# gopi-erabati/Object-Pose-Estimation

Measured on NVIDIA B200. Metric: frames_per_sec_fpfh_sacia_icp_640x480, higher is better.
Workload: dtype f32

## Files before the change

object-pose-estimation_b200/csrc/pipeline.cu:

```cuda
#include <algorithm>
#include <atomic>
#include <cmath>
#include <functional>
#include <memory>
#include <thread>
#include <sched.h>

#include "ope_host.cuh"

using namespace ope;


namespace {

bool model_cache_enabled() {
  const char* e = std::getenv("OPE_MODEL_CACHE");
  return !e || std::atoi(e) != 0;
}

int clone_cloud(ope_ctx* ctx, const ope_cloud* in, ope_cloud** out) {
  ope_cloud* o = nullptr;
  OPE_TRY(cloud_alloc(ctx, in->n, in->normals != nullptr, &o));
  cudaError_t e = cudaSuccess;
  if (in->n) {
    e = cudaMemcpyAsync(o->pts, in->pts, in->n * sizeof(float4), cudaMemcpyDeviceToDevice, ctx->stream);
    if (e == cudaSuccess && in->normals)
      e = cudaMemcpyAsync(o->normals, in->normals, in->n * sizeof(float4), cudaMemcpyDeviceToDevice, ctx->stream);
  }
  if (e != cudaSuccess) { ope_cloud_free(ctx, o); return fail(ctx, OPE_ERR_CUDA, "device copy failed: %s", cudaGetErrorString(e)); }
  *out = o;
  return OPE_OK;
}

struct StageTimer {
  ope_pose_tracker* t;
  explicit StageTimer(ope_pose_tracker* tr) : t(tr) { if (t->timing) cudaEventRecord(t->ev0, t->ctx->stream); }
  void lap(int s) {
    if (!t->timing) return;
    cudaEventRecord(t->ev1, t->ctx->stream);
    cudaEventSynchronize(t->ev1);
    float ms = 0;
    cudaEventElapsedTime(&ms, t->ev0, t->ev1);
    t->stage_ms[s] += ms;
    std::swap(t->ev0, t->ev1);
  }
};

int sub_sample_and_normals(ope_pose_tracker* t, StageTimer& tm, ope_cloud* in, float leaf, ope_cloud** out) {
  ope_ctx* ctx = t->ctx;
  int* d_idx = nullptr;
  size_t m = 0;
  OPE_TRY(uniform_sample_device(ctx, in, leaf, &d_idx, &m));
  ope_cloud* ds = nullptr;
  int rc = gather_cloud(ctx, in, d_idx, m, &ds);
  dfree(ctx, d_idx);
  if (rc != OPE_OK) return rc;
  dfree(ctx, ds->normals);
  ds->normals = nullptr;
  tm.lap(0);
  const float vp[3] = {0, 0, 0};
  rc = normals_device(ctx, ds, t->prm.normal_k, vp);
  if (rc != OPE_OK) { ope_cloud_free(ctx, ds); return rc; }
  tm.lap(1);
  *out = ds;
  return OPE_OK;
}

struct CloudGuard {
  ope_ctx* ctx;
  ope_cloud* c = nullptr;
  explicit CloudGuard(ope_ctx* x) : ctx(x) {}
  ~CloudGuard() { if (c) ope_cloud_free(ctx, c); }
};
struct DevGuard {
  ope_ctx* ctx;
  float* p = nullptr;
  explicit DevGuard(ope_ctx* x) : ctx(x) {}
  ~DevGuard() { dfree(ctx, p); }
};

}

extern "C" {

int ope_pose_tracker_create(ope_ctx* ctx, const ope_pose_params* prm, ope_pose_tracker** out) {
  OPE_ENTER(ctx);
  if (!ctx || !out) return OPE_ERR_INVALID;
  ope_pose_tracker* t = new ope_pose_tracker();
  t->ctx = ctx;
  if (prm) t->prm = *prm; else ope_pose_params_default(&t->prm);
  if (cudaEventCreate(&t->ev0) != cudaSuccess || cudaEventCreate(&t->ev1) != cudaSuccess ||
      cudaEventCreate(&t->evt0) != cudaSuccess || cudaEventCreate(&t->evt1) != cudaSuccess) {
    delete t;
    return fail(ctx, OPE_ERR_CUDA, "event creation failed");
  }
  *out = t;
  return OPE_OK;
}

void ope_pose_tracker_destroy(ope_pose_tracker* t) {
  if (!t) return;
  if (t->alignedSource) ope_cloud_free(t->ctx, t->alignedSource);
  if (t->cloudModel) ope_cloud_free(t->ctx, t->cloudModel);
  cudaEventDestroy(t->ev0); cudaEventDestroy(t->ev1); cudaEventDestroy(t->evt0); cudaEventDestroy(t->evt1);
  delete t;
}

int ope_pose_stage_ms(const ope_pose_tracker* t, double out[8]) {
  if (!t || !out) return OPE_ERR_INVALID;
  std::memcpy(out, t->stage_ms, sizeof(t->stage_ms));
  return OPE_OK;
}

int ope_pose_estimate_final_device(ope_pose_tracker* t, ope_cloud** source, const ope_cloud* target,
                                   const ope_rng_table* table, ope_pose_result* res) {
  OPE_ENTER((t ? t->ctx : nullptr));
  if (!t || !source || !*source || !res) return OPE_ERR_INVALID;
  ope_ctx* ctx = t->ctx;
  const ope_pose_params& P = t->prm;
  std::memset(res, 0, sizeof(*res));
  std::memset(t->stage_ms, 0, sizeof(t->stage_ms));
  if (t->timing) cudaEventRecord(t->evt0, ctx->stream);
  StageTimer tm(t);
  ope_cloud* p_source = *source;
  const size_t nt = target ? target->n : 0;
  if (t->firstTimePose == 0) {
    if (t->cloudModel) { ope_cloud_free(ctx, t->cloudModel); t->cloudModel = nullptr; }
    OPE_TRY(clone_cloud(ctx, p_source, &t->cloudModel));
  }
  t->firstTimePose++;
  Mat4 coarse = mat4_identity(), fine = mat4_identity();

  if (nt != 0 && t->fitnessScoreFine > P.coarse_refit_threshold) {
    res->ran_coarse = 1;
    CloudGuard sp(ctx), tp(ctx);
    DevGuard fs(ctx), ft(ctx);
    bool cached = t->cache_sp && t->cache_fs && t->firstTimePose == 1 && t->cache_model_n == p_source->n;
    ope_cloud sp_view;
    const ope_cloud* spc = nullptr;
    const float* fsp = nullptr;
    ModelCacheEntry* hit = nullptr;
    unsigned long long src_hash = 0;
    const bool use_ctx_cache = !cached && model_cache_enabled();
    if (use_ctx_cache) {
      OPE_TRY(cloud_content_hash(ctx, p_source, &src_hash));
      for (auto& e : ctx->model_cache)
        if (e.hash == src_hash && e.n == p_source->n && e.leaf == P.coarse_leaf && e.k == P.normal_k && e.radius == P.fpfh_radius) hit = &e;
      if (hit) { hit->stamp = ++ctx->model_cache_clock; ctx->model_cache_hits++; } else ctx->model_cache_misses++;
      tm.lap(0);
    }
    if (cached || hit) {
      sp_view = cached ? *t->cache_sp : *hit->sp;
      sp_view.ctx = ctx; sp_view.grids.clear();
      spc = &sp_view; fsp = cached ? t->cache_fs : hit->fs;
      cached = true;
    } else {
      OPE_TRY(sub_sample_and_normals(t, tm, p_source, P.coarse_leaf, &sp.c));
      spc = sp.c;
    }
    OPE_TRY(sub_sample_and_normals(t, tm, const_cast<ope_cloud*>(target), P.coarse_leaf, &tp.c));
    if (!cached) {
      OPE_TRY(fpfh_device(ctx, sp.c, P.fpfh_radius, &fs.p, nullptr));
      fsp = fs.p;
      if (use_ctx_cache) {
        ModelCacheEntry e;
        e.hash = src_hash; e.n = p_source->n; e.leaf = P.coarse_leaf; e.k = P.normal_k; e.radius = P.fpfh_radius;
        e.sp = sp.c; e.fs = fs.p; e.stamp = ++ctx->model_cache_clock;
        ope_cloud_invalidate(ctx, e.sp);
        sp.c = nullptr; fs.p = nullptr;
        if (ctx->model_cache.size() >= 4) {
          size_t old = 0;
          for (size_t i = 1; i < ctx->model_cache.size(); ++i) if (ctx->model_cache[i].stamp < ctx->model_cache[old].stamp) old = i;
          ope_cloud_free(ctx, ctx->model_cache[old].sp); dfree(ctx, ctx->model_cache[old].fs);
          ctx->model_cache[old] = e;
          hit = &ctx->model_cache[old];
        } else {
          ctx->model_cache.push_back(e);
          hit = &ctx->model_cache.back();
        }
        sp_view = *hit->sp; sp_view.ctx = ctx; sp_view.grids.clear();
        spc = &sp_view; fsp = hit->fs;
        cached = true;
      }
    }
    OPE_TRY(fpfh_device(ctx, tp.c, P.fpfh_radius, &ft.p, nullptr));
    tm.lap(2);
    res->n_src_coarse = (int32_t)spc->n; res->n_tgt_coarse = (int32_t)tp.c->n;
    ope_cloud* fresh = nullptr;
    if ((int)tp.c->n < P.min_target_features) {
      OPE_TRY(clone_cloud(ctx, p_source, &fresh));
    } else {
      ope_reg_result rr;
      int src_rc = sacia_device(ctx, spc, fsp, tp.c, ft.p, P.sacia, table, nullptr, &rr, nullptr);
      if (cached) ope_cloud_invalidate(ctx, &sp_view);
      OPE_TRY(src_rc);
      tm.lap(3);
      std::memcpy(coarse.m, rr.T, sizeof(coarse.m));
      res->sacia_best_iteration = rr.best_iteration; res->sacia_best_error = rr.best_error;
      OPE_TRY(cloud_alloc(ctx, p_source->n, false, &fresh));
      ope_cloud view = *p_source;
      view.normals = nullptr; view.grids.clear();
      const int trc = transform_device(ctx, &view, coarse, fresh);
      if (trc != OPE_OK) { ope_cloud_free(ctx, fresh); return trc; }
      tm.lap(6);
    }
    if (t->alignedSource) ope_cloud_free(ctx, t->alignedSource);
    t->alignedSource = fresh;
  }
  if (nt != 0 && t->alignedSource) {
    CloudGuard sp(ctx), tp(ctx);
    OPE_TRY(sub_sample_and_normals(t, tm, t->alignedSource, P.fine_leaf, &sp.c));
    OPE_TRY(sub_sample_and_normals(t, tm, const_cast<ope_cloud*>(target), P.fine_leaf, &tp.c));
    OPE_TRY(remove_nan_normals_device(ctx, &sp.c));
    OPE_TRY(remove_nan_normals_device(ctx, &tp.c));
    tm.lap(1);
    res->n_src_fine = (int32_t)sp.c->n; res->n_tgt_fine = (int32_t)tp.c->n;
    if ((int)tp.c->n >= P.min_target_points) {
      ope_reg_result rr;
      OPE_TRY(icp_device(ctx, sp.c, tp.c, P.icp, mat4_identity(), &rr, nullptr, nullptr));
      tm.lap(4);
      std::memcpy(fine.m, rr.T, sizeof(fine.m));
      OPE_TRY(fitness_device(ctx, sp.c, tp.c, fine, DBL_MAX, &t->fitnessScoreFine));
      tm.lap(5);
      ope_cloud* moved = nullptr;
      OPE_TRY(cloud_alloc(ctx, t->alignedSource->n, false, &moved));
      int rc = transform_device(ctx, t->alignedSource, fine, moved);
      if (rc != OPE_OK) { ope_cloud_free(ctx, moved); return rc; }
      ope_cloud_free(ctx, t->alignedSource);
      t->alignedSource = moved;
      t->alignedStrength = (double)rr.n_correspondences / (double)((long)sp.c->n + (long)tp.c->n);
      res->icp_iterations = rr.iterations; res->icp_converged = rr.converged; res->icp_state = rr.state;
      tm.lap(6);
    }
  }
  const Mat4 pose = mat4_mul(coarse, fine);
  Mat4 rigid = mat4_identity();
  if (t->cloudModel && t->cloudModel->n > 0 && t->cloudModel->n <= p_source->n) {
    OPE_TRY(umeyama_device(ctx, t->cloudModel->pts, p_source->pts, nullptr, nullptr, t->cloudModel->n, rigid.m));
  }
  const Mat4 final_pose = mat4_mul(rigid, pose);
  {
    ope_cloud* copy = nullptr;
    if (t->alignedSource) OPE_TRY(clone_cloud(ctx, t->alignedSource, &copy));
    else OPE_TRY(cloud_alloc(ctx, 0, false, &copy));
    ope_cloud_free(ctx, p_source);
    *source = copy;
  }
  tm.lap(6);
  std::memcpy(res->final_pose, final_pose.m, 64); std::memcpy(res->coarse_pose, coarse.m, 64);
  std::memcpy(res->fine_pose, fine.m, 64); std::memcpy(res->rigid_model_pose, rigid.m, 64);
  res->fitness = t->fitnessScoreFine; res->align_strength = t->alignedStrength;
  if (t->timing) {
    cudaEventRecord(t->evt1, ctx->stream);
    cudaEventSynchronize(t->evt1);
    float ms = 0;
    cudaEventElapsedTime(&ms, t->evt0, t->evt1);
    t->stage_ms[7] = ms;
  }
  return OPE_OK;
}

}

namespace ope {
int run_chunks_on_lanes(ope_ctx* ctx, size_t n, const std::atomic<int>* stop,
                        const std::function<int(ope_ctx*, size_t, size_t, size_t)>& run_chunk, size_t chunk_items) {
  const char* ce = std::getenv("OPE_BATCH_CHUNK");
  const char* le = std::getenv("OPE_BATCH_LANES");
  int cores = (int)std::thread::hardware_concurrency();
  {
    cpu_set_t set;
    CPU_ZERO(&set);
    if (sched_getaffinity(0, sizeof(set), &set) == 0 && CPU_COUNT(&set) > 0) cores = CPU_COUNT(&set);
    const char* lw = std::getenv("LOCAL_WORLD_SIZE");
    if (lw && std::atoi(lw) > 1) cores = std::max(1, cores / std::atoi(lw));
  }
  int lanes = std::max(1, std::min(le ? std::atoi(le) : std::max(2, cores - 1), 8));
  if (ctx->batch_timing) lanes = 1;
  size_t chunk = chunk_items ? chunk_items : (size_t)std::max(1, ce ? std::atoi(ce) : 296);
  if (!ce && !chunk_items) {
    if (lanes > 1) {
      const size_t per_round = (size_t)lanes * 32;
      const size_t rounds = std::max<size_t>(1, (n + per_round / 2) / per_round);
      chunk = std::max<size_t>(std::min<size_t>(8, n), (n + rounds * lanes - 1) / (rounds * lanes));
    } else {
      const size_t rounds = std::max<size_t>(3, (n + 295) / 296);
      chunk = std::max<size_t>(std::min<size_t>(74, n), (n + rounds - 1) / rounds);
    }
  }
  const size_t n_chunks = (n + chunk - 1) / chunk;
  lanes = (int)std::min<size_t>((size_t)lanes, n_chunks);
  while ((int)ctx->workers.size() < lanes - 1) {
    ope_ctx* w = nullptr;
    const int rc = ope_ctx_create(ctx->device, nullptr, &w);
    if (rc != OPE_OK) return fail(ctx, rc, "worker context creation failed");
    ctx->workers.push_back(w);
  }
  if (lanes > 1) OPE_TRY(ope_ctx_synchronize(ctx));
  int wait_mode = lanes + 1 > cores ? 2 : 0;
  if (const char* e = std::getenv("OPE_BATCH_LANE_SYNC")) wait_mode = std::strcmp(e, "block") == 0 ? 2 : std::strcmp(e, "yield") == 0 ? 1 : 0;
  struct WaitMode {
    ope_ctx* main; cudaEvent_t saved_event; bool saved_yield; cudaEvent_t mine = nullptr;
    explicit WaitMode(ope_ctx* c) : main(c), saved_event(c->sync_event), saved_yield(c->sync_yield) {}
    ~WaitMode() { main->sync_event = saved_event; main->sync_yield = saved_yield; if (mine) cudaEventDestroy(mine); }
  } wait_guard(ctx);
  if (lanes > 1) {
    for (int l = 0; l < lanes; ++l) {
      ope_ctx* c = l == 0 ? ctx : ctx->workers[(size_t)l - 1];
      if (l > 0 && c->sync_event) { cudaEventDestroy(c->sync_event); c->sync_event = nullptr; }
      cudaEvent_t ev = nullptr;
      if (wait_mode != 0 && cudaEventCreateWithFlags(&ev, (wait_mode == 2 ? cudaEventBlockingSync : 0) | cudaEventDisableTiming) != cudaSuccess) ev = nullptr;
      if (l == 0) wait_guard.mine = ev;
      c->sync_event = ev;
      c->sync_yield = wait_mode == 1 && ev;
    }
  }
  std::atomic<size_t> next_chunk{0};
  std::atomic<int> lane_rc{OPE_OK};
  std::mutex lane_mu;
  std::string lane_msg;
  auto run_lane = [&](ope_ctx* c) {
    ope::enter(c);
    for (;;) {
      const size_t f0 = next_chunk.fetch_add(1) * chunk;
      if (f0 >= n || lane_rc.load() != OPE_OK || (stop && stop->load() != OPE_OK)) break;
      const size_t nf = std::min(chunk, n - f0);
      const int rc = run_chunk(c, f0, nf, f0 / chunk);
      if (rc != OPE_OK) {
        std::lock_guard<std::mutex> lock(lane_mu);
        if (lane_rc.load() == OPE_OK) { lane_rc.store(rc); lane_msg = c->error; }
        break;
      }
    }
    if (c != ctx) stream_sync(c);
  };
  {
    std::vector<std::thread> lane_threads;
    struct JoinLanes { std::vector<std::thread>& t; ~JoinLanes() { for (auto& th : t) if (th.joinable()) th.join(); } } join_lanes{lane_threads};
    try {
      for (int l = 1; l < lanes; ++l) lane_threads.emplace_back(run_lane, ctx->workers[(size_t)l - 1]);
    } catch (...) {
    }
    run_lane(ctx);
  }
  if (lane_rc.load() != OPE_OK) return fail(ctx, lane_rc.load(), "%s", lane_msg.c_str());
  return OPE_OK;
}

}

extern "C" {

namespace {

int pose_one_frame(ope_ctx* c, const ope_pose_params& P, const ope_cloud* model, const ope_cloud* sp, const float* fs,
                   const ope_frame_input& in, const ope_rng_table* table, ope_pose_result* res) {
  struct IcpSettings {
    ope_ctx* c; bool prefer_small; int max_blocks;
    ~IcpSettings() { c->icp_prefer_small = prefer_small; c->icp_max_blocks = max_blocks; }
  } restore{c, c->icp_prefer_small, c->icp_max_blocks};
  c->icp_prefer_small = true;
  c->icp_max_blocks = std::max(8, c->sm_count / 8);
  ope_pose_tracker* t = nullptr;
  int rc = ope_pose_tracker_create(c, &P, &t);
  ope_cloud* src = nullptr;
  ope_cloud* tgt_owned = nullptr;
  const ope_cloud* tgt = nullptr;
  if (rc == OPE_OK) {
    t->timing = false;
    t->cache_sp = sp; t->cache_fs = fs; t->cache_model_n = model->n;
    rc = clone_cloud(c, model, &src);
  }
  if (rc == OPE_OK) {
    if (in.points) {
      if (in.n > 0) rc = ope_cloud_upload(c, in.points, in.n, in.stride, in.offset, nullptr, 0, 0, &tgt_owned);
      tgt = tgt_owned;
    } else if (in.cloud && ((const ope_cloud*)in.cloud)->n > 0) {
      ope_cloud view = *(const ope_cloud*)in.cloud;
      view.normals = nullptr; view.grids.clear(); view.bbox_valid = false;
      rc = clone_cloud(c, &view, &tgt_owned);
      tgt = tgt_owned;
    }
  }
  if (rc == OPE_OK) rc = ope_pose_estimate_final_device(t, &src, tgt, table, res);
  if (src) ope_cloud_free(c, src);
  if (tgt_owned) ope_cloud_free(c, tgt_owned);
  if (t) ope_pose_tracker_destroy(t);
  return rc;
}

}

int ope_pose_batch(ope_ctx* ctx, const ope_pose_params* prm, const float* model_xyz, size_t n_model, const ope_frame_input* frames,
                   size_t n_frames, const ope_rng_table* tables, int workers, ope_pose_result* results, int32_t* status) {
  OPE_ENTER(ctx);
  if (!ctx || !model_xyz || n_model == 0 || (!frames && n_frames) || !results) return OPE_ERR_INVALID;
  if (n_frames == 0) return OPE_OK;
  ope_pose_params P;
  if (prm) P = *prm; else ope_pose_params_default(&P);
  struct Borrowed { ope_cloud* c = nullptr; } model, sp;
  struct BorrowedF { float* p = nullptr; } fs;
  Mat4 rigid = mat4_identity();
  {
    unsigned long long h = 0x9e3779b97f4a7c15ull;
    const uint32_t* w = (const uint32_t*)model_xyz;
    unsigned long long h2 = 0xc2b2ae3d27d4eb4full;
    const size_t words = n_model * 3;
    size_t i = 0;
    for (; i + 2 <= words; i += 2) {
      h = (h ^ w[i]) * 0x9fb21c651e98df25ull; h = (h << 29) | (h >> 35);
      h2 = (h2 ^ w[i + 1]) * 0x9fb21c651e98df25ull; h2 = (h2 << 31) | (h2 >> 33);
    }
    for (; i < words; ++i) { h = (h ^ w[i]) * 0x9fb21c651e98df25ull; h = (h << 29) | (h >> 35); }
    h ^= h2 * 3 + n_model;
    BatchModelCache& C = ctx->batch_model;
    const bool hit = model_cache_enabled() && C.model && C.hash == h && C.n == n_model && C.leaf == P.coarse_leaf && C.k == P.normal_k &&
                     C.radius == P.fpfh_radius;
    if (!hit) {
      if (C.model) ope_cloud_free(ctx, C.model);
      if (C.sp) ope_cloud_free(ctx, C.sp);
      dfree(ctx, C.fs);
      C = BatchModelCache();
      OPE_TRY(ope_cloud_upload(ctx, model_xyz, n_model, 12, 0, nullptr, 0, 0, &C.model));
      ope_pose_tracker tmp;
      tmp.ctx = ctx; tmp.prm = P; tmp.timing = false;
      StageTimer tm(&tmp);
      OPE_TRY(sub_sample_and_normals(&tmp, tm, C.model, P.coarse_leaf, &C.sp));
      OPE_TRY(fpfh_device(ctx, C.sp, P.fpfh_radius, &C.fs, nullptr));
      Mat4 R = mat4_identity();
      OPE_TRY(umeyama_device(ctx, C.model->pts, C.model->pts, nullptr, nullptr, C.model->n, R.m));
      std::memcpy(C.rigid, R.m, sizeof(C.rigid));
      C.hash = h; C.n = n_model; C.leaf = P.coarse_leaf; C.k = P.normal_k; C.radius = P.fpfh_radius;
    }
    model.c = C.model; sp.c = C.sp; fs.p = C.fs;
    std::memcpy(rigid.m, C.rigid, sizeof(C.rigid));
  }
  std::vector<int32_t> draw_s, draw_p;
  std::vector<ope_rng_table> drawn;
  std::atomic<size_t> tables_ready{n_frames};
  std::atomic<int> draw_rc{OPE_OK};
  std::thread drawer;
  struct JoinDrawer { std::thread& t; ~JoinDrawer() { if (t.joinable()) t.join(); } } join_drawer{drawer};
  if (!tables) {
    const int H = P.sacia.max_iterations, S = P.sacia.nr_samples, K = P.sacia.k_correspondences;
    if (H < 1 || S < 1 || K < 1) return fail(ctx, OPE_ERR_INVALID, "bad SAC-IA parameters");
    auto xyz = std::make_shared<std::vector<float>>(3 * std::max<size_t>(sp.c->n, 1));
    OPE_TRY(ope_cloud_download(ctx, sp.c, xyz->data(), nullptr));
    draw_s.resize(n_frames * (size_t)H * S); draw_p.resize(n_frames * (size_t)H * S);
    drawn.resize(n_frames);
    tables_ready.store(0);
    const size_t n_sp = sp.c->n;
    const float msd0 = P.sacia.min_sample_distance;
    auto draw_all = [&, xyz, H, S, K, n_sp, msd0]() {
      for (size_t f = 0; f < n_frames; ++f) {
        float msd = msd0;
        int32_t* s = draw_s.data() + f * (size_t)H * S;
        int32_t* p = draw_p.data() + f * (size_t)H * S;
        const int rc = ope_sacia_draw(xyz->data(), n_sp, 12, H, S, K, &msd, s, p);
        if (rc != OPE_OK) { draw_rc.store(rc); tables_ready.store(n_frames); return; }
        drawn[f] = ope_rng_table{H, S, s, p};
        tables_ready.store(f + 1, std::memory_order_release);
      }
    };
    try { drawer = std::thread(draw_all); } catch (...) { draw_all(); }
    tables = drawn.data();
  }
  const bool fast = icp_small_batch_applicable(P.icp, 1, 1) && P.icp.n_rejectors >= 0;
  std::mutex frame_mu;
  std::vector<size_t> rest;
  int lrc = run_chunks_on_lanes(ctx, n_frames, &draw_rc, [&](ope_ctx* c, size_t f0, size_t nf, size_t) -> int {
    PoseChunk ch;
    ch.targets = frames + f0; ch.first = f0; ch.active.assign(nf, fast ? 1 : 0);
    ch.src_pts = sp.c->pts; ch.src_fpfh = fs.p; ch.src_n = (int)sp.c->n;
    ch.fine_src.assign(nf, model.c->pts); ch.fine_n.assign(nf, (int)model.c->n);
    OPE_TRY(pose_chunk(c, P, (int)nf, ch, [&](PoseChunk& k) -> int {
      while (tables_ready.load(std::memory_order_acquire) < f0 + nf) sched_yield();
      for (size_t i = 0; i < nf; ++i) k.tables[i] = tables + f0 + i;
      return OPE_OK;
    }));
    for (size_t i = 0; i < nf; ++i) {
      const size_t f = f0 + i;
      if (ch.active[i]) {
        results[f] = chunk_pose_result(ch, (int)i, rigid);
        if (status) status[f] = OPE_OK;
        continue;
      }
      std::lock_guard<std::mutex> lock(frame_mu);
      rest.push_back(f);
    }
    return OPE_OK;
  });
  if (lrc != OPE_OK) {
    if (draw_rc.load() != OPE_OK) tables_ready.store(n_frames);
    return lrc;
  }
  if (drawer.joinable()) drawer.join();
  if (draw_rc.load() != OPE_OK) return fail(ctx, draw_rc.load(), "selectSamples failed");
  std::sort(rest.begin(), rest.end());
  size_t failed_frame = n_frames;
  int failed_rc = OPE_OK;
  std::string failed_msg;
  lrc = run_chunks_on_lanes(ctx, rest.size(), nullptr, [&](ope_ctx* c, size_t i0, size_t, size_t) -> int {
    const size_t f = rest[i0];
    const int rc = pose_one_frame(c, P, model.c, sp.c, fs.p, frames[f], tables + f, &results[f]);
    if (status) status[f] = rc;
    if (rc != OPE_OK) {
      std::lock_guard<std::mutex> lock(frame_mu);
      if (f < failed_frame) { failed_frame = f; failed_rc = rc; failed_msg = c->error; }
    }
    return OPE_OK;
  }, 1);
  if (lrc != OPE_OK) return lrc;
  if (failed_rc != OPE_OK) return fail(ctx, failed_rc, "frame %zu: %s", failed_frame, failed_msg.c_str());
  return OPE_OK;
}

int ope_register_point_clouds(ope_ctx* ctx, const ope_frame_input* views, size_t n_views, const ope_icp_params* prm, int normal_k,
                              ope_reg_result* pair_results, ope_cloud** merged) {
  OPE_ENTER(ctx);
  if (!ctx || !views || n_views == 0 || !prm || !merged) return OPE_ERR_INVALID;
  auto load = [&](const ope_frame_input& v, ope_cloud** out) -> int {
    if (v.points) return ope_cloud_upload(ctx, v.points, v.n, v.stride, v.offset, nullptr, 0, 0, out);
    if (!v.cloud) return fail(ctx, OPE_ERR_INVALID, "view without points");
    ope_cloud view = *(const ope_cloud*)v.cloud;
    view.normals = nullptr; view.grids.clear();
    return clone_cloud(ctx, &view, out);
  };
  CloudGuard cur(ctx);
  OPE_TRY(load(views[0], &cur.c));
  const float vp[3] = {0, 0, 0};
  for (size_t i = 0; i + 1 < n_views; ++i) {
    CloudGuard tgt(ctx), moved(ctx);
    OPE_TRY(load(views[i + 1], &tgt.c));
    ope_reg_result rr;
    std::memset(&rr, 0, sizeof(rr));
    for (int j = 0; j < 16; ++j) rr.T[j] = (j % 5 == 0) ? 1.f : 0.f;
    if (cur.c->n > 0 && tgt.c->n > 0) {
      ope_cloud_invalidate(ctx, cur.c);
      OPE_TRY(normals_device(ctx, cur.c, normal_k, vp));
      OPE_TRY(normals_device(ctx, tgt.c, normal_k, vp));
      OPE_TRY(icp_device(ctx, cur.c, tgt.c, *prm, mat4_identity(), &rr, nullptr, nullptr));
    }
    if (pair_results) pair_results[i] = rr;
    Mat4 M;
    std::memcpy(M.m, rr.T, sizeof(M.m));
    OPE_TRY(cloud_alloc(ctx, cur.c->n, false, &moved.c));
    ope_cloud view = *cur.c;
    view.normals = nullptr; view.grids.clear();
    OPE_TRY(transform_device(ctx, &view, M, moved.c));
    dfree(ctx, tgt.c->normals); tgt.c->normals = nullptr;
    OPE_TRY(ope_cloud_append(ctx, moved.c, tgt.c));
    std::swap(cur.c, moved.c);
  }
  OPE_CUDA_TRY(ctx, stream_sync(ctx));
  *merged = cur.c;
  cur.c = nullptr;
  return OPE_OK;
}

int ope_pose_batch_stage_ms(ope_ctx* ctx, int enable, double out[12]) {
  if (!ctx) return OPE_ERR_INVALID;
  if (out) std::memcpy(out, ctx->batch_stage_ms, 12 * sizeof(double));
  if (enable >= 0) { ctx->batch_timing = enable != 0; std::memset(ctx->batch_stage_ms, 0, sizeof(ctx->batch_stage_ms)); }
  return OPE_OK;
}

int ope_pose_estimate_final(ope_pose_tracker* t, float* source_xyz, size_t ns, const void* target, size_t nt, size_t tstride,
                            size_t toffset, const ope_rng_table* table, ope_pose_result* res) {
  OPE_ENTER((t ? t->ctx : nullptr));
  if (!t || !source_xyz || !res) return OPE_ERR_INVALID;
  ope_ctx* ctx = t->ctx;
  ope_cloud* src = nullptr;
  OPE_TRY(ope_cloud_upload(ctx, source_xyz, ns, 12, 0, nullptr, 0, 0, &src));
  CloudGuard tg(ctx);
  if (nt > 0) {
    int rc = ope_cloud_upload(ctx, target, nt, tstride, toffset, nullptr, 0, 0, &tg.c);
    if (rc != OPE_OK) { ope_cloud_free(ctx, src); return rc; }
  }
  int rc = ope_pose_estimate_final_device(t, &src, tg.c, table, res);
  if (rc == OPE_OK && src->n == ns) rc = ope_cloud_download(ctx, src, source_xyz, nullptr);
  ope_cloud_free(ctx, src);
  return rc;
}

}
// ... 1 lines not shown
```

object-pose-estimation_b200/csrc/registration.cu:

```cuda
#include <cooperative_groups.h>

#include <algorithm>
#include <cmath>
#include <cstdlib>

#include <map>
#include <mutex>

#include <chrono>
#include "ope_host.cuh"
#include "ope_octet.cuh"

namespace cg = cooperative_groups;

namespace ope {

__global__ void transform_kernel(const float4* __restrict__ in, const float4* __restrict__ in_n, int n, Mat4 T,
                                 float4* __restrict__ out, float4* __restrict__ out_n) {
  int i = blockIdx.x * blockDim.x + threadIdx.x;
  if (i >= n) return;
  float4 p = __ldg(in + i);
  float4 o = p;
  xform_point(T, p.x, p.y, p.z, o.x, o.y, o.z);
  out[i] = o;
  if (in_n && out_n) {
    float4 v = __ldg(in_n + i);
    float4 w = v;
    xform_normal(T, v.x, v.y, v.z, w.x, w.y, w.z);
    out_n[i] = w;
  }
}

static constexpr int kRedThreads = 256;
static constexpr int kMomentAcc = 16;

__device__ __forceinline__ double warp_sum_d(double v) {
  for (int o = 16; o > 0; o >>= 1) v += __shfl_xor_sync(0xffffffffu, v, o);
  return v;
}

template <int NACC>
__device__ __forceinline__ void block_reduce_store(double* acc, double* smem , double* dst) {
  const int lane = threadIdx.x & 31, warp = threadIdx.x >> 5, nw = blockDim.x >> 5;
#pragma unroll
  for (int a = 0; a < NACC; ++a) acc[a] = warp_sum_d(acc[a]);
  if (lane == 0)
    for (int a = 0; a < NACC; ++a) smem[warp * NACC + a] = acc[a];
  __syncthreads();
  if (threadIdx.x < NACC) {
    double s = 0.0;
    for (int w = 0; w < nw; ++w) s += smem[w * NACC + threadIdx.x];
    dst[threadIdx.x] = s;
  }
  __syncthreads();
}

__global__ void moments_kernel(const float4* __restrict__ src, const float4* __restrict__ tgt, const int* __restrict__ is,
                               const int* __restrict__ it, int n, double* __restrict__ partials) {
  __shared__ double smem[(kRedThreads / 32) * kMomentAcc];
  double acc[kMomentAcc];
  for (int a = 0; a < kMomentAcc; ++a) acc[a] = 0.0;
  double o[3];
  { const float4 t0 = __ldg(tgt); moment_origin(t0.x, t0.y, t0.z, o[0], o[1], o[2]); }
  for (int i = blockIdx.x * blockDim.x + threadIdx.x; i < n; i += gridDim.x * blockDim.x) {
    const float4 s = __ldg(src + (is ? is[i] : i));
    const float4 t = __ldg(tgt + (it ? it[i] : i));
    const double sv[3] = {(double)s.x - o[0], (double)s.y - o[1], (double)s.z - o[2]};
    const double tv[3] = {(double)t.x - o[0], (double)t.y - o[1], (double)t.z - o[2]};
    acc[0] += 1.0;
    acc[1] += sv[0]; acc[2] += sv[1]; acc[3] += sv[2];
    acc[4] += tv[0]; acc[5] += tv[1]; acc[6] += tv[2];
    for (int c = 0; c < 3; ++c)
      for (int r = 0; r < 3; ++r) acc[7 + c * 3 + r] += tv[r] * sv[c];
  }
  block_reduce_store<kMomentAcc>(acc, smem, partials + (size_t)blockIdx.x * kMomentAcc);
}
__device__ __forceinline__ void umeyama_final(const double* __restrict__ partials, int nblocks, float* __restrict__ out16, const float4* __restrict__ tgt) {
  __shared__ double acc[kMomentAcc];
  const int a = threadIdx.x >> 5, lane = threadIdx.x & 31;
  if (a < kMomentAcc) {
    double s = 0.0;
    for (int b = lane; b < nblocks; b += 32) s += partials[(size_t)b * kMomentAcc + a];
    s = warp_sum_d(s);
    if (lane == 0) acc[a] = s;
  }
  __syncthreads();
  if (threadIdx.x == 0) {
    Mat4 T;
    double o[3];
    const float4 t0 = __ldg(tgt);
    moment_origin(t0.x, t0.y, t0.z, o[0], o[1], o[2]);
    umeyama_from_moments(acc, T, o[0], o[1], o[2]);
    for (int i = 0; i < 16; ++i) out16[i] = T.m[i];
  }
}
__global__ void umeyama_final_kernel(const double* __restrict__ partials, int nblocks, float* __restrict__ out16,
                                     const float4* __restrict__ tgt) {
  umeyama_final(partials, nblocks, out16, tgt);
}

__global__ void __launch_bounds__(kRedThreads) track_commit_kernel(const TrackCommit* __restrict__ commits, double* __restrict__ partials) {
  __shared__ double smem[(kRedThreads / 32) * kMomentAcc];
  const TrackCommit& c = commits[blockIdx.y];
  if ((int)blockIdx.x >= c.nb) return;
  const int stride = c.nb * kRedThreads;
  Mat4 C, F;
  for (int i = 0; i < 16; ++i) { C.m[i] = c.coarse[i]; F.m[i] = c.fine[i]; }
  for (int i = blockIdx.x * kRedThreads + threadIdx.x; i < c.n_in; i += stride) {
    float4 p = __ldg(c.in + i);
    if (c.pre) { float4 q = p; xform_point(C, p.x, p.y, p.z, q.x, q.y, q.z); p = q; }
    float4 o = p;
    xform_point(F, p.x, p.y, p.z, o.x, o.y, o.z);
    c.out_aligned[i] = o;
    c.out_source[i] = o;
  }
  if (c.n_model == 0) return;
  double acc[kMomentAcc];
  for (int a = 0; a < kMomentAcc; ++a) acc[a] = 0.0;
  double o[3];
  { const float4 t0 = __ldg(c.src); moment_origin(t0.x, t0.y, t0.z, o[0], o[1], o[2]); }
  for (int i = blockIdx.x * kRedThreads + threadIdx.x; i < c.n_model; i += stride) {
    const float4 s = __ldg(c.model + i);
    const float4 t = __ldg(c.src + i);
    const double sv[3] = {(double)s.x - o[0], (double)s.y - o[1], (double)s.z - o[2]};
    const double tv[3] = {(double)t.x - o[0], (double)t.y - o[1], (double)t.z - o[2]};
    acc[0] += 1.0;
    acc[1] += sv[0]; acc[2] += sv[1]; acc[3] += sv[2];
    acc[4] += tv[0]; acc[5] += tv[1]; acc[6] += tv[2];
    for (int cc = 0; cc < 3; ++cc)
      for (int r = 0; r < 3; ++r) acc[7 + cc * 3 + r] += tv[r] * sv[cc];
  }
  block_reduce_store<kMomentAcc>(acc, smem, partials + ((size_t)blockIdx.y * gridDim.x + blockIdx.x) * kMomentAcc);
}
__global__ void track_umeyama_final_kernel(const TrackCommit* __restrict__ commits, const double* __restrict__ partials, int max_nb,
                                           float* __restrict__ out16) {
  const TrackCommit& c = commits[blockIdx.x];
  if (c.n_model == 0) return;
  umeyama_final(partials + (size_t)blockIdx.x * max_nb * kMomentAcc, c.nb, out16 + (size_t)blockIdx.x * 16, c.src);
}

static constexpr int kNnThreads = 256;
__global__ void __launch_bounds__(kNnThreads) fitness_kernel(GridView g, const float4* __restrict__ src, int n, Mat4 T,
                                                             float max_range_f, double* __restrict__ partials) {
  extern __shared__ __align__(16) unsigned char smem_raw[];
  Nn1Smem<kNnThreads>* nn = reinterpret_cast<Nn1Smem<kNnThreads>*>(smem_raw);
  __shared__ double smem[(kNnThreads / 32) * 2];
  double acc[2] = {0.0, 0.0};
  for (int base = blockIdx.x * kNnThreads; base < n; base += gridDim.x * kNnThreads) {
    const int i = base + (int)threadIdx.x;
    float x = 0, y = 0, z = 0;
    bool ok = false;
    if (i < n) {
      const float4 p = __ldg(src + i);
      xform_point(T, p.x, p.y, p.z, x, y, z);
      ok = finite3(x, y, z);
    }
    float d2;
    const int idx = block_nn1<kNnThreads>(g, nn, ok, x, y, z, FLT_MAX, -1, nullptr, d2);
    if (ok && idx >= 0 && d2 <= max_range_f) { acc[0] += (double)d2; acc[1] += 1.0; }
  }
  block_reduce_store<2>(acc, smem, partials + (size_t)blockIdx.x * 2);
}
static constexpr int kFitSmemMax = 4096;
__global__ void __launch_bounds__(kNnThreads) fitness_smem_kernel(const float4* __restrict__ tgt, int nt, const float4* __restrict__ src, int n,
                                                                  Mat4 T, float max_range_f, double* __restrict__ partials) {
  extern __shared__ __align__(16) float4 tg_fit[];
  __shared__ double smem[(kNnThreads / 32) * 2];
  const int nt8 = (nt + 7) & ~7;
  for (int j = threadIdx.x; j < nt8; j += kNnThreads) tg_fit[j] = j < nt ? __ldg(tgt + j) : make_float4(INFINITY, INFINITY, INFINITY, 0.0f);
  __syncthreads();
  double acc[2] = {0.0, 0.0};
  for (int base = blockIdx.x * kNnThreads; base < n; base += gridDim.x * kNnThreads) {
    const int i = base + (int)threadIdx.x;
    float x = 0, y = 0, z = 0;
    bool ok = false;
    if (i < n) {
      const float4 p = __ldg(src + i);
      xform_point(T, p.x, p.y, p.z, x, y, z);
      ok = finite3(x, y, z);
    }
    float best = INFINITY;
    if (ok) {
      for (int j0 = 0; j0 < nt8; j0 += 8) {
        float d2[8];
#pragma unroll
        for (int u = 0; u < 8; ++u) { const float4 t = tg_fit[j0 + u]; d2[u] = dist2(x, y, z, t.x, t.y, t.z); }
#pragma unroll
        for (int u = 0; u < 8; ++u) if (d2[u] < best) best = d2[u];
      }
    }
    if (ok && best <= max_range_f) { acc[0] += (double)best; acc[1] += 1.0; }
  }
  block_reduce_store<2>(acc, smem, partials + (size_t)blockIdx.x * 2);
}
__global__ void sum_partials_kernel(const double* __restrict__ partials, int nblocks, int nacc, double* __restrict__ out) {
  const int a = threadIdx.x >> 5, lane = threadIdx.x & 31;
  if (blockIdx.x != 0 || a >= nacc) return;
  double s = 0.0;
  for (int b = lane; b < nblocks; b += 32) s += partials[(size_t)b * nacc + a];
  s = warp_sum_d(s);
  if (lane == 0) out[a] = s;
}

struct IcpDev {
  GridView grid;
  const float4* tgt_pts;
  const float4* tgt_nrm;
  const float4* src0_pts;
  const float4* src0_nrm;
  const float4* src_sorted;
  int n_src;
  int n_work;
  float4* cur_pts;
  float4* cur_nrm;
  int max_iterations, min_corr, estimator, k_search, n_rej, transformation, variant, force_all;
  int rej_kind[OPE_MAX_REJECTORS];
  double rej_thr[OPE_MAX_REJECTORS];
  double max_corr_dist;
  float max_d2_f;
  double rot_thr, trans_thr, rel_mse_thr, abs_mse_thr;
  int max_similar, fail_after_max;
  int* corr_match;
  float* corr_d2;
  int* seed;
  float4* ref;
  float cert_gap;
  int dfs_max;
  int tgt_in_smem;
  int n_tgt;
  int split_min;
  int small_max;
  float4* def_q;
  int4* def_m;
  float4* def_res;
  int* def_count;
  int* def_head;
  double* partials;
  unsigned* barrier;
  ope_reg_result* result;
  long long* phase_cycles;
  Mat4 guess;
};

static constexpr int kIcpThreads = 512;
static constexpr int kIcpWarps = kIcpThreads / 32;
static constexpr int kIcpAcc = 17;
static constexpr int kIcpMaxBlocks = 1024;
static constexpr int kIcpSmemMaxTargets = 4096;
static constexpr int kIcpSplitMin = 6144;


struct IcpSmem {
  OctStack wstack[kIcpWarps];
  float2 knn_buf[kIcpWarps][kKnnBufCap + 32];
  LeafList leaves[kIcpWarps];
  int dir[kDirEntries];
  Nn1Smem<kIcpThreads> nn;
  double red[kIcpWarps][kIcpAcc];
  double totals[kIcpAcc];
  int prefix[2][kIcpMaxBlocks];
  int warp_cnt[2][kIcpWarps];
  int n_def[2];
  Mat4 T_inc;
  int stop;
};

__device__ __forceinline__ void grid_barrier(unsigned* counter, unsigned target) {
  __syncthreads();
  if (threadIdx.x == 0) {
    asm volatile("red.release.gpu.global.add.u32 [%0], 1;" ::"l"(counter) : "memory");
    unsigned v;
    do {
      asm volatile("ld.acquire.gpu.global.u32 %0, [%1];" : "=r"(v) : "l"(counter) : "memory");
    } while (v < target);
  }
  __syncthreads();
}

__device__ __forceinline__ double warp_reduce16(const double* v, int lane, int& slot) {
  double w8[8], w4[4], w2[2], w1;
  const bool b16 = lane & 16, b8 = lane & 8, b4 = lane & 4, b2 = lane & 2;
#pragma unroll
  for (int j = 0; j < 8; ++j) {
    const double keep = b16 ? v[j + 8] : v[j], give = b16 ? v[j] : v[j + 8];
    w8[j] = keep + __shfl_xor_sync(0xffffffffu, give, 16);
  }
#pragma unroll
  for (int j = 0; j < 4; ++j) {
    const double keep = b8 ? w8[j + 4] : w8[j], give = b8 ? w8[j] : w8[j + 4];
    w4[j] = keep + __shfl_xor_sync(0xffffffffu, give, 8);
  }
#pragma unroll
  for (int j = 0; j < 2; ++j) {
    const double keep = b4 ? w4[j + 2] : w4[j], give = b4 ? w4[j] : w4[j + 2];
    w2[j] = keep + __shfl_xor_sync(0xffffffffu, give, 4);
  }
  {
    const double keep = b2 ? w2[1] : w2[0], give = b2 ? w2[0] : w2[1];
    w1 = keep + __shfl_xor_sync(0xffffffffu, give, 2);
  }
  w1 += __shfl_xor_sync(0xffffffffu, w1, 1);
  slot = (b16 ? 8 : 0) + (b8 ? 4 : 0) + (b4 ? 2 : 0) + (b2 ? 1 : 0);
  return w1;
}

__device__ __forceinline__ double moment_term(int e, const float4 p, const float4 t, float d2, const double o[3]) {
  if (e == 0) return 1.0;
  if (e < 4) return e == 1 ? (double)p.x - o[0] : (e == 2 ? (double)p.y - o[1] : (double)p.z - o[2]);
  if (e < 7) return e == 4 ? (double)t.x - o[0] : (e == 5 ? (double)t.y - o[1] : (double)t.z - o[2]);
  if (e < 16) {
    const int c = (e - 7) / 3, r = (e - 7) % 3;
    const double sv = c == 0 ? (double)p.x - o[0] : (c == 1 ? (double)p.y - o[1] : (double)p.z - o[2]);
    const double tv = r == 0 ? (double)t.x - o[0] : (r == 1 ? (double)t.y - o[1] : (double)t.z - o[2]);
    return tv * sv;
  }
  return (double)d2;
}

__device__ __forceinline__ int icp_reject(const IcpDev& a, int s, int orig, const float4 p, int match) {
  const bool stale = a.variant == OPE_ICP_VARIANT_MODCORR;
  for (int r = 0; r < a.n_rej && match >= 0; ++r) {
    const float4 sn = stale ? __ldg(a.src0_nrm + orig) : a.cur_nrm[s];
    double score;
    if (a.rej_kind[r] == OPE_REJ_SURFACE_NORMAL) {
      const float4 tn = __ldg(a.tgt_nrm + match);
      score = (double)((sn.x * tn.x) + (sn.y * tn.y) + (sn.z * tn.z));
    } else {
      const float4 sp = stale ? __ldg(a.src0_pts + orig) : p;
      const double sl = (double)sqrtf(sp.x * sp.x + sp.y * sp.y + sp.z * sp.z);
      score = (double)((sn.x * (-sp.x / sl)) + (sn.y * (-sp.y / sl)) + (sn.z * (-sp.z / sl)));
    }
    if (!(score > a.rej_thr[r])) match = -1;
  }
  return match;
}

__device__ __forceinline__ int icp_gate(const IcpDev& a, int s, int orig, const float4 p, int nn, float d2) {
  int match = nn;
  if (match >= 0 && (double)d2 > a.max_corr_dist * a.max_corr_dist) match = -1;
  if (match >= 0) match = icp_reject(a, s, orig, p, match);
  return match;
}

__device__ __forceinline__ int icp_correspond_shooting(const IcpDev& a, OctStack* st, int s, int orig, const float4 p, bool use_seed,
                                                       float& d2_out, const float4* tg_smem = nullptr, float2* knn_buf = nullptr) {
  const unsigned full = 0xffffffffu;
  const int lane = threadIdx.x & 31;
  const bool ok = finite3(p.x, p.y, p.z);
  const bool stale = a.variant == OPE_ICP_VARIANT_MODCORR;
  const int k = a.k_search < a.grid.n ? a.k_search : a.grid.n;
  float bound = FLT_MAX;
  if (use_seed && ok) {
    int pj = -1;
    if (lane < k) pj = a.seed[(size_t)s * a.k_search + lane];
    float d = 0.0f;
    if (pj >= 0) { const float4 t = tg_smem ? tg_smem[pj] : __ldg(a.tgt_pts + pj); d = dist2(p.x, p.y, p.z, t.x, t.y, t.z); }
    const bool all_valid = __ballot_sync(full, lane >= k || pj >= 0) == full;
    for (int o = 16; o > 0; o >>= 1) d = fmaxf(d, __shfl_xor_sync(full, d, o));
    if (all_valid) bound = d;
  }
  float ld;
  int li;
  const int cnt = tg_smem ? (knn_buf ? warp_knn_smem_bounded(tg_smem, a.n_tgt, a.grid.n, ok, p.x, p.y, p.z, a.k_search, bound, knn_buf, ld, li)
                                     : warp_knn_smem(tg_smem, a.n_tgt, a.grid.n, ok, p.x, p.y, p.z, a.k_search, bound, ld, li))
                          : warp_knn(a.grid, st, ok, p.x, p.y, p.z, a.k_search, bound, ld, li);
  if (a.seed && lane < a.k_search) a.seed[(size_t)s * a.k_search + lane] = (lane < cnt) ? li : -1;
  int match = -1;
  float d2 = 0.0f;
  if (cnt > 0) {
    const float4 nr = stale ? __ldg(a.src0_nrm + orig) : a.cur_nrm[s];
    const double N[3] = {nr.x, nr.y, nr.z};
    double dist = DBL_MAX;
    int jdx = 0x7fffffff;
    if (lane < cnt) {
      const float4 t = tg_smem ? tg_smem[li] : __ldg(a.tgt_pts + li);
      const float px = t.x - p.x, py = t.y - p.y, pz = t.z - p.z;
      const double V[3] = {px, py, pz};
      const double C0 = N[1] * V[2] - N[2] * V[1], C1 = N[2] * V[0] - N[0] * V[2], C2 = N[0] * V[1] - N[1] * V[0];
      dist = C0 * C0 + C1 * C1 + C2 * C2;
      jdx = lane;
      if (!(dist < DBL_MAX)) { dist = DBL_MAX; jdx = 0x7fffffff; }
    }
    for (int o = 16; o > 0; o >>= 1) {
      const double od = __shfl_xor_sync(full, dist, o);
      const int oj = __shfl_xor_sync(full, jdx, o);
      if (od < dist || (od == dist && oj < jdx)) { dist = od; jdx = oj; }
    }
    const int pick = jdx == 0x7fffffff ? 0 : jdx;
    const double min_dist = jdx == 0x7fffffff ? DBL_MAX : dist;
    if (!(min_dist > a.max_corr_dist)) {
      match = __shfl_sync(full, li, pick);
      d2 = __shfl_sync(full, ld, pick);
    }
  }
  if (match >= 0) match = icp_reject(a, s, orig, p, match);
  d2_out = d2;
  return match;
}

__device__ __forceinline__ void icp_move(const IcpDev& a, const Mat4& T, int s) {
  float4 p = a.cur_pts[s];
  if (!finite3(p.x, p.y, p.z)) return;
  float x, y, z;
  xform_point(T, p.x, p.y, p.z, x, y, z);
  p.x = x; p.y = y; p.z = z;
  a.cur_pts[s] = p;
  if (a.cur_nrm) {
    float4 v = a.cur_nrm[s];
    if (finite3(v.x, v.y, v.z)) {
      xform_normal(T, v.x, v.y, v.z, x, y, z);
      v.x = x; v.y = y; v.z = z;
      a.cur_nrm[s] = v;
    }
  }
}

__global__ void __launch_bounds__(kIcpThreads, 1) icp_kernel(IcpDev a) {
  extern __shared__ __align__(16) unsigned char smem_raw[];
  IcpSmem* sm = reinterpret_cast<IcpSmem*>(smem_raw);
  double morg[3];
  { const float4 t0 = a.n_tgt > 0 ? __ldg(a.tgt_pts) : make_float4(0, 0, 0, 0); moment_origin(t0.x, t0.y, t0.z, morg[0], morg[1], morg[2]); }
  const int lane = threadIdx.x & 31, warp = threadIdx.x >> 5;
  const int gwarp = blockIdx.x * kIcpWarps + warp, n_gwarps = gridDim.x * kIcpWarps;
  const bool shooting = a.estimator == OPE_EST_NORMAL_SHOOTING;
  OctStack* st = &sm->wstack[warp];

  const int chunk = (a.n_work + (int)gridDim.x - 1) / (int)gridDim.x;
  const int lo = min(a.n_work, (int)blockIdx.x * chunk), hi = min(a.n_work, lo + chunk);
  const int wchunk = (a.n_work + n_gwarps - 1) / n_gwarps;
  const int wlo = min(a.n_work, gwarp * wchunk), whi = min(a.n_work, wlo + wchunk);

  const bool have_guess = !mat4_is_identity(a.guess);
  for (int s = blockIdx.x * kIcpThreads + threadIdx.x; s < a.n_work; s += gridDim.x * kIcpThreads) {
    float4 p = __ldg(a.src_sorted + s);
    const int orig = __float_as_int(p.w);
    float4 v = a.src0_nrm ? __ldg(a.src0_nrm + orig) : make_float4(0, 0, 0, 0);
    if (have_guess) {
      float x, y, z;
      xform_point(a.guess, p.x, p.y, p.z, x, y, z);
      p.x = x; p.y = y; p.z = z;
      if (a.src0_nrm && finite3(v.x, v.y, v.z)) {
        xform_normal(a.guess, v.x, v.y, v.z, x, y, z);
        v.x = x; v.y = y; v.z = z;
      }
    }
    a.cur_pts[s] = p;
    if (a.cur_nrm) a.cur_nrm[s] = v;
  }
  float4* tg_smem = nullptr;
  if (a.tgt_in_smem) {
    tg_smem = reinterpret_cast<float4*>(smem_raw + ((sizeof(IcpSmem) + 15) & ~(size_t)15));
    for (int j = threadIdx.x; j < a.n_tgt; j += kIcpThreads) tg_smem[j] = __ldg(a.tgt_pts + j);
  } else {
    far_dir_load(a.grid, sm->dir);
  }
  FarDir fdir;
  fdir.sdir = sm->dir; fdir.dl = far_dir_level(a.grid);
  unsigned bar_target = gridDim.x;
  grid_barrier(a.barrier, bar_target);

  Mat4 final_t = a.guess;
  double prev_mse = DBL_MAX, cur_mse = DBL_MAX;
  int similar = 0, iterations = 0, state = OPE_CONV_NOT_CONVERGED, converged = 0, n_corr = 0;
  int pass = 0;

  long long t_phase[7] = {0, 0, 0, 0, 0, 0, 0};
  long long t_prev[7] = {0, 0, 0, 0, 0, 0, 0};
  const bool prof_any = a.phase_cycles != nullptr;
  long long n_far = 0;
  const bool prof = a.phase_cycles != nullptr && blockIdx.x == 0 && threadIdx.x == 0;
  for (;; ++pass) {
    long long t0 = prof ? clock64() : 0;
    for (int e = lane; e < kIcpAcc; e += 32) sm->red[warp][e] = 0.0;
    if (threadIdx.x < 2) sm->n_def[threadIdx.x] = 0;
    __syncthreads();
    if (!shooting) {
      for (int base = lo; base < hi; base += kIcpThreads) {
        const int s = base + (int)threadIdx.x;
        const bool in_range = s < hi;
        float4 p = make_float4(0, 0, 0, 0);
        int sd = -1;
        if (in_range) { p = a.cur_pts[s]; if (pass > 0) sd = __ldcg(a.seed + s); }
        const int orig = __float_as_int(p.w);
        const bool ok = in_range && a.grid.n > 0 && finite3(p.x, p.y, p.z);
        Nn1State nst;
        nst.d1 = FLT_MAX; nst.i1 = 0x7fffffff; nst.s2 = FLT_MAX;
        bool far = false, certified = false;
        int total = 0;
        unsigned node_mask = 0u;
        if (ok) {
          const float ux = (p.x - a.grid.ox) * a.grid.inv_h, uy = (p.y - a.grid.oy) * a.grid.inv_h, uz = (p.z - a.grid.oz) * a.grid.inv_h;
          if (sd >= 0) {
            const float4 t = __ldg(a.tgt_pts + sd);
            nst.d1 = dist2(p.x, p.y, p.z, t.x, t.y, t.z);
            nst.i1 = sd;
            const float4 rf = __ldcg(a.ref + s);
            if (rf.w > 0.0f) {
              const float delta = sqrtf(dist2(p.x, p.y, p.z, rf.x, rf.y, rf.z));
              const float d1n = sqrtf(nst.d1);
              certified = (d1n + 2.0f * delta) * 1.00001f + 2e-6f < rf.w;
              if (!certified && a.max_d2_f < FLT_MAX) {
                const float lim = sqrtf(a.max_d2_f) * 1.00001f + 2e-6f;
                certified = d1n > lim && rf.w - delta > lim;
              }
            }
          } else {
            nn1_probe(a.grid, p.x, p.y, p.z, ux, uy, uz, [&](int b, int e) {
              for (int i = b; i < e; ++i) {
                const float4 c = __ldg(a.grid.pts + i);
                nn1_offer(nst, dist2(p.x, p.y, p.z, c.x, c.y, c.z), __float_as_int(c.w));
              }
            });
            nst.s2 = FLT_MAX;
          }
          if (!certified) {
            float r2 = 0.0f;
            far = !nn1_fast(a.grid, p.x, p.y, p.z, ux, uy, uz, a.max_d2_f, a.cert_gap, nst, &r2, &total, &node_mask);
            if (far && total <= a.dfs_max) {
              nn1_thread_dfs(a.grid, p.x, p.y, p.z, ux, uy, uz, a.max_d2_f, a.cert_gap, nst, &r2);
              far = false;
            }
            if (!far) a.ref[s] = make_float4(p.x, p.y, p.z, sqrtf(fminf(nst.s2, r2)));
          }
        }
        const float best_d2 = nst.d1;
        const int best_i = nst.i1;
        int nsub = far ? ((total > a.split_min) ? __popc(node_mask) : 1) : 0;
// ... 7 lines not shown
          __syncthreads();
          if (block_total > hi - lo) { nsub = nsub > 1 ? 1 : nsub; continue; }
          before += incl - nsub;
          if (far) {
            int k = 0;
            for (int j = 0; j < 8; ++j) {
              if (nsub > 1 && !((node_mask >> j) & 1u)) continue;
              if (nsub == 1 && j > 0) break;
              const int slot = hi - 1 - (before + k);
              a.def_q[slot] = make_float4(p.x, p.y, p.z, nst.d1);
              a.def_m[slot] = make_int4(s, nst.i1, orig, nsub > 1 ? j : -1);
              ++k;
            }
          }
          if (threadIdx.x == 0) sm->n_def[1] = block_total;
          break;
        }
        __syncthreads();
        int m = -1;
        float d2 = 0.0f;
        if (ok && !far) {
          const int nn = best_i == 0x7fffffff ? -1 : best_i;
          a.seed[s] = nn;
          d2 = best_d2;
          m = icp_gate(a, s, orig, p, nn, d2);
          a.corr_match[orig] = m;
          a.corr_d2[orig] = d2;
        } else if (in_range && !far) {
          a.seed[s] = -1;
          a.corr_match[orig] = -1;
        }
        if (__ballot_sync(0xffffffffu, m >= 0) != 0u) {
          double v[16];
#pragma unroll
          for (int e = 0; e < 16; ++e) v[e] = 0.0;
          double dsum = 0.0;
          if (m >= 0) {
            const float4 t = __ldg(a.tgt_pts + m);
#pragma unroll
            for (int e = 0; e < 16; ++e) v[e] = moment_term(e, p, t, d2, morg);
            dsum = (double)d2;
          }
          int slot;
          const double w = warp_reduce16(v, lane, slot);
          dsum = warp_sum_d(dsum);
          if ((lane & 1) == 0) sm->red[warp][slot] += w;
          if (lane == 1) sm->red[warp][16] += dsum;
        }
        __syncthreads();
      }
      if (threadIdx.x < 2) a.def_count[threadIdx.x * gridDim.x + blockIdx.x] = sm->n_def[threadIdx.x];
      if (prof) { const long long t1 = clock64(); t_phase[0] += t1 - t0; t0 = t1; n_far += sm->n_def[0] + sm->n_def[1]; }
      bar_target += gridDim.x;
      grid_barrier(a.barrier, bar_target);
      if (prof) { const long long t1 = clock64(); t_phase[1] += t1 - t0; t0 = t1; }
      if (warp < 2) {
        int run = 0;
        for (int b0 = 0; b0 < (int)gridDim.x; b0 += 32) {
          const int b = b0 + lane;
          int c = b < (int)gridDim.x ? __ldcg(a.def_count + warp * gridDim.x + b) : 0;
          for (int o = 1; o < 32; o <<= 1) { const int t = __shfl_up_sync(0xffffffffu, c, o); if (lane >= o) c += t; }
          if (b < (int)gridDim.x) sm->prefix[warp][b] = run + c;
          run += __shfl_sync(0xffffffffu, c, 31);
        }
      }
      __syncthreads();
      if (blockIdx.x == 0 && threadIdx.x < 2) a.def_head[((pass + 1) & 1) * 2 + threadIdx.x] = 0;
      {
        const int total_l = sm->prefix[1][gridDim.x - 1];
        int* head = a.def_head + (pass & 1) * 2 + 1;
        OctStack* stw = &sm->wstack[warp];
        LeafList* llw = &sm->leaves[warp];
        for (;;) {
          int e = 0;
          if (lane == 0) e = atomicAdd(head, 1);
          e = __shfl_sync(0xffffffffu, e, 0);
          if (e >= total_l) break;
          int bl = 0, br = (int)gridDim.x - 1;
          while (bl < br) { const int mid = (bl + br) >> 1; if (sm->prefix[1][mid] > e) br = mid; else bl = mid + 1; }
          const int j = e - (bl > 0 ? sm->prefix[1][bl - 1] : 0);
          const int slot = min(a.n_work, min(a.n_work, bl * chunk) + chunk) - 1 - j;
          const float4 q = __ldcg(a.def_q + slot);
          const int4 qm = __ldcg(a.def_m + slot);
          Nn1State nst;
          nst.d1 = q.w; nst.i1 = qm.y; nst.s2 = FLT_MAX;
          float r2 = 0.0f;
          const long long q0 = prof_any ? clock64() : 0;
          unsigned long long* cnt = (prof_any && pass < 64) ? (unsigned long long*)(a.phase_cycles + 16 + 64 * 8 + 64 + pass * 4) : nullptr;
          if (pass == 0) coop_nn1_far<32, true>(a.grid, fdir, stw, llw, q.x, q.y, q.z, a.max_d2_f, a.cert_gap, nst, &r2, cnt, qm.w);
          else coop_nn1_far<32, false>(a.grid, fdir, stw, llw, q.x, q.y, q.z, a.max_d2_f, a.cert_gap, nst, &r2, cnt, qm.w);
          if (prof_any && lane == 0 && pass < 64) {
            atomicMax((unsigned long long*)(a.phase_cycles + 16 + pass * 8 + 7), (unsigned long long)(clock64() - q0));
            atomicAdd((unsigned long long*)(a.phase_cycles + 16 + 64 * 8 + pass), 1ull);
          }
          if (lane == 0) a.def_res[slot] = make_float4(nst.d1, __int_as_float(nst.i1), nst.s2, r2);
          __syncwarp();
        }
      }
      if (prof) { const long long t1 = clock64(); t_phase[2] += t1 - t0; t0 = t1; }
      bar_target += gridDim.x;
      grid_barrier(a.barrier, bar_target);
      if (prof) { const long long t1 = clock64(); t_phase[3] += t1 - t0; t0 = t1; }
      {
        const int n_def = sm->n_def[1];
        for (int base = 0; base < n_def; base += kIcpThreads) {
          const int j = base + (int)threadIdx.x;
          int m = -1;
          float d2 = 0.0f;
          float4 p = make_float4(0, 0, 0, 0);
          if (j < n_def) {
            const int qslot = hi - 1 - j;
            const int4 qm = a.def_m[qslot];
            const bool first = j == 0 || a.def_m[qslot + 1].x != qm.x;
            if (first) {
              p = a.def_q[qslot];
              Nn1State nst;
              nst.d1 = FLT_MAX; nst.i1 = 0x7fffffff; nst.s2 = FLT_MAX;
              float r2 = FLT_MAX;
              for (int k = 0; k < 8 && j + k < n_def; ++k) {
                if (k > 0 && a.def_m[qslot - k].x != qm.x) break;
                const float4 r = __ldcg(a.def_res + (qslot - k));
                const float rd1 = r.x, rs2 = r.z;
                const int ri1 = __float_as_int(r.y);
                r2 = fminf(r2, r.w);
                if (ri1 == nst.i1) { nst.s2 = fminf(nst.s2, rs2); continue; }
                if (nb_less(rd1, ri1, nst.d1, nst.i1)) { nst.s2 = fminf(fminf(nst.s2, rs2), nst.d1); nst.d1 = rd1; nst.i1 = ri1; }
                else nst.s2 = fminf(fminf(nst.s2, rs2), rd1);
              }
              const int nn = nst.i1 == 0x7fffffff ? -1 : nst.i1;
              d2 = nst.d1;
              m = icp_gate(a, qm.x, qm.z, p, nn, d2);
              a.seed[qm.x] = nn; a.corr_match[qm.z] = m; a.corr_d2[qm.z] = d2;
              a.ref[qm.x] = make_float4(p.x, p.y, p.z, sqrtf(fminf(nst.s2, r2)));
            }
          }
          if (__ballot_sync(0xffffffffu, m >= 0) != 0u) {
            double v[16];
#pragma unroll
            for (int e = 0; e < 16; ++e) v[e] = 0.0;
            double dsum = 0.0;
            if (m >= 0) {
              const float4 t = __ldg(a.tgt_pts + m);
#pragma unroll
              for (int e = 0; e < 16; ++e) v[e] = moment_term(e, p, t, d2, morg);
              dsum = (double)d2;
            }
            int slot;
            const double w = warp_reduce16(v, lane, slot);
            dsum = warp_sum_d(dsum);
            if ((lane & 1) == 0) sm->red[warp][slot] += w;
            if (lane == 1) sm->red[warp][16] += dsum;
          }
        }
      }
      if (prof) { const long long t1 = clock64(); t_phase[4] += t1 - t0; t0 = t1; }
    } else {
      for (int s = wlo; s < whi; ++s) {
        const float4 p = a.cur_pts[s];
        const int orig = __float_as_int(p.w);
        float d2 = 0.0f;
        const int m = icp_correspond_shooting(a, st, s, orig, p, pass > 0, d2, tg_smem, sm->knn_buf[warp]);
        if (lane == 0) { a.corr_match[orig] = m; a.corr_d2[orig] = d2; }
        if (m >= 0 && lane < kIcpAcc) {
          const float4 t = tg_smem ? tg_smem[m] : __ldg(a.tgt_pts + m);
          sm->red[warp][lane] += moment_term(lane, p, t, d2, morg);
        }
        __syncwarp();
      }
      if (prof) { const long long t1 = clock64(); t_phase[0] += t1 - t0; t0 = t1; }
    }
    __syncthreads();
    double* my_partials = a.partials + ((size_t)(pass & 1) * gridDim.x + blockIdx.x) * kIcpAcc;
    if (threadIdx.x < kIcpAcc) {
      double sum = 0.0;
#pragma unroll
      for (int w = 0; w < kIcpWarps; ++w) sum += sm->red[w][threadIdx.x];
      my_partials[threadIdx.x] = sum;
    }
    bar_target += gridDim.x;
    grid_barrier(a.barrier, bar_target);
    if (prof) { const long long t1 = clock64(); t_phase[4] += t1 - t0; t0 = t1; }
    for (int e = warp; e < kIcpAcc; e += kIcpWarps) {
      const double* base = a.partials + (size_t)(pass & 1) * gridDim.x * kIcpAcc;
      double sum = 0.0;
      for (int b0 = lane; b0 < (int)gridDim.x; b0 += 32 * 8) {
        double v[8];
#pragma unroll
        for (int k = 0; k < 8; ++k) { const int b = b0 + 32 * k; v[k] = b < (int)gridDim.x ? __ldcg(base + (size_t)b * kIcpAcc + e) : 0.0; }
#pragma unroll
        for (int k = 0; k < 8; ++k) sum += v[k];
      }
      sum = warp_sum_d(sum);
      if (lane == 0) sm->totals[e] = sum;
    }
    __syncthreads();
    if (warp == 0) {
      int stop = 0;
      n_corr = (int)sm->totals[0];
      if (n_corr < a.min_corr) {
        state = OPE_CONV_NO_CORRESPONDENCES; converged = 0; stop = 2;
        if (lane == 0) sm->T_inc = mat4_identity();
      } else {
        const double n = sm->totals[0];
        double mean = 0.0;
        if (lane < 6) mean = sm->totals[1 + lane] / n;
        double ms[3], mt[3];
#pragma unroll
        for (int k = 0; k < 3; ++k) { ms[k] = __shfl_sync(0xffffffffu, mean, k); mt[k] = __shfl_sync(0xffffffffu, mean, 3 + k); }
        float sg = 0.0f;
        if (lane < 9) {
          const int c = lane / 3, r = lane % 3;
          const double msc = c == 0 ? ms[0] : (c == 1 ? ms[1] : ms[2]);
          const double mtr = r == 0 ? mt[0] : (r == 1 ? mt[1] : mt[2]);
          sg = (float)(sm->totals[7 + lane] / n - mtr * msc);
        }
        float sigma[9];
#pragma unroll
        for (int k = 0; k < 9; ++k) sigma[k] = __shfl_sync(0xffffffffu, sg, k);
        if (lane == 0) {
          Mat4 T;
          const double msu[3] = {ms[0] + morg[0], ms[1] + morg[1], ms[2] + morg[2]};
          const double mtu[3] = {mt[0] + morg[0], mt[1] + morg[1], mt[2] + morg[2]};
          umeyama_from_sigma_means(sigma, msu, mtu, T);
          sm->T_inc = T;
          final_t = mat4_mul(T, final_t);
          ++iterations;
          state = OPE_CONV_NOT_CONVERGED;
          int conv = 0;
          if (iterations >= a.max_iterations) {
            if (!a.fail_after_max) { state = OPE_CONV_ITERATIONS; conv = 1; }
            else { conv = 0; stop = 1; }
          } else {
            const double cos_angle = 0.5 * (double)(T(0, 0) + T(1, 1) + T(2, 2) - 1);
            const double translation_sqr = (double)(T(0, 3) * T(0, 3) + T(1, 3) * T(1, 3) + T(2, 3) * T(2, 3));
            int hit = 0, hit_state = 0;
            if (cos_angle >= a.rot_thr && translation_sqr <= a.trans_thr) { hit = 1; hit_state = OPE_CONV_TRANSFORM; }
            else {
              cur_mse = sm->totals[16] / (double)n_corr;
              if (fabs(cur_mse - prev_mse) < a.abs_mse_thr) { hit = 1; hit_state = OPE_CONV_ABS_MSE; }
              else if (fabs(cur_mse - prev_mse) / prev_mse < a.rel_mse_thr) { hit = 1; hit_state = OPE_CONV_REL_MSE; }
              else prev_mse = cur_mse;
            }
            if (hit) {
              if (similar < a.max_similar) ++similar;
              else { similar = 0; state = hit_state; conv = 1; }
            }
          }
          converged = conv;
          if (a.force_all && iterations < a.max_iterations) conv = 0;
          if (conv) stop = 1;
        }
      }
      if (lane == 0) sm->stop = stop;
    }
    __syncthreads();
    if (prof) { const long long t1 = clock64(); t_phase[5] += t1 - t0; t0 = t1; }
    const int stop = sm->stop;
    if (stop != 2) {
      const Mat4 T = sm->T_inc;
      if (!shooting) { for (int s = lo + (int)threadIdx.x; s < hi; s += kIcpThreads) icp_move(a, T, s); }
      else { for (int s = wlo + lane; s < whi; s += 32) icp_move(a, T, s); __syncwarp(); }
    }
    if (prof) {
      const long long t1 = clock64(); t_phase[6] += t1 - t0;
      if (pass < 64) for (int k = 0; k < 7; ++k) { a.phase_cycles[16 + pass * 8 + k] = t_phase[k] - t_prev[k]; t_prev[k] = t_phase[k]; }
    }
    if (stop) break;
  }
  if (prof) {
    for (int i = 0; i < 7; ++i) a.phase_cycles[i] = t_phase[i];
    a.phase_cycles[7] = n_far;
  }
  if (blockIdx.x == 0 && threadIdx.x == 0) {
    ope_reg_result r;
    for (int i = 0; i < 16; ++i) r.T[i] = final_t.m[i];
    r.converged = converged; r.state = state; r.iterations = iterations; r.n_correspondences = n_corr;
    r.last_mse = cur_mse; r.best_error = 0.0; r.best_iteration = 0; r.reserved = 0;
    *a.result = r;
  }
}

static constexpr int kSlabSlots = 32;
static constexpr int kIcpSmallMaxBlocks = 32;

static constexpr int kIcpSmallThreads = 128;
template <int THREADS>
__device__ __forceinline__ void heap_sift(float2* column, int i, float2 v, const int n) {
  for (;;) {
    const int l = 2 * i + 1;
    if (l >= n) break;
    float2 cv = column[l * THREADS];
    int pick = l;
    if (l + 1 < n) {
      const float2 cr = column[(l + 1) * THREADS];
      if (nb_less(cv.x, __float_as_int(cv.y), cr.x, __float_as_int(cr.y))) { cv = cr; pick = l + 1; }
    }
    if (!nb_less(v.x, __float_as_int(v.y), cv.x, __float_as_int(cv.y))) break;
    column[i * THREADS] = cv;
    i = pick;
  }
  column[i * THREADS] = v;
}

template <int THREADS>
struct IcpSmallSmem {
  double red[THREADS / 32][kIcpAcc];
  double totals[kIcpAcc];
  float2 knn_buf[THREADS / 32][kKnnBufCap + 32];
  float4 wbox[THREADS / 32][2];
  Mat4 T_inc;
  int stop;
};

template <int THREADS>
__device__ __forceinline__ void icp_small_body(const IcpDev& a, const int bid, const int nblk) {
  constexpr int kIcpThreads = THREADS, kIcpWarps = THREADS / 32;
  extern __shared__ __align__(16) unsigned char smem_raw[];
  double morg[3];
  { const float4 t0 = a.n_tgt > 0 ? __ldg(a.tgt_pts) : make_float4(0, 0, 0, 0); moment_origin(t0.x, t0.y, t0.z, morg[0], morg[1], morg[2]); }
  IcpSmallSmem<THREADS>* sm = reinterpret_cast<IcpSmallSmem<THREADS>*>(smem_raw);
  float4* tg = reinterpret_cast<float4*>(smem_raw + ((sizeof(IcpSmallSmem<THREADS>) + 15) & ~(size_t)15));
  const int n_tgt8 = (a.n_tgt + 7) & ~7, n_groups = n_tgt8 >> 3;
  float4* blo = tg + n_tgt8;
  float4* bhi = blo + n_groups;
  float2* slab = reinterpret_cast<float2*>(bhi + n_groups);
  const unsigned full = 0xffffffffu;
  const int tid = threadIdx.x, lane = tid & 31, warp = tid >> 5;
  const int s = bid * kIcpThreads + tid;
  const bool in_range = s < a.n_work;
  const bool stale = a.variant == OPE_ICP_VARIANT_MODCORR;
  const int k = a.k_search < a.grid.n ? a.k_search : a.grid.n;
  auto col = [&](int slot) -> float2& { return slab[slot * kIcpThreads + tid]; };

  float4 p = make_float4(0, 0, 0, 0), nv = make_float4(0, 0, 0, 0);
  int orig = 0;
  if (in_range) {
    p = __ldg(a.src_sorted + s);
    orig = __float_as_int(p.w);
    if (a.src0_nrm) nv = __ldg(a.src0_nrm + orig);
    if (!mat4_is_identity(a.guess)) {
      float x, y, z;
      xform_point(a.guess, p.x, p.y, p.z, x, y, z);
      p.x = x; p.y = y; p.z = z;
      if (a.src0_nrm && finite3(nv.x, nv.y, nv.z)) { xform_normal(a.guess, nv.x, nv.y, nv.z, x, y, z); nv.x = x; nv.y = y; nv.z = z; }
    }
  }
  for (int j = tid; j < n_tgt8; j += kIcpThreads) tg[j] = j < a.n_tgt ? __ldg(a.tgt_pts + j) : make_float4(INFINITY, INFINITY, INFINITY, 0.0f);
  __syncthreads();
  for (int g = tid; g < n_groups; g += kIcpThreads) {
    float4 lo = make_float4(INFINITY, INFINITY, INFINITY, 0.0f), hi = make_float4(-INFINITY, -INFINITY, -INFINITY, 0.0f);
    for (int u = 0; u < 8; ++u) {
      const float4 t = tg[8 * g + u];
      if (!finite3(t.x, t.y, t.z)) continue;
      lo.x = fminf(lo.x, t.x); lo.y = fminf(lo.y, t.y); lo.z = fminf(lo.z, t.z);
      hi.x = fmaxf(hi.x, t.x); hi.y = fmaxf(hi.y, t.y); hi.z = fmaxf(hi.z, t.z);
    }
    blo[g] = lo; bhi[g] = hi;
  }
  __syncthreads();
  const bool ok = in_range && k > 0 && finite3(p.x, p.y, p.z);

  Mat4 final_t = a.guess;
  double prev_mse = DBL_MAX, cur_mse = DBL_MAX;
  int similar = 0, iterations = 0, state = OPE_CONV_NOT_CONVERGED, converged = 0, n_corr = 0;
  unsigned bar_target = 0;
  const bool prof = a.phase_cycles != nullptr && bid == 0 && tid == 0;
  long long t_phase[4] = {0, 0, 0, 0};

  auto coop_query = [&](int q, float bound) {
    const float qx = __shfl_sync(full, p.x, q), qy = __shfl_sync(full, p.y, q), qz = __shfl_sync(full, p.z, q);
    float ld; int li;
    const int cnt = warp_knn_smem_bounded(tg, a.n_tgt, a.grid.n, true, qx, qy, qz, a.k_search, bound, sm->knn_buf[warp], ld, li);
    float2* c = slab + (warp * 32 + q);
    if (lane < kSlabSlots) c[lane * kIcpThreads] = lane < cnt ? make_float2(ld, __int_as_float(li)) : make_float2(FLT_MAX, __int_as_float(-1));
    return cnt;
  };

  for (int pass = 0;; ++pass) {
    long long t0 = prof ? clock64() : 0;
    int c = 0;
    bool have = false;
    bool seeded = pass > 0;
    if (pass == 0) {
      const bool leader = (lane & 7) == 0;
      const unsigned lead = __ballot_sync(full, ok && leader);
      for (unsigned m = lead; m != 0u; m &= m - 1u) { const int q = __ffs(m) - 1; const int cnt = coop_query(q, FLT_MAX); if (lane == q) { c = cnt; have = true; } }
      __syncwarp();
      seeded = !leader && ((lead >> (lane & ~7)) & 1u);
    }
    float bound = FLT_MAX;
    if (ok && !have && seeded) {
      const float2* seed_col = slab + (pass == 0 ? (tid & ~7) : tid);
      float b = 0.0f;
      bool all = true;
#pragma unroll 4
      for (int j = 0; j < k; ++j) {
        const int idx = __float_as_int(seed_col[j * kIcpThreads].y);
        if (idx < 0) { all = false; continue; }
        const float4 t = tg[idx];
        b = fmaxf(b, dist2(p.x, p.y, p.z, t.x, t.y, t.z));
      }
      if (all) bound = b;
    }
    if (pass == 0) __syncwarp();
    const bool scan = ok && !have && bound < FLT_MAX;
    int n_ins = 0;
    bool heaped = false;
    float2 root = make_float2(0.0f, 0.0f);
    const long long ts0 = a.phase_cycles ? clock64() : 0;
    if (__any_sync(full, scan)) {
      auto insert_full = [&](float d2, int j) {
        ++n_ins;
        if (!heaped) {
          for (int i = kSlabSlots / 2 - 1; i >= 0; --i) heap_sift<THREADS>(slab + tid, i, col(i), kSlabSlots);
          heaped = true;
          root = col(0);
          bound = root.x;
        }
        if (nb_less(d2, j, root.x, __float_as_int(root.y))) {
          heap_sift<THREADS>(slab + tid, 0, make_float2(d2, __int_as_float(j)), kSlabSlots);
          root = col(0);
          bound = root.x;
        }
      };
      float wlx = scan ? p.x : INFINITY, wly = scan ? p.y : INFINITY, wlz = scan ? p.z : INFINITY;
      float whx = scan ? p.x : -INFINITY, why = scan ? p.y : -INFINITY, whz = scan ? p.z : -INFINITY;
      float wb = scan ? bound : 0.0f;
#pragma unroll
      for (int o = 16; o > 0; o >>= 1) {
        wlx = fminf(wlx, __shfl_xor_sync(full, wlx, o)); wly = fminf(wly, __shfl_xor_sync(full, wly, o)); wlz = fminf(wlz, __shfl_xor_sync(full, wlz, o));
        whx = fmaxf(whx, __shfl_xor_sync(full, whx, o)); why = fmaxf(why, __shfl_xor_sync(full, why, o)); whz = fmaxf(whz, __shfl_xor_sync(full, whz, o));
        wb = fmaxf(wb, __shfl_xor_sync(full, wb, o));
      }
      if (lane == 0) { sm->wbox[warp][0] = make_float4(wlx, wly, wlz, wb * 1.0002f + 1e-30f); sm->wbox[warp][1] = make_float4(whx, why, whz, 0.0f); }
      __syncwarp();
      for (int g0 = 0; g0 < n_groups; g0 += 32) {
        bool near = false;
        if (g0 + lane < n_groups) {
          const float4 lo = blo[g0 + lane], hi = bhi[g0 + lane], wl = sm->wbox[warp][0], wh = sm->wbox[warp][1];
          const float ex = fmaxf(fmaxf(lo.x - wh.x, wl.x - hi.x), 0.0f), ey = fmaxf(fmaxf(lo.y - wh.y, wl.y - hi.y), 0.0f),
                      ez = fmaxf(fmaxf(lo.z - wh.z, wl.z - hi.z), 0.0f);
          near = ex * ex + ey * ey + ez * ez <= wl.w;
        }
        for (unsigned cand = __ballot_sync(full, near); cand != 0u; cand &= cand - 1u) {
          const int g = g0 + __ffs(cand) - 1;
          const int j0 = 8 * g;
          bool mine = scan;
          if (mine) {
            const float4 lo = blo[g], hi = bhi[g];
            const float ex = fmaxf(fmaxf(lo.x - p.x, p.x - hi.x), 0.0f), ey = fmaxf(fmaxf(lo.y - p.y, p.y - hi.y), 0.0f),
                        ez = fmaxf(fmaxf(lo.z - p.z, p.z - hi.z), 0.0f);
            mine = ex * ex + ey * ey + ez * ez <= bound * 1.0001f + 1e-30f;
          }
          if (!mine) continue;
          float d2[8];
#pragma unroll
          for (int u = 0; u < 8; ++u) { const float4 t = tg[j0 + u]; d2[u] = dist2(p.x, p.y, p.z, t.x, t.y, t.z); }
          unsigned hit = 0u;
#pragma unroll
          for (int u = 0; u < 8; ++u) hit |= (d2[u] <= bound ? 1u : 0u) << u;
          if (hit == 0u) continue;
          if (c + __popc(hit) <= kSlabSlots) {
#pragma unroll
            for (int u = 0; u < 8; ++u)
              if ((hit >> u) & 1u) { col(c) = make_float2(d2[u], __int_as_float(j0 + u)); ++c; }
          } else {
#pragma unroll
            for (int u = 0; u < 8; ++u) {
              const bool h = (hit >> u) & 1u;
              const bool room = c < kSlabSlots;
              if (h & room) col(c) = make_float2(d2[u], __int_as_float(j0 + u));
              if (h & !room) insert_full(d2[u], j0 + u);
              c += (h & room) ? 1 : 0;
            }
          }
        }
      }
    }
    const bool unserved = ok && !have && (!scan || c < k);
    const unsigned redo = __ballot_sync(full, unserved);
    if (a.phase_cycles && pass < 64) {
      unsigned long long* pc = (unsigned long long*)(a.phase_cycles + 16 + pass * 8);
      const unsigned long long dt = (unsigned long long)(clock64() - ts0);
      if (lane == 0) { atomicAdd(pc + 0, dt); atomicMax(pc + 1, dt); atomicAdd(pc + 5, 1ull); }
      if (n_ins > 0) { atomicAdd(pc + 2, (unsigned long long)n_ins); atomicAdd(pc + 3, 1ull); }
      if (ok) atomicAdd(pc + 4, (unsigned long long)c);
    }
    if (a.phase_cycles && bid == 0 && lane == 0 && pass > 0) atomicAdd((unsigned long long*)&a.phase_cycles[4], (unsigned long long)__popc(redo));
    if (a.phase_cycles && bid == 0 && ok && pass > 0) atomicAdd((unsigned long long*)&a.phase_cycles[5], (unsigned long long)c);
    for (unsigned m = redo; m != 0u; m &= m - 1u) {
      const int q = __ffs(m) - 1;
      const float bq = __shfl_sync(full, scan ? bound : FLT_MAX, q);
      const int cnt = coop_query(q, bq);
      if (lane == q) c = cnt;
    }
    __syncwarp();
    if (prof) { const long long t1 = clock64(); t_phase[0] += t1 - t0; t0 = t1; }
    int match = -1;
    float d2m = 0.0f;
    if (ok && c > 0) {
      const float4 nr = stale ? __ldg(a.src0_nrm + orig) : nv;
      const double N0 = nr.x, N1 = nr.y, N2 = nr.z;
      double best = DBL_MAX;
      int best_idx = -1, first_idx = -1;
      float best_d2 = 0.0f, first_d2 = 0.0f;
      while (heaped && c > k) {
        --c;
        if (c > 0) heap_sift<THREADS>(slab + tid, 0, col(c), c);
      }
      while (c > k) {
        int worst = 0;
        float2 wv = col(0);
        for (int e = 1; e < c; ++e) { const float2 o = col(e); if (nb_less(wv.x, __float_as_int(wv.y), o.x, __float_as_int(o.y))) { wv = o; worst = e; } }
        --c;
        if (worst != c) col(worst) = col(c);
      }
      float best_key = 0.0f;
#pragma unroll 4
      for (int e = 0; e < c; ++e) {
        const float2 mine = col(e);
        const int mi = __float_as_int(mine.y);
        if (first_idx < 0 || nb_less(mine.x, mi, first_d2, first_idx)) { first_idx = mi; first_d2 = mine.x; }
        const float4 t = tg[mi];
        const float px = t.x - p.x, py = t.y - p.y, pz = t.z - p.z;
        const double V0 = px, V1 = py, V2 = pz;
        const double C0 = N1 * V2 - N2 * V1, C1 = N2 * V0 - N0 * V2, C2 = N0 * V1 - N1 * V0;
        const double dist = C0 * C0 + C1 * C1 + C2 * C2;
        if (dist < DBL_MAX && (dist < best || (dist == best && nb_less(mine.x, mi, best_key, best_idx)))) {
          best = dist; best_idx = mi; best_d2 = mine.x; best_key = mine.x;
        }
      }
      const int pick_idx = best_idx < 0 ? first_idx : best_idx;
      const float pick_d2 = best_idx < 0 ? first_d2 : best_d2;
      const double min_dist = best_idx < 0 ? DBL_MAX : best;
      if (!(min_dist > a.max_corr_dist)) { match = pick_idx; d2m = pick_d2; }
      for (int r = 0; r < a.n_rej && match >= 0; ++r) {
        const float4 sn = stale ? __ldg(a.src0_nrm + orig) : nv;
        double score;
        if (a.rej_kind[r] == OPE_REJ_SURFACE_NORMAL) {
          const float4 tn = __ldg(a.tgt_nrm + match);
          score = (double)((sn.x * tn.x) + (sn.y * tn.y) + (sn.z * tn.z));
        } else {
          const float4 sp = stale ? __ldg(a.src0_pts + orig) : p;
          const double sl = (double)sqrtf(sp.x * sp.x + sp.y * sp.y + sp.z * sp.z);
          score = (double)((sn.x * (-sp.x / sl)) + (sn.y * (-sp.y / sl)) + (sn.z * (-sp.z / sl)));
        }
        if (!(score > a.rej_thr[r])) match = -1;
      }
    }
    if (ok) for (int j = (c < k ? c : k); j < k; ++j) col(j) = make_float2(FLT_MAX, __int_as_float(-1));
    if (in_range) { a.corr_match[orig] = match; a.corr_d2[orig] = d2m; }
    if (prof) { const long long t1 = clock64(); t_phase[1] += t1 - t0; t0 = t1; }
    {
      double v[16];
#pragma unroll
      for (int e = 0; e < 16; ++e) v[e] = 0.0;
      double dsum = 0.0;
      if (match >= 0) {
        const float4 t = tg[match];
#pragma unroll
        for (int e = 0; e < 16; ++e) v[e] = moment_term(e, p, t, d2m, morg);
        dsum = (double)d2m;
      }
      int slot;
      const double wsum = warp_reduce16(v, lane, slot);
      dsum = warp_sum_d(dsum);
      if ((lane & 1) == 0) sm->red[warp][slot] = wsum;
      if (lane == 1) sm->red[warp][16] = dsum;
    }
    __syncthreads();
    double* my_partials = a.partials + ((size_t)(pass & 1) * nblk + bid) * kIcpAcc;
    if (tid < kIcpAcc) {
      double sum = 0.0;
#pragma unroll
      for (int wv = 0; wv < kIcpWarps; ++wv) sum += sm->red[wv][tid];
      my_partials[tid] = sum;
    }
    if (nblk > 1) { bar_target += nblk; grid_barrier(a.barrier, bar_target); } else __syncthreads();
    if (tid < kIcpAcc) {
      const double* base = a.partials + (size_t)(pass & 1) * nblk * kIcpAcc;
      double sum = 0.0;
      for (int b0 = 0; b0 < nblk; b0 += 8) {
        double v[8];
#pragma unroll
        for (int u = 0; u < 8; ++u) v[u] = b0 + u < nblk ? __ldcg(base + (size_t)(b0 + u) * kIcpAcc + tid) : 0.0;
#pragma unroll
        for (int u = 0; u < 8; ++u) sum += v[u];
      }
      sm->totals[tid] = sum;
    }
    __syncthreads();
    if (prof) { const long long t1 = clock64(); t_phase[2] += t1 - t0; t0 = t1; }
    if (tid == 0) {
      int stop = 0;
      n_corr = (int)sm->totals[0];
      if (n_corr < a.min_corr) {
        state = OPE_CONV_NO_CORRESPONDENCES; converged = 0; stop = 2;
        sm->T_inc = mat4_identity();
      } else {
        Mat4 T;
        umeyama_from_moments(sm->totals, T, morg[0], morg[1], morg[2]);
        sm->T_inc = T;
        final_t = mat4_mul(T, final_t);
        ++iterations;
        state = OPE_CONV_NOT_CONVERGED;
        int conv = 0;
        if (iterations >= a.max_iterations) {
          if (!a.fail_after_max) { state = OPE_CONV_ITERATIONS; conv = 1; }
          else { conv = 0; stop = 1; }
        } else {
          const double cos_angle = 0.5 * (double)(T(0, 0) + T(1, 1) + T(2, 2) - 1);
          const double translation_sqr = (double)(T(0, 3) * T(0, 3) + T(1, 3) * T(1, 3) + T(2, 3) * T(2, 3));
          int hit = 0, hit_state = 0;
          if (cos_angle >= a.rot_thr && translation_sqr <= a.trans_thr) { hit = 1; hit_state = OPE_CONV_TRANSFORM; }
          else {
            cur_mse = sm->totals[16] / (double)n_corr;
            if (fabs(cur_mse - prev_mse) < a.abs_mse_thr) { hit = 1; hit_state = OPE_CONV_ABS_MSE; }
            else if (fabs(cur_mse - prev_mse) / prev_mse < a.rel_mse_thr) { hit = 1; hit_state = OPE_CONV_REL_MSE; }
            else prev_mse = cur_mse;
          }
          if (hit) {
            if (similar < a.max_similar) ++similar;
            else { similar = 0; state = hit_state; conv = 1; }
          }
        }
        converged = conv;
        if (a.force_all && iterations < a.max_iterations) conv = 0;
        if (conv) stop = 1;
      }
      sm->stop = stop;
    }
    __syncthreads();
    const int stop = sm->stop;
    if (stop != 2 && in_range && finite3(p.x, p.y, p.z)) {
      const Mat4 T = sm->T_inc;
      float x, y, z;
      xform_point(T, p.x, p.y, p.z, x, y, z);
      p.x = x; p.y = y; p.z = z;
      if (a.src0_nrm && finite3(nv.x, nv.y, nv.z)) { xform_normal(T, nv.x, nv.y, nv.z, x, y, z); nv.x = x; nv.y = y; nv.z = z; }
    }
    if (prof) { const long long t1 = clock64(); t_phase[3] += t1 - t0; }
    if (stop) break;
  }
  if (prof) for (int i = 0; i < 4; ++i) a.phase_cycles[i] = t_phase[i];
  if (bid == 0 && tid == 0) {
    ope_reg_result r;
    for (int i = 0; i < 16; ++i) r.T[i] = final_t.m[i];
    r.converged = converged; r.state = state; r.iterations = iterations; r.n_correspondences = n_corr;
    r.last_mse = cur_mse; r.best_error = 0.0; r.best_iteration = 0; r.reserved = 0;
    *a.result = r;
  }
}

template <int THREADS>
__global__ void __launch_bounds__(THREADS, 512 / THREADS) icp_small_kernel(IcpDev a) {
  icp_small_body<THREADS>(a, (int)blockIdx.x, (int)gridDim.x);
}
template <int THREADS>
__global__ void __launch_bounds__(THREADS, 512 / THREADS) icp_small_batch_kernel(const IcpDev* __restrict__ descs, const int2* __restrict__ map,
                                                                                unsigned* ticket) {
  __shared__ int s_ticket;
  __shared__ IcpDev s_desc;
  if (threadIdx.x == 0) s_ticket = (int)atomicAdd(ticket, 1u);
  __syncthreads();
  const int2 fb = map[s_ticket];
  for (int w = threadIdx.x; w < (int)(sizeof(IcpDev) / 4); w += THREADS) reinterpret_cast<int*>(&s_desc)[w] = reinterpret_cast<const int*>(descs + fb.x)[w];
  __syncthreads();
  icp_small_body<THREADS>(s_desc, fb.y, (s_desc.n_work + THREADS - 1) / THREADS);
}

__global__ void __launch_bounds__(kIcpThreads, 1) correspond_once_kernel(IcpDev a) {
  extern __shared__ __align__(16) unsigned char smem_raw[];
  IcpSmem* sm = reinterpret_cast<IcpSmem*>(smem_raw);
  const int lane = threadIdx.x & 31, warp = threadIdx.x >> 5;
  if (a.estimator != OPE_EST_NORMAL_SHOOTING) {
    for (int base = blockIdx.x * kIcpThreads; base < a.n_src; base += gridDim.x * kIcpThreads) {
      const int i = base + (int)threadIdx.x;
      const bool in_range = i < a.n_src;
      float4 p = make_float4(0, 0, 0, 0);
      if (in_range) p = a.cur_pts[i];
      const bool ok = in_range && finite3(p.x, p.y, p.z);
      float d2 = 0.0f;
      const int nn = block_nn1<kIcpThreads>(a.grid, &sm->nn, ok, p.x, p.y, p.z, a.max_d2_f, -1, nullptr, d2);
      if (in_range) {
        const int m = ok ? icp_gate(a, i, i, p, nn, d2) : -1;
        a.corr_match[i] = m; a.corr_d2[i] = d2;
      }
    }
  } else {
    OctStack* st = &sm->wstack[warp];
    for (int i = blockIdx.x * kIcpWarps + warp; i < a.n_src; i += gridDim.x * kIcpWarps) {
      const float4 p = a.cur_pts[i];
      float d2 = 0.0f;
      const int m = icp_correspond_shooting(a, st, i, i, p, false, d2);
      if (lane == 0) { a.corr_match[i] = m; a.corr_d2[i] = d2; }
      __syncwarp();
    }
  }
}

__global__ void __launch_bounds__(kIcpThreads, 1) reciprocal_filter_kernel(GridView gsrc, const float4* __restrict__ tgt_pts, int* match,
                                                                           int n, float max_d2_f, double max_corr_dist) {
  extern __shared__ __align__(16) unsigned char smem_raw[];
  IcpSmem* sm = reinterpret_cast<IcpSmem*>(smem_raw);
  for (int base = blockIdx.x * kIcpThreads; base < n; base += gridDim.x * kIcpThreads) {
    const int i = base + (int)threadIdx.x;
    const int m = i < n ? match[i] : -1;
    float4 q = make_float4(0, 0, 0, 0);
    if (m >= 0) q = __ldg(tgt_pts + m);
    const bool ok = m >= 0 && finite3(q.x, q.y, q.z);
    float d2 = 0.0f;
    const int back = block_nn1<kIcpThreads>(gsrc, &sm->nn, ok, q.x, q.y, q.z, max_d2_f, -1, nullptr, d2);
    if (m >= 0 && !(ok && back == i && !((double)d2 > max_corr_dist * max_corr_dist))) match[i] = -1;
  }
}

__global__ void fixed_pairs_kernel(IcpDev a, const int* __restrict__ fq, const int* __restrict__ fm, int n_fixed, int front,
                                   int* __restrict__ is, int* __restrict__ it, float* __restrict__ d2) {
  for (int j = threadIdx.x; j < n_fixed; j += blockDim.x) {
    const int q = fq[j], m = fm[j];
    const float4 s = a.cur_pts[q], t = __ldg(a.tgt_pts + m);
    const float px = t.x - s.x, py = t.y - s.y, pz = t.z - s.z;
    const float dist = front ? (float)((double)(px * px + py * py + pz * pz) * 1e10) : d2[j];
    int keep_all = front ? m : -1, keep_first = a.n_rej > 0 ? m : -1;
    if (front) keep_all = icp_reject(a, q, q, s, m);
    if (a.n_rej > 0) {
      IcpDev one = a;
      one.n_rej = 1;
      keep_first = icp_reject(one, q, q, s, m);
    }
    is[j] = q; it[j] = keep_all; d2[j] = dist;
    is[n_fixed + j] = q; it[n_fixed + j] = keep_first; d2[n_fixed + j] = dist;
  }
}

__global__ void fixed_finite_kernel(const float4* __restrict__ src, const float4* __restrict__ tgt, const int* __restrict__ fq,
                                    const int* __restrict__ fm, int n_fixed, int* __restrict__ first_bad) {
  for (int j = threadIdx.x; j < n_fixed; j += blockDim.x) {
    const float4 s = __ldg(src + fq[j]), t = __ldg(tgt + fm[j]);
    if (!finite3(s.x, s.y, s.z) || !finite3(t.x, t.y, t.z)) atomicMin(first_bad, j);
  }
}

static constexpr int kPairAcc = kMomentAcc + 1;
__global__ void pairs_moments_kernel(const float4* __restrict__ src, const float4* __restrict__ tgt, const int* __restrict__ is,
                                     const int* __restrict__ it, const float* __restrict__ d2, int n, double* __restrict__ partials) {
  __shared__ double smem[(kRedThreads / 32) * kPairAcc];
  double acc[kPairAcc];
  for (int a = 0; a < kPairAcc; ++a) acc[a] = 0.0;
  double o[3];
  { const float4 t0 = __ldg(tgt); moment_origin(t0.x, t0.y, t0.z, o[0], o[1], o[2]); }
  for (int i = blockIdx.x * blockDim.x + threadIdx.x; i < n; i += gridDim.x * blockDim.x) {
    const int m = it[i];
    if (m < 0) continue;
    const float4 s = __ldg(src + (is ? is[i] : i));
    const float4 t = __ldg(tgt + m);
    const double sv[3] = {(double)s.x - o[0], (double)s.y - o[1], (double)s.z - o[2]};
    const double tv[3] = {(double)t.x - o[0], (double)t.y - o[1], (double)t.z - o[2]};
    acc[0] += 1.0;
    acc[1] += sv[0]; acc[2] += sv[1]; acc[3] += sv[2];
    acc[4] += tv[0]; acc[5] += tv[1]; acc[6] += tv[2];
    for (int c = 0; c < 3; ++c)
      for (int r = 0; r < 3; ++r) acc[7 + c * 3 + r] += tv[r] * sv[c];
    acc[kMomentAcc] += (double)d2[i];
  }
  block_reduce_store<kPairAcc>(acc, smem, partials + (size_t)blockIdx.x * kPairAcc);
}

static constexpr int kSaciaThreads = 256;
static constexpr int kSaciaMaxSamples = 16;
static constexpr int kSaciaSmemMaxTargets = 8192;

__global__ void __launch_bounds__(kSaciaThreads) sacia_kernel(SaciaBatch a, GridView grid, float* __restrict__ terms_all) {
  extern __shared__ __align__(16) unsigned char smem_raw[];
  Nn1Smem<kSaciaThreads>* nn = reinterpret_cast<Nn1Smem<kSaciaThreads>*>(smem_raw);
  __shared__ Mat4 T;
  const int h = a.h_begin + blockIdx.x;
  if (threadIdx.x < 16) T.m[threadIdx.x] = __ldg(a.transforms + (size_t)h * 16 + threadIdx.x);
  __syncthreads();
  const Mat4 M = T;
  float* terms = terms_all + (size_t)blockIdx.x * a.ns;
  for (int base = 0; base < a.ns; base += kSaciaThreads) {
    const int i = base + (int)threadIdx.x;
    float x = 0, y = 0, z = 0;
    bool ok = false;
    if (i < a.ns) {
      const float4 p = __ldg(a.src + i);
      xform_point(M, p.x, p.y, p.z, x, y, z);
      ok = finite3(x, y, z);
    }
    float d2;
    const int idx = block_nn1<kSaciaThreads>(grid, nn, ok, x, y, z, a.threshold, -1, nullptr, d2);
    if (i < a.ns) terms[i] = (ok && idx >= 0 && d2 <= a.threshold) ? d2 / a.threshold : 1.0f;
  }
  __syncthreads();
  if (threadIdx.x == 0) {
    float error = 0.0f;
    for (int i = 0; i < a.ns; ++i) error += terms[i];
    a.errors[h] = error;
  }
}
__device__ __forceinline__ float box_d2(const float4 lo, const float4 hi, float x, float y, float z) {
  const float ex = fmaxf(fmaxf(lo.x - x, x - hi.x), 0.0f), ey = fmaxf(fmaxf(lo.y - y, y - hi.y), 0.0f), ez = fmaxf(fmaxf(lo.z - z, z - hi.z), 0.0f);
  return ex * ex + ey * ey + ez * ez;
}
static constexpr int kSeedG = 12;
static constexpr int kSeedCells = kSeedG * kSeedG * kSeedG;
static_assert(kSaciaSmemMaxTargets <= 65536, "the seed grid stores target indices as unsigned short");
static constexpr int kSaciaHypPerBlock = 16;
static constexpr int kSaciaScoreThreads = 128;

static constexpr int kSaciaOrderMax = 4096;
__global__ void __launch_bounds__(kSaciaThreads) sacia_source_order_kernel(SaciaBatch a, int out_stride, float4* __restrict__ out_all) {
  __shared__ unsigned long long keys[kSaciaOrderMax];
  __shared__ float red[6][kSaciaThreads / 32];
  __shared__ float box[6];
  const int f = blockIdx.x;
  if (a.src_stride && !a.active[f]) return;
  const float4* src = a.src + (size_t)f * a.src_stride;
  const int n = a.src_counts ? a.src_counts[f] : a.ns;
  float4* out = out_all + (size_t)f * out_stride;
  const int tid = threadIdx.x, lane = tid & 31, warp = tid >> 5;
  if (n > kSaciaOrderMax) {
    for (int i = tid; i < n; i += kSaciaThreads) { float4 p = __ldg(src + i); p.w = __int_as_float(i); out[i] = p; }
    return;
  }
  float lo[3] = {INFINITY, INFINITY, INFINITY}, hi[3] = {-INFINITY, -INFINITY, -INFINITY};
  for (int i = tid; i < n; i += kSaciaThreads) {
    const float4 p = __ldg(src + i);
    if (!finite3(p.x, p.y, p.z)) continue;
    lo[0] = fminf(lo[0], p.x); lo[1] = fminf(lo[1], p.y); lo[2] = fminf(lo[2], p.z);
    hi[0] = fmaxf(hi[0], p.x); hi[1] = fmaxf(hi[1], p.y); hi[2] = fmaxf(hi[2], p.z);
  }
  for (int o = 16; o > 0; o >>= 1)
    for (int d = 0; d < 3; ++d) { lo[d] = fminf(lo[d], __shfl_xor_sync(0xffffffffu, lo[d], o)); hi[d] = fmaxf(hi[d], __shfl_xor_sync(0xffffffffu, hi[d], o)); }
  if (lane == 0) for (int d = 0; d < 3; ++d) { red[d][warp] = lo[d]; red[3 + d][warp] = hi[d]; }
  __syncthreads();
  if (tid < 6) {
    float v = red[tid][0];
    for (int w = 1; w < kSaciaThreads / 32; ++w) v = tid < 3 ? fminf(v, red[tid][w]) : fmaxf(v, red[tid][w]);
    box[tid] = v;
  }
  __syncthreads();
  const float ext = fmaxf(fmaxf(box[3] - box[0], box[4] - box[1]), fmaxf(box[5] - box[2], 1e-9f));
  const float scale = 1023.0f / ext;
  int m2 = 1;
  while (m2 < n) m2 <<= 1;
  for (int i = tid; i < m2; i += kSaciaThreads) {
    unsigned long long k = ~0ull;
    if (i < n) {
      const float4 p = __ldg(src + i);
      unsigned code = 0x3fffffffu;
      if (finite3(p.x, p.y, p.z))
        code = morton3((unsigned)fminf(fmaxf((p.x - box[0]) * scale, 0.0f), 1023.0f), (unsigned)fminf(fmaxf((p.y - box[1]) * scale, 0.0f), 1023.0f),
                       (unsigned)fminf(fmaxf((p.z - box[2]) * scale, 0.0f), 1023.0f));
      k = ((unsigned long long)code << 32) | (unsigned)i;
    }
    keys[i] = k;
  }
  __syncthreads();
  for (int k2 = 2; k2 <= m2; k2 <<= 1)
    for (int j2 = k2 >> 1; j2 > 0; j2 >>= 1) {
      for (int i = tid; i < m2; i += kSaciaThreads) {
        const int l = i ^ j2;
        if (l > i) {
          const bool up = (i & k2) == 0;
          const unsigned long long ki = keys[i], kl = keys[l];
          if ((ki > kl) == up) { keys[i] = kl; keys[l] = ki; }
        }
      }
      __syncthreads();
    }
  for (int j = tid; j < n; j += kSaciaThreads) {
    const int from = (int)(unsigned)(keys[j] & 0xffffffffull);
    float4 p = __ldg(src + from);
    p.w = __int_as_float(from);
    out[j] = p;
  }
}

__global__ void __launch_bounds__(128) sacia_transform_batch_kernel(SaciaBatch a, int frames) {
  const int nh = a.h_end - a.h_begin;
  const int idx = blockIdx.x * 128 + threadIdx.x;
  if (idx >= frames * nh) return;
  const int f = idx / nh, h = a.h_begin + idx - f * nh;
  if (!a.active[f]) return;
  const float4* tgt = a.tgt + (size_t)f * a.stride;
  double acc[16];
  for (int i = 0; i < 16; ++i) acc[i] = 0.0;
  const int* samples = a.samples + ((size_t)f * a.H + h) * a.nr_samples;
  const int* picks = a.picks + ((size_t)f * a.H + h) * a.nr_samples;
  const int* knn = a.knn_idx + (size_t)f * a.ns * a.k_corr;
  const float4* src = a.src + (size_t)f * a.src_stride;
  for (int j = 0; j < a.nr_samples; ++j) {
    const int si = samples[j];
    int ti = knn[(size_t)si * a.k_corr + picks[j]];
    if (ti < 0) ti = knn[(size_t)si * a.k_corr];
    const float4 sp = __ldg(src + si), tp = __ldg(tgt + ti);
    const double sv[3] = {sp.x, sp.y, sp.z}, tv[3] = {tp.x, tp.y, tp.z};
    acc[0] += 1.0;
    for (int k = 0; k < 3; ++k) { acc[1 + k] += sv[k]; acc[4 + k] += tv[k]; }
    for (int c = 0; c < 3; ++c)
      for (int r = 0; r < 3; ++r) acc[7 + c * 3 + r] += tv[r] * sv[c];
  }
  Mat4 M;
  umeyama_from_moments(acc, M);
  float* out = a.transforms + ((size_t)f * a.H + h) * 16;
  for (int i = 0; i < 16; ++i) out[i] = M.m[i];
}

__global__ void __launch_bounds__(kSaciaThreads) sacia_seed_batch_kernel(SaciaBatch a) {
  extern __shared__ __align__(16) unsigned char smem_raw[];
  float4* tg = reinterpret_cast<float4*>(smem_raw);
  __shared__ float red[6][kSaciaThreads / 32];
  __shared__ float box[6];
  const int f = blockIdx.x;
  if (!a.active[f]) return;
  const int nt = a.counts[f];
  const int tid = threadIdx.x, lane = tid & 31, warp = tid >> 5;
  const float4* scan = (a.tgt_scan ? a.tgt_scan : a.tgt) + (size_t)f * a.stride;
  float lo[3] = {INFINITY, INFINITY, INFINITY}, hi[3] = {-INFINITY, -INFINITY, -INFINITY};
  for (int j = tid; j < nt; j += kSaciaThreads) {
    const float4 t = __ldg(scan + j);
    tg[j] = t;
    if (finite3(t.x, t.y, t.z)) {
      lo[0] = fminf(lo[0], t.x); lo[1] = fminf(lo[1], t.y); lo[2] = fminf(lo[2], t.z);
      hi[0] = fmaxf(hi[0], t.x); hi[1] = fmaxf(hi[1], t.y); hi[2] = fmaxf(hi[2], t.z);
    }
  }
  for (int o = 16; o > 0; o >>= 1)
    for (int d = 0; d < 3; ++d) { lo[d] = fminf(lo[d], __shfl_xor_sync(0xffffffffu, lo[d], o)); hi[d] = fmaxf(hi[d], __shfl_xor_sync(0xffffffffu, hi[d], o)); }
  if (lane == 0) for (int d = 0; d < 3; ++d) { red[d][warp] = lo[d]; red[3 + d][warp] = hi[d]; }
  __syncthreads();
  if (tid < 6) {
    float v = red[tid][0];
    for (int w = 1; w < kSaciaThreads / 32; ++w) v = tid < 3 ? fminf(v, red[tid][w]) : fmaxf(v, red[tid][w]);
    box[tid] = v;
  }
  __syncthreads();
  float ext = fmaxf(fmaxf(box[3] - box[0], box[4] - box[1]), box[5] - box[2]);
  if (!(ext > 1e-6f) || !(ext < FLT_MAX)) ext = 1e-6f;
  const float cell = 1.5f * ext / (float)kSeedG;
  float org[3];
  for (int d = 0; d < 3; ++d) { org[d] = 0.5f * (box[d] + box[3 + d]) - 0.5f * cell * (float)kSeedG; if (!(fabsf(org[d]) < FLT_MAX)) org[d] = 0.0f; }
  if (tid == 0 && blockIdx.y == 0) { a.seed_geo[f] = make_float4(org[0], org[1], org[2], 1.0f / cell); a.best_bits[f] = 0x7f800000u; }
  for (int c = (int)blockIdx.y * kSaciaThreads + tid; c < kSeedCells; c += (int)gridDim.y * kSaciaThreads) {
    const int cx = c % kSeedG, cy = (c / kSeedG) % kSeedG, cz = c / (kSeedG * kSeedG);
    const float x = org[0] + ((float)cx + 0.5f) * cell, y = org[1] + ((float)cy + 0.5f) * cell, z = org[2] + ((float)cz + 0.5f) * cell;
    float best = FLT_MAX;
    int arg = 0;
#pragma unroll 4
    for (int j = 0; j < nt; ++j) {
      const float4 t = tg[j];
      const float d2 = dist2(x, y, z, t.x, t.y, t.z);
      if (d2 < best) { best = d2; arg = j; }
    }
    a.seed_tab[(size_t)f * kSeedCells + c] = (unsigned short)arg;
  }
}

__global__ void __launch_bounds__(kSaciaScoreThreads) sacia_score_batch_kernel(SaciaBatch a, int hyp_per_block) {
  extern __shared__ __align__(16) unsigned char smem_raw[];
  const int f = blockIdx.x;
  if (!a.active[f]) return;
  const int nt = a.counts[f];
  const int nt8 = (nt + 7) & ~7, n_groups = nt8 >> 3;
  float4* tg = reinterpret_cast<float4*>(smem_raw);
  float4* glo = tg + nt8;
  float4* ghi = glo + n_groups;
  float* terms = reinterpret_cast<float*>(ghi + n_groups);
  unsigned short* seed = reinterpret_cast<unsigned short*>(terms + a.ns);
// ... 620 lines not shown
  }
  if (out_aligned) {
    if (n > 0) OPE_TRY(transform_device(ctx, src, final_t, work));
    *out_aligned = work;
    work = nullptr;
  }
  return OPE_OK;
}

class LibcRandSession {
 public:
  LibcRandSession() {
#if defined(__GLIBC__)
    if (!usable()) return;
    begin();
#endif
  }
  ~LibcRandSession() {
#if defined(__GLIBC__)
    if (state_) end();
#endif
  }
  LibcRandSession(const LibcRandSession&) = delete;
  LibcRandSession& operator=(const LibcRandSession&) = delete;
  inline int next() {
#if defined(__GLIBC__)
    if (state_) return step();
#endif
    return rand();
  }
  inline int index(int n) {
    const int r = next();
#if RAND_MAX == 2147483647
    if (n >= 0 && n <= (1 << 21)) return (int)(((long long)n * (long long)r) >> 31);
#endif
    return (int)(n * (r / (RAND_MAX + 1.0)));
  }

 private:
#if defined(__GLIBC__)
  int32_t* word_ = nullptr;
  int32_t* state_ = nullptr;
  int32_t *fptr_ = nullptr, *rptr_ = nullptr, *end_ = nullptr;
  int type_ = 0;

  bool begin() {
    static const int kDeg[5] = {0, 7, 15, 31, 63}, kSep[5] = {0, 3, 1, 3, 1};
    borrow_mutex().lock();
    alignas(8) static char parked[128];
    static bool parked_ready = false;
    char* prev = parked_ready ? setstate(parked) : initstate(1u, parked, sizeof(parked));
    parked_ready = true;
    if (!prev) { borrow_mutex().unlock(); return false; }
    word_ = reinterpret_cast<int32_t*>(prev);
    type_ = word_[0] % 5;
    const int rear = word_[0] / 5;
    if (type_ < 0 || type_ > 4 || (type_ > 0 && (rear < 0 || rear >= kDeg[type_]))) {
      setstate(prev);
      word_ = nullptr;
      borrow_mutex().unlock();
      return false;
    }
    state_ = word_ + 1;
    if (type_ > 0) { rptr_ = state_ + rear; fptr_ = state_ + (rear + kSep[type_]) % kDeg[type_]; end_ = state_ + kDeg[type_]; }
    return true;
  }
  void end() {
    word_[0] = type_ == 0 ? 0 : (int32_t)(5 * (rptr_ - state_) + type_);
    setstate(reinterpret_cast<char*>(word_));
    state_ = nullptr;
    borrow_mutex().unlock();
  }
  static std::mutex& borrow_mutex() { static std::mutex m; return m; }
  inline int step() {
    if (type_ == 0) {
      const int32_t v = (int32_t)(((uint32_t)state_[0] * 1103515245u + 12345u) & 0x7fffffffu);
      state_[0] = v;
      return v;
    }
    const uint32_t v = (uint32_t)*fptr_ + (uint32_t)*rptr_;
    *fptr_ = (int32_t)v;
    ++fptr_;
    if (fptr_ >= end_) { fptr_ = state_; ++rptr_; }
    else { ++rptr_; if (rptr_ >= end_) rptr_ = state_; }
    return (int)(v >> 1);
  }
  static bool usable() {
    static std::once_flag once;
    static bool ok = false;
    std::call_once(once, [] {
      if (const char* e = std::getenv("OPE_LIBC_RAND_FAST")) { if (std::atoi(e) == 0) return; }
      int32_t saved[65];
      int fast[8], slow[8];
      LibcRandSession probe(0);
      auto rewind = [&](size_t words) {
        std::memcpy(probe.word_, saved, words * sizeof(int32_t));
        probe.state_ = nullptr;
        setstate(reinterpret_cast<char*>(probe.word_));
        borrow_mutex().unlock();
      };
      if (!probe.begin()) return;
      const size_t words = probe.type_ == 0 ? 2 : (size_t)(probe.end_ - probe.state_) + 1;
      std::memcpy(saved, probe.word_, words * sizeof(int32_t));
      for (int i = 0; i < 8; ++i) fast[i] = probe.step();
      rewind(words);
      for (int i = 0; i < 8; ++i) slow[i] = rand();
      if (!probe.begin()) return;
      rewind(words);
      ok = std::memcmp(fast, slow, sizeof(fast)) == 0;
    });
    return ok;
  }
  explicit LibcRandSession(int) {}
#endif
};

static float sqrt_threshold(float m) {
  if (!(m > 0.0f)) return 0.0f;
  float c = m * m;
  if (!(c < INFINITY)) return INFINITY;
  while (c > 0.0f && std::sqrt(c) >= m) c = std::nextafter(c, 0.0f);
  while (std::sqrt(c) < m) c = std::nextafter(c, INFINITY);
  return c;
}

static int draw_samples(LibcRandSession& rng, const float* src, size_t ns, size_t stride_f, int nr_samples, float& min_sample_distance,
                        int32_t* out) {
  if (nr_samples > (int)ns) return OPE_ERR_INVALID;
  int without = 0;
  const int max_without = (int)(3 * ns);
  int cnt = 0;
  float too_close = sqrt_threshold(min_sample_distance);
  while (cnt < nr_samples) {
    const int si = rng.index((int)ns);
    bool valid = true;
    const float* a = src + (size_t)si * stride_f;
    for (int i = 0; i < cnt; ++i) {
      const float* b = src + (size_t)out[i] * stride_f;
      const float dx = a[0] - b[0], dy = a[1] - b[1], dz = a[2] - b[2];
      float s = dx * dx;
      s = s + dy * dy;
      s = s + dz * dz;
      if (si == out[i] || s < too_close) { valid = false; break; }
    }
    if (valid) { out[cnt++] = si; without = 0; }
    else ++without;
    if (without >= max_without) { min_sample_distance *= 0.5f; too_close = sqrt_threshold(min_sample_distance); without = 0; }
  }
  return OPE_OK;
}

static size_t sacia_score_bytes(int max_nt, int ns) {
  const size_t nt8 = ((size_t)max_nt + 7) & ~(size_t)7;
  return (nt8 + 2 * (nt8 / 8)) * sizeof(float4) + (size_t)ns * sizeof(float) + (size_t)kSeedCells * sizeof(unsigned short);
}

int sacia_device(ope_ctx* ctx, const ope_cloud* src, const float* d_fsrc, const ope_cloud* tgt, const float* d_ftgt,
                 const ope_sacia_params& prm, const ope_rng_table* table, const float* host_src_xyz3, ope_reg_result* res,
                 float* out_errors_host) {
  const int H = prm.max_iterations, S = prm.nr_samples, K = prm.k_correspondences;
  if (H < 1 || S < 1 || S > kSaciaMaxSamples || K < 1 || K > 16) return fail(ctx, OPE_ERR_INVALID, "bad SAC-IA parameters");
  if (src->n == 0 || tgt->n == 0) return fail(ctx, OPE_ERR_EMPTY, "empty cloud");
  if ((size_t)S > src->n) return fail(ctx, OPE_ERR_INVALID, "The number of samples must not be greater than the number of points");
  int h0 = 0, h1 = H;
  if (prm.hypothesis_end > prm.hypothesis_begin) { h0 = std::min(H, std::max(0, prm.hypothesis_begin)); h1 = std::max(h0, std::min(H, prm.hypothesis_end)); }
  float final_msd = prm.min_sample_distance;
  std::vector<int32_t> hs, hp;
  const int32_t *samples = nullptr, *picks = nullptr;
  if (table) {
    if (table->n_hypotheses < H || table->nr_samples != S) return fail(ctx, OPE_ERR_INVALID, "rng table shape mismatch");
    samples = table->samples; picks = table->picks;
  } else {
    std::vector<float> xyz;
    const float* hx = host_src_xyz3;
    if (!hx) {
      xyz.resize(3 * src->n);
      OPE_TRY(ope_cloud_download(ctx, src, xyz.data(), nullptr));
      hx = xyz.data();
    }
    hs.resize((size_t)H * S); hp.resize((size_t)H * S);
    float& msd = final_msd;
    LibcRandSession rng;
    for (int it = 0; it < H; ++it) {
      int rc = draw_samples(rng, hx, src->n, 3, S, msd, hs.data() + (size_t)it * S);
      if (rc != OPE_OK) return fail(ctx, rc, "selectSamples failed");
      for (int s = 0; s < S; ++s) hp[(size_t)it * S + s] = rng.index(K);
    }
    samples = hs.data(); picks = hp.data();
  }
  for (size_t i = 0; i < (size_t)H * S; ++i)
    if (samples[i] < 0 || (size_t)samples[i] >= src->n || picks[i] < 0 || picks[i] >= K)
      return fail(ctx, OPE_ERR_INVALID, "rng table entry out of range");
  const size_t ns = src->n;
  Scratch<int> d_samples(ctx), d_picks(ctx), d_knn(ctx), d_frame(ctx);
  Scratch<float> d_errors(ctx), d_T(ctx), d_knn_d2(ctx);
  Scratch<ope_reg_result> d_res(ctx);
  OPE_TRY(d_samples.alloc((size_t)H * S)); OPE_TRY(d_picks.alloc((size_t)H * S));
  OPE_TRY(d_knn.alloc(ns * K)); OPE_TRY(d_knn_d2.alloc(ns * K));
  OPE_TRY(d_errors.alloc(H)); OPE_TRY(d_T.alloc((size_t)H * 16)); OPE_TRY(d_res.alloc(1)); OPE_TRY(d_frame.alloc(2));
  const int frame[2] = {(int)tgt->n, 1};
  OPE_CUDA_TRY(ctx, cudaMemcpyAsync(d_samples.p, samples, (size_t)H * S * sizeof(int), cudaMemcpyHostToDevice, ctx->stream));
  OPE_CUDA_TRY(ctx, cudaMemcpyAsync(d_picks.p, picks, (size_t)H * S * sizeof(int), cudaMemcpyHostToDevice, ctx->stream));
  OPE_CUDA_TRY(ctx, cudaMemcpyAsync(d_frame.p, frame, sizeof(frame), cudaMemcpyHostToDevice, ctx->stream));
  OPE_CUDA_TRY(ctx, cudaMemsetAsync(d_errors.p, 0xff, (size_t)H * sizeof(float), ctx->stream));
  OPE_TRY(feature_knn_device(ctx, d_ftgt, tgt->n, d_fsrc, ns, 33, K, d_knn.p, d_knn_d2.p));
  SaciaBatch a;
  std::memset(&a, 0, sizeof(a));
  a.src = src->pts; a.ns = (int)ns; a.tgt = tgt->pts; a.counts = d_frame.p; a.active = d_frame.p + 1;
  a.nr_samples = S; a.k_corr = K; a.H = H; a.h_begin = h0; a.h_end = h1;
  a.samples = d_samples.p; a.picks = d_picks.p; a.knn_idx = d_knn.p;
  a.threshold = (float)prm.max_correspondence_distance; a.errors = d_errors.p; a.transforms = d_T.p;
  a.early_exit = out_errors_host == nullptr;
  const char* force = std::getenv("OPE_SACIA_PATH");
  bool use_smem = tgt->n <= (size_t)kSaciaSmemMaxTargets && !(force && std::strcmp(force, "grid") == 0);
  if (use_smem) {
    int optin = 0;
    cudaFuncAttributes fa;
    OPE_CUDA_TRY(ctx, cudaDeviceGetAttribute(&optin, cudaDevAttrMaxSharedMemoryPerBlockOptin, ctx->device));
    OPE_CUDA_TRY(ctx, cudaFuncGetAttributes(&fa, (const void*)sacia_score_batch_kernel));
    use_smem = sacia_score_bytes((int)tgt->n, (int)ns) + fa.sharedSizeBytes <= (size_t)optin;
  }
  GridView grid;
  if (!use_smem) {
    OPE_TRY(cloud_bbox(ctx, const_cast<ope_cloud*>(tgt)));
    OPE_TRY(cloud_grid(ctx, tgt, knn_cell_size(tgt, 1), &grid));
  }
  OPE_TRY(sacia_batch_device(ctx, a, 1, (int)tgt->n, use_smem ? nullptr : &grid, d_res.p));
  void* h;
  OPE_TRY(read_back(ctx, d_res.p, sizeof(ope_reg_result), &h));
  std::memcpy(res, h, sizeof(ope_reg_result));
  res->last_mse = (double)final_msd;
  if (out_errors_host) {
    OPE_CUDA_TRY(ctx, cudaMemcpyAsync(out_errors_host, d_errors.p, (size_t)H * sizeof(float), cudaMemcpyDeviceToHost, ctx->stream));
    OPE_CUDA_TRY(ctx, ope::stream_sync(ctx));
  }
  return OPE_OK;
}

int sacia_batch_device(ope_ctx* ctx, const SaciaBatch& a_in, int frames, int max_nt, const GridView* grid, ope_reg_result* d_results) {
  SaciaBatch a = a_in;
  if (frames <= 0 || a.H <= 0) return OPE_OK;
  if (a.nr_samples < 1 || a.nr_samples > kSaciaMaxSamples || a.k_corr < 1 || a.k_corr > 16) return fail(ctx, OPE_ERR_INVALID, "bad SAC-IA parameters");
  if (a.h_begin < 0 || a.h_end > a.H || a.h_begin > a.h_end) return fail(ctx, OPE_ERR_INVALID, "bad SAC-IA hypothesis range");
  if (grid && (frames != 1 || a.src_counts)) return fail(ctx, OPE_ERR_INVALID, "the grid SAC-IA scorer takes one frame");
  if (!grid && max_nt > kSaciaSmemMaxTargets) return fail(ctx, OPE_ERR_CAPACITY, "batched SAC-IA: target larger than the shared-memory path");
  { const char* e = std::getenv("OPE_SACIA_EARLY_EXIT"); if (e && std::atoi(e) == 0) a.early_exit = 0; }
  const int nh = a.h_end - a.h_begin;
  Scratch<unsigned short> seed_tab(ctx);
  Scratch<float4> seed_geo(ctx), src_scan(ctx);
  Scratch<unsigned> best_bits(ctx);
  Scratch<float> terms(ctx);
  if (nh > 0) {
    sacia_transform_batch_kernel<<<div_up((size_t)frames * nh, 128), 128, 0, ctx->stream>>>(a, frames);
    OPE_TRY(check_launch(ctx, "sacia_transform_batch_kernel"));
  }
  if (nh > 0 && grid) {
    OPE_TRY(terms.alloc((size_t)nh * a.ns));
    OPE_TRY(dyn_smem(ctx, (const void*)sacia_kernel, sizeof(Nn1Smem<kSaciaThreads>)));
    cudaEventRecord(ctx->kev[1][0], ctx->stream);
    sacia_kernel<<<nh, kSaciaThreads, sizeof(Nn1Smem<kSaciaThreads>), ctx->stream>>>(a, *grid, terms.p);
    cudaEventRecord(ctx->kev[1][1], ctx->stream);
    ctx->kev_valid[1] = true;
    OPE_TRY(check_launch(ctx, "sacia_kernel"));
  } else if (nh > 0) {
    OPE_TRY(seed_tab.alloc((size_t)frames * kSeedCells)); OPE_TRY(seed_geo.alloc((size_t)frames)); OPE_TRY(best_bits.alloc((size_t)frames));
    const int sources = a.src_stride ? frames : 1;
    OPE_TRY(src_scan.alloc((size_t)sources * a.ns));
    a.seed_tab = seed_tab.p; a.seed_geo = seed_geo.p; a.best_bits = best_bits.p; a.src_scan = src_scan.p;
    sacia_source_order_kernel<<<sources, kSaciaThreads, 0, ctx->stream>>>(a, a.ns, src_scan.p);
    OPE_TRY(check_launch(ctx, "sacia_source_order_kernel"));
    const size_t nt8 = ((size_t)max_nt + 7) & ~(size_t)7, bytes = sacia_score_bytes(max_nt, a.ns);
    const unsigned seed_blocks = std::max(1u, std::min(div_up(kSeedCells, kSaciaThreads), (unsigned)(2 * ctx->sm_count / frames)));
    OPE_TRY(dyn_smem(ctx, (const void*)sacia_seed_batch_kernel, nt8 * sizeof(float4)));
    sacia_seed_batch_kernel<<<dim3(frames, seed_blocks), kSaciaThreads, nt8 * sizeof(float4), ctx->stream>>>(a);
    OPE_TRY(check_launch(ctx, "sacia_seed_batch_kernel"));
    int hyp_per_block = kSaciaHypPerBlock;
    while (hyp_per_block > 1 && (size_t)frames * div_up(nh, hyp_per_block) < 2 * (size_t)ctx->sm_count) hyp_per_block /= 2;
    OPE_TRY(dyn_smem(ctx, (const void*)sacia_score_batch_kernel, bytes));
    cudaEventRecord(ctx->kev[1][0], ctx->stream);
    sacia_score_batch_kernel<<<dim3(frames, div_up(nh, hyp_per_block)), kSaciaScoreThreads, bytes, ctx->stream>>>(a, hyp_per_block);
    cudaEventRecord(ctx->kev[1][1], ctx->stream);
    ctx->kev_valid[1] = true;
    OPE_TRY(check_launch(ctx, "sacia_score_batch_kernel"));
  }
  sacia_select_batch_kernel<<<div_up((size_t)frames, 128), 128, 0, ctx->stream>>>(a, frames, d_results);
  return check_launch(ctx, "sacia_select_batch_kernel");
}

int fitness_batch_device(ope_ctx* ctx, const float4* tgt, const int* tgt_counts, const float4* src, const int* src_counts, int stride, int frames,
                         int max_nt, const ope_reg_result* d_icp, const int* d_active, double* d_out) {
  if (frames <= 0) return OPE_OK;
  if (max_nt > kFitSmemMax) return fail(ctx, OPE_ERR_CAPACITY, "batched fitness: target larger than the shared-memory path");
  OPE_TRY(dyn_smem(ctx, (const void*)fitness_smem_batch_kernel, (size_t)kFitSmemMax * sizeof(float4)));
  const size_t bytes = (((size_t)max_nt + 7) & ~(size_t)7) * sizeof(float4);
  fitness_smem_batch_kernel<<<frames, kNnThreads, bytes, ctx->stream>>>(tgt, tgt_counts, src, src_counts, stride, d_icp, d_active, d_out);
  return check_launch(ctx, "fitness_smem_batch_kernel");
}

bool icp_small_batch_applicable(const ope_icp_params& prm, size_t n_src, size_t n_tgt) {
  return prm.estimator == OPE_EST_NORMAL_SHOOTING && prm.transformation == OPE_TE_SVD && !prm.use_reciprocal && n_tgt > 0 &&
         n_tgt <= (size_t)kIcpSmemMaxTargets && n_src > 0 && n_src <= (size_t)kIcpSmallMaxBlocks * kIcpSmallThreads &&
         prm.k_search >= 1 && prm.k_search <= kSlabSlots;
}
template <int THREADS>
static int icp_small_batch_launch(ope_ctx* ctx, const ope_icp_params& prm, const IcpBatchFrame* frames, int n_frames, ope_reg_result* d_results) {
  if (n_frames <= 0) return OPE_OK;
  const bool trace = std::getenv("OPE_BATCH_TRACE") != nullptr;
  auto now = [] { return std::chrono::steady_clock::now(); };
  auto ms_since = [&](std::chrono::steady_clock::time_point t) { return std::chrono::duration<double, std::milli>(now() - t).count(); };
  const auto t_enter = now();
  std::vector<IcpDev> descs((size_t)n_frames);
  std::vector<int2> map;
  size_t max_nt = 0, total_src = 0, total_blocks = 0;
  for (int i = 0; i < n_frames; ++i) {
    if (!icp_small_batch_applicable(prm, (size_t)frames[i].n_src, (size_t)frames[i].n_tgt)) return fail(ctx, OPE_ERR_UNSUPPORTED, "alignment %d does not fit the small-cloud ICP kernel", i);
    max_nt = std::max(max_nt, (size_t)frames[i].n_tgt);
    total_src += (size_t)frames[i].n_src;
    total_blocks += ((size_t)frames[i].n_src + THREADS - 1) / THREADS;
  }
  Scratch<int> match(ctx);
  Scratch<float> d2(ctx);
  Scratch<double> partials(ctx);
  Scratch<unsigned> bars(ctx);
  Scratch<IcpDev> d_descs(ctx);
  Scratch<int2> d_map(ctx);
  OPE_TRY(match.alloc(total_src)); OPE_TRY(d2.alloc(total_src));
  OPE_TRY(partials.alloc(2 * total_blocks * kIcpAcc));
  OPE_TRY(bars.alloc((size_t)n_frames + 1));
  OPE_TRY(d_descs.alloc((size_t)n_frames)); OPE_TRY(d_map.alloc(total_blocks));
  OPE_CUDA_TRY(ctx, cudaMemsetAsync(bars.p, 0, ((size_t)n_frames + 1) * sizeof(unsigned), ctx->stream));
  size_t so = 0, bo = 0;
  map.reserve(total_blocks);
  for (int i = 0; i < n_frames; ++i) {
    IcpDev& a = descs[(size_t)i];
    std::memset(&a, 0, sizeof(a));
    const IcpBatchFrame& f = frames[i];
    a.grid.n = f.n_tgt;
    a.tgt_in_smem = 1; a.n_tgt = f.n_tgt;
    a.tgt_pts = f.tgt_pts; a.tgt_nrm = f.tgt_nrm;
    a.src0_pts = f.src_pts; a.src0_nrm = f.src_nrm; a.src_sorted = f.src_pts;
    a.n_src = f.n_src; a.n_work = f.n_src;
    a.max_iterations = prm.max_iterations; a.min_corr = prm.min_number_correspondences;
    a.estimator = prm.estimator; a.k_search = prm.k_search; a.n_rej = prm.n_rejectors;
    a.transformation = prm.transformation; a.variant = prm.variant; a.force_all = prm.force_all_iterations;
    for (int r = 0; r < OPE_MAX_REJECTORS; ++r) { a.rej_kind[r] = prm.rejector_kind[r]; a.rej_thr[r] = prm.rejector_threshold[r]; }
    a.max_corr_dist = prm.max_correspondence_distance;
    const double m2 = prm.max_correspondence_distance * prm.max_correspondence_distance;
    a.max_d2_f = (m2 >= (double)FLT_MAX || !(m2 == m2)) ? FLT_MAX : (float)m2;
    a.rot_thr = 1.0 - prm.transformation_epsilon; a.trans_thr = prm.transformation_epsilon;
    a.rel_mse_thr = prm.euclidean_fitness_epsilon; a.abs_mse_thr = prm.mse_threshold_absolute;
    a.max_similar = prm.max_iterations_similar_transforms; a.fail_after_max = prm.failure_after_max_iterations;
    a.guess = mat4_identity();
    const int nblk = (f.n_src + THREADS - 1) / THREADS;
    a.corr_match = match.p + so; a.corr_d2 = d2.p + so;
    a.partials = partials.p + 2 * bo * kIcpAcc;
    a.barrier = bars.p + i;
    a.result = d_results + i;
    for (int b = 0; b < nblk; ++b) map.push_back(make_int2(i, b));
    so += (size_t)f.n_src; bo += (size_t)nblk;
  }
  for (int r = 0; r < prm.n_rejectors; ++r)
    if (prm.rejector_kind[r] != OPE_REJ_SURFACE_NORMAL && prm.rejector_kind[r] != OPE_REJ_SELF_OCCLUDED_NORMAL)
      return fail(ctx, OPE_ERR_UNSUPPORTED, "unknown correspondence rejector kind %d", prm.rejector_kind[r]);
  OPE_CUDA_TRY(ctx, cudaMemcpyAsync(d_descs.p, descs.data(), descs.size() * sizeof(IcpDev), cudaMemcpyHostToDevice, ctx->stream));
  OPE_CUDA_TRY(ctx, cudaMemcpyAsync(d_map.p, map.data(), map.size() * sizeof(int2), cudaMemcpyHostToDevice, ctx->stream));
  const double t_prep = ms_since(t_enter);
  OPE_CUDA_TRY(ctx, ope::stream_sync(ctx));
  if (trace) fprintf(stderr, "[ope batch] icp launch: host preparation %.3f ms, then %.3f ms until the stream had drained\n", t_prep, ms_since(t_enter) - t_prep);
  const size_t nt8 = (max_nt + 7) & ~(size_t)7;
  const size_t smem_bytes = ((sizeof(IcpSmallSmem<THREADS>) + 15) & ~(size_t)15) + nt8 * sizeof(float4) + (nt8 / 8) * 2 * sizeof(float4) +
                            (size_t)kSlabSlots * THREADS * sizeof(float2);
  const void* kernel = (const void*)icp_small_batch_kernel<THREADS>;
  OPE_TRY(dyn_smem(ctx, kernel, smem_bytes));
  int per_sm = 0;
  OPE_CUDA_TRY(ctx, cudaOccupancyMaxActiveBlocksPerMultiprocessor(&per_sm, kernel, THREADS, smem_bytes));
  if ((size_t)per_sm * ctx->sm_count < (size_t)kIcpSmallMaxBlocks) return fail(ctx, OPE_ERR_CUDA, "icp_small_batch_kernel: one alignment's blocks cannot be co-resident");
  cudaEventRecord(ctx->kev[0][0], ctx->stream);
  icp_small_batch_kernel<THREADS><<<(unsigned)total_blocks, THREADS, smem_bytes, ctx->stream>>>(d_descs.p, d_map.p, bars.p + n_frames);
  cudaEventRecord(ctx->kev[0][1], ctx->stream);
  ctx->kev_valid[0] = true;
  return check_launch(ctx, "icp_small_batch_kernel");
}

int icp_small_batch_device(ope_ctx* ctx, const ope_icp_params& prm, const IcpBatchFrame* frames, int n_frames, ope_reg_result* d_results) {
  const char* e = std::getenv("OPE_ICP_BATCH_THREADS");
  const int t = e ? std::atoi(e) : 256;
  if (t == 128) return icp_small_batch_launch<128>(ctx, prm, frames, n_frames, d_results);
  return icp_small_batch_launch<256>(ctx, prm, frames, n_frames, d_results);
}

}

using namespace ope;

extern "C" {

void ope_icp_params_default(ope_icp_params* p) {
  std::memset(p, 0, sizeof(*p));
  p->max_iterations = 10;
  p->transformation_epsilon = 0.0;
  p->euclidean_fitness_epsilon = -DBL_MAX;
  p->max_correspondence_distance = std::sqrt(DBL_MAX);
  p->min_number_correspondences = 3;
  p->estimator = OPE_EST_NEAREST;
  p->k_search = 10;
  p->transformation = OPE_TE_SVD;
  p->variant = OPE_ICP_VARIANT_MOD;
  p->mse_threshold_absolute = 1e-12;
}
void ope_sacia_params_default(ope_sacia_params* p) {
  std::memset(p, 0, sizeof(*p));
  p->max_iterations = 10; p->nr_samples = 3; p->k_correspondences = 10; p->min_sample_distance = 0.0f;
  p->max_correspondence_distance = std::sqrt(DBL_MAX);
}
void ope_pose_params_default(ope_pose_params* p) {
  std::memset(p, 0, sizeof(*p));
  p->coarse_leaf = 0.01f; p->fine_leaf = 0.008f; p->normal_k = 30; p->fpfh_radius = 0.03f;
  ope_sacia_params_default(&p->sacia);
  p->sacia.max_iterations = 400; p->sacia.nr_samples = 5; p->sacia.k_correspondences = 5;
  p->sacia.min_sample_distance = 0.01f; p->sacia.max_correspondence_distance = 0.05;
  p->min_target_features = 10; p->min_target_points = 100;
  ope_icp_params_default(&p->icp);
  p->icp.max_iterations = 100; p->icp.transformation_epsilon = 1e-8; p->icp.euclidean_fitness_epsilon = 1e-8;
  p->icp.estimator = OPE_EST_NORMAL_SHOOTING; p->icp.k_search = 20;
  p->icp.n_rejectors = 2;
  p->icp.rejector_kind[0] = OPE_REJ_SURFACE_NORMAL; p->icp.rejector_threshold[0] = 0.7;
  p->icp.rejector_kind[1] = OPE_REJ_SELF_OCCLUDED_NORMAL; p->icp.rejector_threshold[1] = 0.6;
  p->icp.transformation = OPE_TE_SVD; p->icp.with_normals = 1;
  p->coarse_refit_threshold = 1e-4;
}

int ope_cloud_transform(ope_ctx* ctx, const ope_cloud* cloud, const float T[16], ope_cloud** out) {
  OPE_ENTER(ctx);
  if (!ctx || !cloud || !T || !out) return OPE_ERR_INVALID;
  ope_cloud* o = nullptr;
  OPE_TRY(cloud_alloc(ctx, cloud->n, cloud->normals != nullptr, &o));
  Mat4 M;
  std::memcpy(M.m, T, sizeof(M.m));
  int rc = transform_device(ctx, cloud, M, o);
  if (rc != OPE_OK) { ope_cloud_free(ctx, o); return rc; }
  OPE_CUDA_TRY(ctx, ope::stream_sync(ctx));
  *out = o;
  return OPE_OK;
}

int ope_umeyama(ope_ctx* ctx, const ope_cloud* src, const ope_cloud* tgt, const int32_t* isrc, const int32_t* itgt, size_t n,
                float T[16]) {
  OPE_ENTER(ctx);
  if (!ctx || !src || !tgt || !T || n == 0) return OPE_ERR_INVALID;
  if ((!isrc && n > src->n) || (!itgt && n > tgt->n)) return fail(ctx, OPE_ERR_INVALID, "n exceeds cloud size");
  Scratch<int> ds(ctx), dt(ctx);
  if (isrc) {
    for (size_t i = 0; i < n; ++i) if (isrc[i] < 0 || (size_t)isrc[i] >= src->n) return fail(ctx, OPE_ERR_INVALID, "source index out of range");
    OPE_TRY(ds.alloc(n));
    OPE_CUDA_TRY(ctx, cudaMemcpyAsync(ds.p, isrc, n * sizeof(int), cudaMemcpyHostToDevice, ctx->stream));
  }
  if (itgt) {
    for (size_t i = 0; i < n; ++i) if (itgt[i] < 0 || (size_t)itgt[i] >= tgt->n) return fail(ctx, OPE_ERR_INVALID, "target index out of range");
    OPE_TRY(dt.alloc(n));
    OPE_CUDA_TRY(ctx, cudaMemcpyAsync(dt.p, itgt, n * sizeof(int), cudaMemcpyHostToDevice, ctx->stream));
  }
  return umeyama_device(ctx, src->pts, tgt->pts, isrc ? ds.p : nullptr, itgt ? dt.p : nullptr, n, T);
}

int ope_point_to_plane(ope_ctx* ctx, const ope_cloud* src, const ope_cloud* tgt, const int32_t* isrc, const int32_t* itgt, size_t n,
                       int kind, float T[16], int32_t* lm_info) {
  OPE_ENTER(ctx);
  if (!ctx || !src || !tgt || !T) return OPE_ERR_INVALID;
  if (!tgt->normals) return fail(ctx, OPE_ERR_INVALID, "point-to-plane estimation needs target normals");
  if ((!isrc && n > src->n) || (!itgt && n > tgt->n)) return fail(ctx, OPE_ERR_INVALID, "n exceeds cloud size");
  Scratch<int> ds(ctx), dt(ctx);
  std::vector<int> ident;
  if (isrc) {
    for (size_t i = 0; i < n; ++i) if (isrc[i] < 0 || (size_t)isrc[i] >= src->n) return fail(ctx, OPE_ERR_INVALID, "source index out of range");
    OPE_TRY(ds.alloc(n));
    OPE_CUDA_TRY(ctx, cudaMemcpyAsync(ds.p, isrc, n * sizeof(int), cudaMemcpyHostToDevice, ctx->stream));
  }
  if (itgt) {
    for (size_t i = 0; i < n; ++i) if (itgt[i] < 0 || (size_t)itgt[i] >= tgt->n) return fail(ctx, OPE_ERR_INVALID, "target index out of range");
  } else {
    ident.resize(n);
    for (size_t i = 0; i < n; ++i) ident[i] = (int)i;
    itgt = ident.data();
  }
  OPE_TRY(dt.alloc(n));
  OPE_CUDA_TRY(ctx, cudaMemcpyAsync(dt.p, itgt, n * sizeof(int), cudaMemcpyHostToDevice, ctx->stream));
  Mat4 M;
  int rc = point_to_plane_device(ctx, src->pts, tgt->pts, tgt->normals, isrc ? ds.p : nullptr, dt.p, nullptr, n, kind, &M, nullptr, nullptr, lm_info);
  ope::stream_sync(ctx);
  if (rc == OPE_OK) std::memcpy(T, M.m, sizeof(M.m));
  return rc;
}

int ope_fitness(ope_ctx* ctx, const ope_cloud* src, const ope_cloud* tgt, const float T[16], double max_range, double* out) {
  OPE_ENTER(ctx);
  if (!ctx || !src || !tgt || !T || !out) return OPE_ERR_INVALID;
  if (tgt->n == 0) return fail(ctx, OPE_ERR_EMPTY, "No input target dataset was given!");
  Mat4 M;
  std::memcpy(M.m, T, sizeof(M.m));
  return fitness_device(ctx, src, tgt, M, max_range, out);
}

int ope_correspondences(ope_ctx* ctx, const ope_cloud* src, const ope_cloud* tgt, const ope_icp_params* prm,
                        ope_correspondence* out, size_t* out_n) {
  OPE_ENTER(ctx);
  if (!ctx || !src || !tgt || !prm || !out || !out_n) return OPE_ERR_INVALID;
  *out_n = 0;
  if (tgt->n == 0) return fail(ctx, OPE_ERR_EMPTY, "No input target dataset was given!");
  if (src->n == 0) return OPE_OK;
  IcpDev a;
  std::memset(&a, 0, sizeof(a));
  OPE_TRY(icp_fill(ctx, src, tgt, *prm, &a));
  a.variant = OPE_ICP_VARIANT_MOD;
  a.cur_pts = src->pts; a.cur_nrm = src->normals;
  const size_t n = src->n;
  Scratch<int> match(ctx), seed(ctx);
  Scratch<float> d2(ctx);
  const bool shooting = prm->estimator == OPE_EST_NORMAL_SHOOTING;
  OPE_TRY(match.alloc(n)); OPE_TRY(d2.alloc(n));
  OPE_TRY(seed.alloc(shooting ? n * (size_t)prm->k_search : n));
  a.corr_match = match.p; a.corr_d2 = d2.p; a.seed = seed.p;
  OPE_TRY(dyn_smem(ctx, (const void*)correspond_once_kernel, sizeof(IcpSmem)));
  const size_t want = shooting ? div_up(n, kIcpWarps) : div_up(n, kIcpThreads);
  correspond_once_kernel<<<(unsigned)std::min<size_t>(want, (size_t)ctx->sm_count * 4), kIcpThreads, sizeof(IcpSmem), ctx->stream>>>(a);
  OPE_TRY(check_launch(ctx, "correspond_once_kernel"));
  if (prm->use_reciprocal) {
    OPE_TRY(cloud_bbox(ctx, const_cast<ope_cloud*>(src)));
    GridView gsrc;
    OPE_TRY(cloud_grid(ctx, src, knn_cell_size(src, 1), &gsrc));
    OPE_TRY(dyn_smem(ctx, (const void*)reciprocal_filter_kernel, sizeof(IcpSmem)));
    reciprocal_filter_kernel<<<(unsigned)std::min<size_t>(div_up(n, kIcpThreads), (size_t)ctx->sm_count * 4), kIcpThreads, sizeof(IcpSmem),
                               ctx->stream>>>(gsrc, tgt->pts, match.p, (int)n, a.max_d2_f, a.max_corr_dist);
    OPE_TRY(check_launch(ctx, "reciprocal_filter_kernel"));
  }
  std::vector<int> hm(n);
  std::vector<float> hd(n);
  OPE_CUDA_TRY(ctx, cudaMemcpyAsync(hm.data(), match.p, n * sizeof(int), cudaMemcpyDeviceToHost, ctx->stream));
  OPE_CUDA_TRY(ctx, cudaMemcpyAsync(hd.data(), d2.p, n * sizeof(float), cudaMemcpyDeviceToHost, ctx->stream));
  OPE_CUDA_TRY(ctx, ope::stream_sync(ctx));
  corr_to_host(hm, hd, out, out_n);
  return OPE_OK;
}

int ope_icp_align(ope_ctx* ctx, const ope_cloud* src, const ope_cloud* tgt, const ope_icp_params* prm, const float guess[16],
                  ope_reg_result* res, ope_correspondence* out_corr, ope_cloud** out_aligned) {
  OPE_ENTER(ctx);
  if (!ctx || !src || !prm || !res) return OPE_ERR_INVALID;
  Mat4 I = mat4_identity();
  std::memset(res, 0, sizeof(*res));
  std::memcpy(res->T, I.m, sizeof(I.m));
  if (out_aligned) *out_aligned = nullptr;
  if (!tgt || tgt->n == 0) return fail(ctx, OPE_ERR_EMPTY, "No input target dataset was given!");
  Mat4 G = I;
  if (guess) std::memcpy(G.m, guess, sizeof(G.m));
  return icp_device(ctx, src, tgt, *prm, G, res, out_corr, out_aligned);
}

int ope_icp_align_fixed(ope_ctx* ctx, const ope_cloud* src, const ope_cloud* tgt, const ope_icp_params* prm, const float guess[16],
                        ope_correspondence* fixed, size_t n_fixed, ope_reg_result* res, ope_correspondence* out_corr, ope_cloud** out_aligned) {
  OPE_ENTER(ctx);
  if (!ctx || !src || !prm || !res || (n_fixed && !fixed)) return OPE_ERR_INVALID;
  if (n_fixed == 0) return ope_icp_align(ctx, src, tgt, prm, guess, res, out_corr, out_aligned);
  Mat4 I = mat4_identity();
  std::memset(res, 0, sizeof(*res));
  std::memcpy(res->T, I.m, sizeof(I.m));
  if (out_aligned) *out_aligned = nullptr;
  if (!tgt || tgt->n == 0) return fail(ctx, OPE_ERR_EMPTY, "No input target dataset was given!");
  Mat4 G = I;
  if (guess) std::memcpy(G.m, guess, sizeof(G.m));
  return icp_stepwise_device(ctx, src, tgt, *prm, G, res, out_corr, out_aligned, fixed, n_fixed);
}

int ope_sacia_draw(const float* src_xyz, size_t ns, size_t stride_bytes, int iterations, int nr_samples, int k_correspondences,
                   float* min_sample_distance, int32_t* samples, int32_t* picks) {
  if (!src_xyz || !samples || !picks || !min_sample_distance || stride_bytes % 4 != 0 || stride_bytes < 12) return OPE_ERR_INVALID;
  LibcRandSession rng;
  for (int it = 0; it < iterations; ++it) {
    int rc = draw_samples(rng, src_xyz, ns, stride_bytes / 4, nr_samples, *min_sample_distance, samples + (size_t)it * nr_samples);
    if (rc != OPE_OK) return rc;
    for (int s = 0; s < nr_samples; ++s) picks[(size_t)it * nr_samples + s] = rng.index(k_correspondences);
  }
  return OPE_OK;
}

int ope_sacia_align(ope_ctx* ctx, const ope_cloud* src, const float* fsrc, const ope_cloud* tgt, const float* ftgt,
                    const ope_sacia_params* prm, const ope_rng_table* table, ope_reg_result* res, float* out_errors) {
  OPE_ENTER(ctx);
  if (!ctx || !src || !fsrc || !tgt || !ftgt || !prm || !res) return OPE_ERR_INVALID;
  Mat4 I = mat4_identity();
  std::memset(res, 0, sizeof(*res));
  std::memcpy(res->T, I.m, sizeof(I.m));
  Scratch<float> dfs(ctx), dft(ctx);
  OPE_TRY(dfs.alloc(src->n * 33)); OPE_TRY(dft.alloc(tgt->n * 33));
  if (src->n) OPE_CUDA_TRY(ctx, cudaMemcpyAsync(dfs.p, fsrc, src->n * 33 * sizeof(float), cudaMemcpyHostToDevice, ctx->stream));
  if (tgt->n) OPE_CUDA_TRY(ctx, cudaMemcpyAsync(dft.p, ftgt, tgt->n * 33 * sizeof(float), cudaMemcpyHostToDevice, ctx->stream));
  return sacia_device(ctx, src, dfs.p, tgt, dft.p, *prm, table, nullptr, res, out_errors);
}

}
```

Measured before the change: 6664.

## Run each small ICP alignment in one block with chunked work loop

Restructures the batched small-cloud ICP kernel so that each alignment runs in a single block. The block loops over 32-point chunks and keeps its convergence state in shared memory, replacing the multi-block design that synchronised through a global barrier. Per-point current positions, normals and kNN seeds are persisted in global scratch between iterations. This removes inter-block barrier and ticket-map overhead but gives each alignment far less parallelism. The default lane chunk grouping in the batch scheduler is also enlarged.

```diff
diff --git a/object-pose-estimation_b200/csrc/pipeline.cu b/object-pose-estimation_b200/csrc/pipeline.cu
--- a/object-pose-estimation_b200/csrc/pipeline.cu
+++ b/object-pose-estimation_b200/csrc/pipeline.cu
@@ -280,7 +280,7 @@
   size_t chunk = chunk_items ? chunk_items : (size_t)std::max(1, ce ? std::atoi(ce) : 296);
   if (!ce && !chunk_items) {
     if (lanes > 1) {
-      const size_t per_round = (size_t)lanes * 32;
+      const size_t per_round = (size_t)lanes * 128;
       const size_t rounds = std::max<size_t>(1, (n + per_round / 2) / per_round);
       chunk = std::max<size_t>(std::min<size_t>(8, n), (n + rounds * lanes - 1) / (rounds * lanes));
     } else {
diff --git a/object-pose-estimation_b200/csrc/registration.cu b/object-pose-estimation_b200/csrc/registration.cu
--- a/object-pose-estimation_b200/csrc/registration.cu
+++ b/object-pose-estimation_b200/csrc/registration.cu
@@ -223,6 +223,7 @@
   int* corr_match;
   float* corr_d2;
   int* seed;
+  unsigned* knn_prev;
   float4* ref;
   float cert_gap;
   int dfs_max;
@@ -836,6 +837,12 @@
   column[i * THREADS] = v;
 }
 
+struct IcpSmallConv {
+  Mat4 final_t;
+  double prev_mse, cur_mse;
+  int similar, iterations, state, converged, n_corr;
+};
+
 template <int THREADS>
 struct IcpSmallSmem {
   double red[THREADS / 32][kIcpAcc];
@@ -843,63 +850,94 @@
   float2 knn_buf[THREADS / 32][kKnnBufCap + 32];
   float4 wbox[THREADS / 32][2];
   Mat4 T_inc;
+  IcpSmallConv conv;
   int stop;
+  int next_chunk;
 };
 
 template <int THREADS>
-__device__ __forceinline__ void icp_small_body(const IcpDev& a, const int bid, const int nblk) {
-  constexpr int kIcpThreads = THREADS, kIcpWarps = THREADS / 32;
+struct IcpSmallView {
+  IcpSmallSmem<THREADS>* sm;
+  float4* tg;
+  float4* blo;
+  float4* bhi;
+  float2* slab;
+  int n_groups;
+  double morg[3];
+};
+
+template <int THREADS>
+__device__ __forceinline__ IcpSmallView<THREADS> icp_small_prepare(const IcpDev& a) {
   extern __shared__ __align__(16) unsigned char smem_raw[];
-  double morg[3];
-  { const float4 t0 = a.n_tgt > 0 ? __ldg(a.tgt_pts) : make_float4(0, 0, 0, 0); moment_origin(t0.x, t0.y, t0.z, morg[0], morg[1], morg[2]); }
-  IcpSmallSmem<THREADS>* sm = reinterpret_cast<IcpSmallSmem<THREADS>*>(smem_raw);
-  float4* tg = reinterpret_cast<float4*>(smem_raw + ((sizeof(IcpSmallSmem<THREADS>) + 15) & ~(size_t)15));
-  const int n_tgt8 = (a.n_tgt + 7) & ~7, n_groups = n_tgt8 >> 3;
-  float4* blo = tg + n_tgt8;
-  float4* bhi = blo + n_groups;
-  float2* slab = reinterpret_cast<float2*>(bhi + n_groups);
+  IcpSmallView<THREADS> v;
+  { const float4 t0 = a.n_tgt > 0 ? __ldg(a.tgt_pts) : make_float4(0, 0, 0, 0); moment_origin(t0.x, t0.y, t0.z, v.morg[0], v.morg[1], v.morg[2]); }
+  v.sm = reinterpret_cast<IcpSmallSmem<THREADS>*>(smem_raw);
+  v.tg = reinterpret_cast<float4*>(smem_raw + ((sizeof(IcpSmallSmem<THREADS>) + 15) & ~(size_t)15));
+  const int n_tgt8 = (a.n_tgt + 7) & ~7;
+  v.n_groups = n_tgt8 >> 3;
+  v.blo = v.tg + n_tgt8;
+  v.bhi = v.blo + v.n_groups;
+  v.slab = reinterpret_cast<float2*>(v.bhi + v.n_groups);
+  const int tid = threadIdx.x;
+  for (int j = tid; j < n_tgt8; j += THREADS) v.tg[j] = j < a.n_tgt ? __ldg(a.tgt_pts + j) : make_float4(INFINITY, INFINITY, INFINITY, 0.0f);
+  if (tid == 0) {
+    IcpSmallConv& cv = v.sm->conv;
+    cv.final_t = a.guess;
+    cv.prev_mse = DBL_MAX; cv.cur_mse = DBL_MAX;
+    cv.similar = 0; cv.iterations = 0; cv.state = OPE_CONV_NOT_CONVERGED; cv.converged = 0; cv.n_corr = 0;
+    v.sm->next_chunk = 0;
+  }
+  __syncthreads();
+  for (int g = tid; g < v.n_groups; g += THREADS) {
+    float4 lo = make_float4(INFINITY, INFINITY, INFINITY, 0.0f), hi = make_float4(-INFINITY, -INFINITY, -INFINITY, 0.0f);
+    for (int u = 0; u < 8; ++u) {
+      const float4 t = v.tg[8 * g + u];
+      if (!finite3(t.x, t.y, t.z)) continue;
+      lo.x = fminf(lo.x, t.x); lo.y = fminf(lo.y, t.y); lo.z = fminf(lo.z, t.z);
+      hi.x = fmaxf(hi.x, t.x); hi.y = fmaxf(hi.y, t.y); hi.z = fmaxf(hi.z, t.z);
+    }
+    v.blo[g] = lo; v.bhi[g] = hi;
+  }
+  __syncthreads();
+  return v;
+}
+
+__device__ __forceinline__ void icp_small_input(const IcpDev& a, int s, float4& p, float4& nv, int& orig) {
+  p = __ldg(a.src_sorted + s);
+  orig = __float_as_int(p.w);
+  nv = a.src0_nrm ? __ldg(a.src0_nrm + orig) : make_float4(0, 0, 0, 0);
+  if (!mat4_is_identity(a.guess)) {
+    float x, y, z;
+    xform_point(a.guess, p.x, p.y, p.z, x, y, z);
+    p.x = x; p.y = y; p.z = z;
+    if (a.src0_nrm && finite3(nv.x, nv.y, nv.z)) { xform_normal(a.guess, nv.x, nv.y, nv.z, x, y, z); nv.x = x; nv.y = y; nv.z = z; }
+  }
+}
+
+__device__ __forceinline__ void icp_small_xform(const Mat4& T, bool normals, float4& p, float4& nv) {
+  if (!finite3(p.x, p.y, p.z)) return;
+  float x, y, z;
+  xform_point(T, p.x, p.y, p.z, x, y, z);
+  p.x = x; p.y = y; p.z = z;
+  if (normals && finite3(nv.x, nv.y, nv.z)) { xform_normal(T, nv.x, nv.y, nv.z, x, y, z); nv.x = x; nv.y = y; nv.z = z; }
+}
+
+template <int THREADS>
+__device__ __forceinline__ int icp_small_query(const IcpDev& a, const IcpSmallView<THREADS>& v, const int pass, const float4 p,
+                                               const float4 nv, const int orig, const bool ok, const bool tally, float& d2m,
+                                               long long* t_phase, long long t0) {
+  constexpr int kIcpThreads = THREADS;
+  IcpSmallSmem<THREADS>* sm = v.sm;
+  const float4* tg = v.tg;
+  const float4* blo = v.blo;
+  const float4* bhi = v.bhi;
+  float2* slab = v.slab;
+  const int n_groups = v.n_groups;
   const unsigned full = 0xffffffffu;
   const int tid = threadIdx.x, lane = tid & 31, warp = tid >> 5;
-  const int s = bid * kIcpThreads + tid;
-  const bool in_range = s < a.n_work;
   const bool stale = a.variant == OPE_ICP_VARIANT_MODCORR;
   const int k = a.k_search < a.grid.n ? a.k_search : a.grid.n;
   auto col = [&](int slot) -> float2& { return slab[slot * kIcpThreads + tid]; };
-
-  float4 p = make_float4(0, 0, 0, 0), nv = make_float4(0, 0, 0, 0);
-  int orig = 0;
-  if (in_range) {
-    p = __ldg(a.src_sorted + s);
-    orig = __float_as_int(p.w);
-    if (a.src0_nrm) nv = __ldg(a.src0_nrm + orig);
-    if (!mat4_is_identity(a.guess)) {
-      float x, y, z;
-      xform_point(a.guess, p.x, p.y, p.z, x, y, z);
-      p.x = x; p.y = y; p.z = z;
-      if (a.src0_nrm && finite3(nv.x, nv.y, nv.z)) { xform_normal(a.guess, nv.x, nv.y, nv.z, x, y, z); nv.x = x; nv.y = y; nv.z = z; }
-    }
-  }
-  for (int j = tid; j < n_tgt8; j += kIcpThreads) tg[j] = j < a.n_tgt ? __ldg(a.tgt_pts + j) : make_float4(INFINITY, INFINITY, INFINITY, 0.0f);
-  __syncthreads();
-  for (int g = tid; g < n_groups; g += kIcpThreads) {
-    float4 lo = make_float4(INFINITY, INFINITY, INFINITY, 0.0f), hi = make_float4(-INFINITY, -INFINITY, -INFINITY, 0.0f);
-    for (int u = 0; u < 8; ++u) {
-      const float4 t = tg[8 * g + u];
-      if (!finite3(t.x, t.y, t.z)) continue;
-      lo.x = fminf(lo.x, t.x); lo.y = fminf(lo.y, t.y); lo.z = fminf(lo.z, t.z);
-      hi.x = fmaxf(hi.x, t.x); hi.y = fmaxf(hi.y, t.y); hi.z = fmaxf(hi.z, t.z);
-    }
-    blo[g] = lo; bhi[g] = hi;
-  }
-  __syncthreads();
-  const bool ok = in_range && k > 0 && finite3(p.x, p.y, p.z);
-
-  Mat4 final_t = a.guess;
-  double prev_mse = DBL_MAX, cur_mse = DBL_MAX;
-  int similar = 0, iterations = 0, state = OPE_CONV_NOT_CONVERGED, converged = 0, n_corr = 0;
-  unsigned bar_target = 0;
-  const bool prof = a.phase_cycles != nullptr && bid == 0 && tid == 0;
-  long long t_phase[4] = {0, 0, 0, 0};
 
   auto coop_query = [&](int q, float bound) {
     const float qx = __shfl_sync(full, p.x, q), qy = __shfl_sync(full, p.y, q), qz = __shfl_sync(full, p.z, q);
@@ -910,204 +948,275 @@
     return cnt;
   };
 
-  for (int pass = 0;; ++pass) {
-    long long t0 = prof ? clock64() : 0;
-    int c = 0;
-    bool have = false;
-    bool seeded = pass > 0;
-    if (pass == 0) {
-      const bool leader = (lane & 7) == 0;
-      const unsigned lead = __ballot_sync(full, ok && leader);
-      for (unsigned m = lead; m != 0u; m &= m - 1u) { const int q = __ffs(m) - 1; const int cnt = coop_query(q, FLT_MAX); if (lane == q) { c = cnt; have = true; } }
-      __syncwarp();
-      seeded = !leader && ((lead >> (lane & ~7)) & 1u);
-    }
-    float bound = FLT_MAX;
-    if (ok && !have && seeded) {
-      const float2* seed_col = slab + (pass == 0 ? (tid & ~7) : tid);
-      float b = 0.0f;
-      bool all = true;
+  int c = 0;
+  bool have = false;
+  bool seeded = pass > 0;
+  if (pass == 0) {
+    const bool leader = (lane & 7) == 0;
+    const unsigned lead = __ballot_sync(full, ok && leader);
+    for (unsigned m = lead; m != 0u; m &= m - 1u) { const int q = __ffs(m) - 1; const int cnt = coop_query(q, FLT_MAX); if (lane == q) { c = cnt; have = true; } }
+    __syncwarp();
+    seeded = !leader && ((lead >> (lane & ~7)) & 1u);
+  }
+  float bound = FLT_MAX;
+  if (ok && !have && seeded) {
+    const float2* seed_col = slab + (pass == 0 ? (tid & ~7) : tid);
+    float b = 0.0f;
+    bool all = true;
 #pragma unroll 4
-      for (int j = 0; j < k; ++j) {
-        const int idx = __float_as_int(seed_col[j * kIcpThreads].y);
-        if (idx < 0) { all = false; continue; }
-        const float4 t = tg[idx];
-        b = fmaxf(b, dist2(p.x, p.y, p.z, t.x, t.y, t.z));
-      }
-      if (all) bound = b;
-    }
-    if (pass == 0) __syncwarp();
-    const bool scan = ok && !have && bound < FLT_MAX;
-    int n_ins = 0;
-    bool heaped = false;
-    float2 root = make_float2(0.0f, 0.0f);
-    const long long ts0 = a.phase_cycles ? clock64() : 0;
-    if (__any_sync(full, scan)) {
-      auto insert_full = [&](float d2, int j) {
-        ++n_ins;
-        if (!heaped) {
-          for (int i = kSlabSlots / 2 - 1; i >= 0; --i) heap_sift<THREADS>(slab + tid, i, col(i), kSlabSlots);
-          heaped = true;
-          root = col(0);
-          bound = root.x;
+    for (int j = 0; j < k; ++j) {
+      const int idx = __float_as_int(seed_col[j * kIcpThreads].y);
+      if (idx < 0) { all = false; continue; }
+      const float4 t = tg[idx];
+      b = fmaxf(b, dist2(p.x, p.y, p.z, t.x, t.y, t.z));
+    }
+    if (all) bound = b;
+  }
+  if (pass == 0) __syncwarp();
+  const bool scan = ok && !have && bound < FLT_MAX;
+  int n_ins = 0;
+  bool heaped = false;
+  float2 root = make_float2(0.0f, 0.0f);
+  const long long ts0 = a.phase_cycles ? clock64() : 0;
+  if (__any_sync(full, scan)) {
+    auto insert_full = [&](float d2, int j) {
+      ++n_ins;
+      if (!heaped) {
+        for (int i = kSlabSlots / 2 - 1; i >= 0; --i) heap_sift<THREADS>(slab + tid, i, col(i), kSlabSlots);
+        heaped = true;
+        root = col(0);
+        bound = root.x;
+      }
+      if (nb_less(d2, j, root.x, __float_as_int(root.y))) {
+        heap_sift<THREADS>(slab + tid, 0, make_float2(d2, __int_as_float(j)), kSlabSlots);
+        root = col(0);
+        bound = root.x;
+      }
+    };
+    float wlx = scan ? p.x : INFINITY, wly = scan ? p.y : INFINITY, wlz = scan ? p.z : INFINITY;
+    float whx = scan ? p.x : -INFINITY, why = scan ? p.y : -INFINITY, whz = scan ? p.z : -INFINITY;
+    float wb = scan ? bound : 0.0f;
+#pragma unroll
+    for (int o = 16; o > 0; o >>= 1) {
+      wlx = fminf(wlx, __shfl_xor_sync(full, wlx, o)); wly = fminf(wly, __shfl_xor_sync(full, wly, o)); wlz = fminf(wlz, __shfl_xor_sync(full, wlz, o));
+      whx = fmaxf(whx, __shfl_xor_sync(full, whx, o)); why = fmaxf(why, __shfl_xor_sync(full, why, o)); whz = fmaxf(whz, __shfl_xor_sync(full, whz, o));
+      wb = fmaxf(wb, __shfl_xor_sync(full, wb, o));
+    }
+    if (lane == 0) { sm->wbox[warp][0] = make_float4(wlx, wly, wlz, wb * 1.0002f + 1e-30f); sm->wbox[warp][1] = make_float4(whx, why, whz, 0.0f); }
+    __syncwarp();
+    for (int g0 = 0; g0 < n_groups; g0 += 32) {
+      bool near = false;
+      if (g0 + lane < n_groups) {
+        const float4 lo = blo[g0 + lane], hi = bhi[g0 + lane], wl = sm->wbox[warp][0], wh = sm->wbox[warp][1];
+        const float ex = fmaxf(fmaxf(lo.x - wh.x, wl.x - hi.x), 0.0f), ey = fmaxf(fmaxf(lo.y - wh.y, wl.y - hi.y), 0.0f),
+                    ez = fmaxf(fmaxf(lo.z - wh.z, wl.z - hi.z), 0.0f);
+        near = ex * ex + ey * ey + ez * ez <= wl.w;
+      }
+      for (unsigned cand = __ballot_sync(full, near); cand != 0u; cand &= cand - 1u) {
+        const int g = g0 + __ffs(cand) - 1;
+        const int j0 = 8 * g;
+        bool mine = scan;
+        if (mine) {
+          const float4 lo = blo[g], hi = bhi[g];
+          const float ex = fmaxf(fmaxf(lo.x - p.x, p.x - hi.x), 0.0f), ey = fmaxf(fmaxf(lo.y - p.y, p.y - hi.y), 0.0f),
+                      ez = fmaxf(fmaxf(lo.z - p.z, p.z - hi.z), 0.0f);
+          mine = ex * ex + ey * ey + ez * ez <= bound * 1.0001f + 1e-30f;
         }
-        if (nb_less(d2, j, root.x, __float_as_int(root.y))) {
-          heap_sift<THREADS>(slab + tid, 0, make_float2(d2, __int_as_float(j)), kSlabSlots);
-          root = col(0);
-          bound = root.x;
-        }
-      };
-      float wlx = scan ? p.x : INFINITY, wly = scan ? p.y : INFINITY, wlz = scan ? p.z : INFINITY;
-      float whx = scan ? p.x : -INFINITY, why = scan ? p.y : -INFINITY, whz = scan ? p.z : -INFINITY;
-      float wb = scan ? bound : 0.0f;
-#pragma unroll
-      for (int o = 16; o > 0; o >>= 1) {
-        wlx = fminf(wlx, __shfl_xor_sync(full, wlx, o)); wly = fminf(wly, __shfl_xor_sync(full, wly, o)); wlz = fminf(wlz, __shfl_xor_sync(full, wlz, o));
-        whx = fmaxf(whx, __shfl_xor_sync(full, whx, o)); why = fmaxf(why, __shfl_xor_sync(full, why, o)); whz = fmaxf(whz, __shfl_xor_sync(full, whz, o));
-        wb = fmaxf(wb, __shfl_xor_sync(full, wb, o));
-      }
-      if (lane == 0) { sm->wbox[warp][0] = make_float4(wlx, wly, wlz, wb * 1.0002f + 1e-30f); sm->wbox[warp][1] = make_float4(whx, why, whz, 0.0f); }
-      __syncwarp();
-      for (int g0 = 0; g0 < n_groups; g0 += 32) {
-        bool near = false;
-        if (g0 + lane < n_groups) {
-          const float4 lo = blo[g0 + lane], hi = bhi[g0 + lane], wl = sm->wbox[warp][0], wh = sm->wbox[warp][1];
-          const float ex = fmaxf(fmaxf(lo.x - wh.x, wl.x - hi.x), 0.0f), ey = fmaxf(fmaxf(lo.y - wh.y, wl.y - hi.y), 0.0f),
-                      ez = fmaxf(fmaxf(lo.z - wh.z, wl.z - hi.z), 0.0f);
-          near = ex * ex + ey * ey + ez * ez <= wl.w;
-        }
-        for (unsigned cand = __ballot_sync(full, near); cand != 0u; cand &= cand - 1u) {
-          const int g = g0 + __ffs(cand) - 1;
-          const int j0 = 8 * g;
-          bool mine = scan;
-          if (mine) {
-            const float4 lo = blo[g], hi = bhi[g];
-            const float ex = fmaxf(fmaxf(lo.x - p.x, p.x - hi.x), 0.0f), ey = fmaxf(fmaxf(lo.y - p.y, p.y - hi.y), 0.0f),
-                        ez = fmaxf(fmaxf(lo.z - p.z, p.z - hi.z), 0.0f);
-            mine = ex * ex + ey * ey + ez * ez <= bound * 1.0001f + 1e-30f;
-          }
-          if (!mine) continue;
-          float d2[8];
-#pragma unroll
-          for (int u = 0; u < 8; ++u) { const float4 t = tg[j0 + u]; d2[u] = dist2(p.x, p.y, p.z, t.x, t.y, t.z); }
-          unsigned hit = 0u;
-#pragma unroll
-          for (int u = 0; u < 8; ++u) hit |= (d2[u] <= bound ? 1u : 0u) << u;
-          if (hit == 0u) continue;
-          if (c + __popc(hit) <= kSlabSlots) {
-#pragma unroll
-            for (int u = 0; u < 8; ++u)
-              if ((hit >> u) & 1u) { col(c) = make_float2(d2[u], __int_as_float(j0 + u)); ++c; }
-          } else {
-#pragma unroll
-            for (int u = 0; u < 8; ++u) {
-              const bool h = (hit >> u) & 1u;
-              const bool room = c < kSlabSlots;
-              if (h & room) col(c) = make_float2(d2[u], __int_as_float(j0 + u));
-              if (h & !room) insert_full(d2[u], j0 + u);
-              c += (h & room) ? 1 : 0;
-            }
+        if (!mine) continue;
+        float d2[8];
+#pragma unroll
+        for (int u = 0; u < 8; ++u) { const float4 t = tg[j0 + u]; d2[u] = dist2(p.x, p.y, p.z, t.x, t.y, t.z); }
+        unsigned hit = 0u;
+#pragma unroll
+        for (int u = 0; u < 8; ++u) hit |= (d2[u] <= bound ? 1u : 0u) << u;
+        if (hit == 0u) continue;
+        if (c + __popc(hit) <= kSlabSlots) {
+#pragma unroll
+          for (int u = 0; u < 8; ++u)
+            if ((hit >> u) & 1u) { col(c) = make_float2(d2[u], __int_as_float(j0 + u)); ++c; }
+        } else {
+#pragma unroll
+          for (int u = 0; u < 8; ++u) {
+            const bool h = (hit >> u) & 1u;
+            const bool room = c < kSlabSlots;
+            if (h & room) col(c) = make_float2(d2[u], __int_as_float(j0 + u));
+            if (h & !room) insert_full(d2[u], j0 + u);
+            c += (h & room) ? 1 : 0;
           }
         }
       }
     }
-    const bool unserved = ok && !have && (!scan || c < k);
-    const unsigned redo = __ballot_sync(full, unserved);
-    if (a.phase_cycles && pass < 64) {
-      unsigned long long* pc = (unsigned long long*)(a.phase_cycles + 16 + pass * 8);
-      const unsigned long long dt = (unsigned long long)(clock64() - ts0);
-      if (lane == 0) { atomicAdd(pc + 0, dt); atomicMax(pc + 1, dt); atomicAdd(pc + 5, 1ull); }
-      if (n_ins > 0) { atomicAdd(pc + 2, (unsigned long long)n_ins); atomicAdd(pc + 3, 1ull); }
-      if (ok) atomicAdd(pc + 4, (unsigned long long)c);
-    }
-    if (a.phase_cycles && bid == 0 && lane == 0 && pass > 0) atomicAdd((unsigned long long*)&a.phase_cycles[4], (unsigned long long)__popc(redo));
-    if (a.phase_cycles && bid == 0 && ok && pass > 0) atomicAdd((unsigned long long*)&a.phase_cycles[5], (unsigned long long)c);
-    for (unsigned m = redo; m != 0u; m &= m - 1u) {
-      const int q = __ffs(m) - 1;
-      const float bq = __shfl_sync(full, scan ? bound : FLT_MAX, q);
-      const int cnt = coop_query(q, bq);
-      if (lane == q) c = cnt;
-    }
-    __syncwarp();
-    if (prof) { const long long t1 = clock64(); t_phase[0] += t1 - t0; t0 = t1; }
-    int match = -1;
-    float d2m = 0.0f;
-    if (ok && c > 0) {
-      const float4 nr = stale ? __ldg(a.src0_nrm + orig) : nv;
-      const double N0 = nr.x, N1 = nr.y, N2 = nr.z;
-      double best = DBL_MAX;
-      int best_idx = -1, first_idx = -1;
-      float best_d2 = 0.0f, first_d2 = 0.0f;
-      while (heaped && c > k) {
-        --c;
-        if (c > 0) heap_sift<THREADS>(slab + tid, 0, col(c), c);
-      }
-      while (c > k) {
-        int worst = 0;
-        float2 wv = col(0);
-        for (int e = 1; e < c; ++e) { const float2 o = col(e); if (nb_less(wv.x, __float_as_int(wv.y), o.x, __float_as_int(o.y))) { wv = o; worst = e; } }
-        --c;
-        if (worst != c) col(worst) = col(c);
-      }
-      float best_key = 0.0f;
+  }
+  const bool unserved = ok && !have && (!scan || c < k);
+  const unsigned redo = __ballot_sync(full, unserved);
+  if (a.phase_cycles && pass < 64) {
+    unsigned long long* pc = (unsigned long long*)(a.phase_cycles + 16 + pass * 8);
+    const unsigned long long dt = (unsigned long long)(clock64() - ts0);
+    if (lane == 0) { atomicAdd(pc + 0, dt); atomicMax(pc + 1, dt); atomicAdd(pc + 5, 1ull); }
+    if (n_ins > 0) { atomicAdd(pc + 2, (unsigned long long)n_ins); atomicAdd(pc + 3, 1ull); }
+    if (ok) atomicAdd(pc + 4, (unsigned long long)c);
+  }
+  if (a.phase_cycles && tally && lane == 0 && pass > 0) atomicAdd((unsigned long long*)&a.phase_cycles[4], (unsigned long long)__popc(redo));
+  if (a.phase_cycles && tally && ok && pass > 0) atomicAdd((unsigned long long*)&a.phase_cycles[5], (unsigned long long)c);
+  for (unsigned m = redo; m != 0u; m &= m - 1u) {
+    const int q = __ffs(m) - 1;
+    const float bq = __shfl_sync(full, scan ? bound : FLT_MAX, q);
+    const int cnt = coop_query(q, bq);
+    if (lane == q) c = cnt;
+  }
+  __syncwarp();
+  if (t_phase) { const long long t1 = clock64(); t_phase[0] += t1 - t0; t0 = t1; }
+  int match = -1;
+  d2m = 0.0f;
+  if (ok && c > 0) {
+    const float4 nr = stale ? __ldg(a.src0_nrm + orig) : nv;
+    const double N0 = nr.x, N1 = nr.y, N2 = nr.z;
+    double best = DBL_MAX;
+    int best_idx = -1, first_idx = -1;
+    float best_d2 = 0.0f, first_d2 = 0.0f;
+    while (heaped && c > k) {
+      --c;
+      if (c > 0) heap_sift<THREADS>(slab + tid, 0, col(c), c);
+    }
+    while (c > k) {
+      int worst = 0;
+      float2 wv = col(0);
+      for (int e = 1; e < c; ++e) { const float2 o = col(e); if (nb_less(wv.x, __float_as_int(wv.y), o.x, __float_as_int(o.y))) { wv = o; worst = e; } }
+      --c;
+      if (worst != c) col(worst) = col(c);
+    }
+    float best_key = 0.0f;
 #pragma unroll 4
-      for (int e = 0; e < c; ++e) {
-        const float2 mine = col(e);
-        const int mi = __float_as_int(mine.y);
-        if (first_idx < 0 || nb_less(mine.x, mi, first_d2, first_idx)) { first_idx = mi; first_d2 = mine.x; }
-        const float4 t = tg[mi];
-        const float px = t.x - p.x, py = t.y - p.y, pz = t.z - p.z;
-        const double V0 = px, V1 = py, V2 = pz;
-        const double C0 = N1 * V2 - N2 * V1, C1 = N2 * V0 - N0 * V2, C2 = N0 * V1 - N1 * V0;
-        const double dist = C0 * C0 + C1 * C1 + C2 * C2;
-        if (dist < DBL_MAX && (dist < best || (dist == best && nb_less(mine.x, mi, best_key, best_idx)))) {
-          best = dist; best_idx = mi; best_d2 = mine.x; best_key = mine.x;
-        }
-      }
-      const int pick_idx = best_idx < 0 ? first_idx : best_idx;
-      const float pick_d2 = best_idx < 0 ? first_d2 : best_d2;
-      const double min_dist = best_idx < 0 ? DBL_MAX : best;
-      if (!(min_dist > a.max_corr_dist)) { match = pick_idx; d2m = pick_d2; }
-      for (int r = 0; r < a.n_rej && match >= 0; ++r) {
-        const float4 sn = stale ? __ldg(a.src0_nrm + orig) : nv;
-        double score;
-        if (a.rej_kind[r] == OPE_REJ_SURFACE_NORMAL) {
-          const float4 tn = __ldg(a.tgt_nrm + match);
-          score = (double)((sn.x * tn.x) + (sn.y * tn.y) + (sn.z * tn.z));
-        } else {
-          const float4 sp = stale ? __ldg(a.src0_pts + orig) : p;
-          const double sl = (double)sqrtf(sp.x * sp.x + sp.y * sp.y + sp.z * sp.z);
-          score = (double)((sn.x * (-sp.x / sl)) + (sn.y * (-sp.y / sl)) + (sn.z * (-sp.z / sl)));
-        }
-        if (!(score > a.rej_thr[r])) match = -1;
-      }
-    }
-    if (ok) for (int j = (c < k ? c : k); j < k; ++j) col(j) = make_float2(FLT_MAX, __int_as_float(-1));
+    for (int e = 0; e < c; ++e) {
+      const float2 mine = col(e);
+      const int mi = __float_as_int(mine.y);
+      if (first_idx < 0 || nb_less(mine.x, mi, first_d2, first_idx)) { first_idx = mi; first_d2 = mine.x; }
+      const float4 t = tg[mi];
+      const float px = t.x - p.x, py = t.y - p.y, pz = t.z - p.z;
+      const double V0 = px, V1 = py, V2 = pz;
+      const double C0 = N1 * V2 - N2 * V1, C1 = N2 * V0 - N0 * V2, C2 = N0 * V1 - N1 * V0;
+      const double dist = C0 * C0 + C1 * C1 + C2 * C2;
+      if (dist < DBL_MAX && (dist < best || (dist == best && nb_less(mine.x, mi, best_key, best_idx)))) {
+        best = dist; best_idx = mi; best_d2 = mine.x; best_key = mine.x;
+      }
+    }
+    const int pick_idx = best_idx < 0 ? first_idx : best_idx;
+    const float pick_d2 = best_idx < 0 ? first_d2 : best_d2;
+    const double min_dist = best_idx < 0 ? DBL_MAX : best;
+    if (!(min_dist > a.max_corr_dist)) { match = pick_idx; d2m = pick_d2; }
+    for (int r = 0; r < a.n_rej && match >= 0; ++r) {
+      const float4 sn = stale ? __ldg(a.src0_nrm + orig) : nv;
+      double score;
+      if (a.rej_kind[r] == OPE_REJ_SURFACE_NORMAL) {
+        const float4 tn = __ldg(a.tgt_nrm + match);
+        score = (double)((sn.x * tn.x) + (sn.y * tn.y) + (sn.z * tn.z));
+      } else {
+        const float4 sp = stale ? __ldg(a.src0_pts + orig) : p;
+        const double sl = (double)sqrtf(sp.x * sp.x + sp.y * sp.y + sp.z * sp.z);
+        score = (double)((sn.x * (-sp.x / sl)) + (sn.y * (-sp.y / sl)) + (sn.z * (-sp.z / sl)));
+      }
+      if (!(score > a.rej_thr[r])) match = -1;
+    }
+  }
+  if (ok) for (int j = (c < k ? c : k); j < k; ++j) col(j) = make_float2(FLT_MAX, __int_as_float(-1));
+  if (t_phase) t_phase[1] += clock64() - t0;
+  return match;
+}
+
+__device__ __forceinline__ void icp_small_moments(const float4* tg, const double morg[3], const float4 p, int match, float d2m, double* out) {
+  const int lane = threadIdx.x & 31;
+  double v[16];
+#pragma unroll
+  for (int e = 0; e < 16; ++e) v[e] = 0.0;
+  double dsum = 0.0;
+  if (match >= 0) {
+    const float4 t = tg[match];
+#pragma unroll
+    for (int e = 0; e < 16; ++e) v[e] = moment_term(e, p, t, d2m, morg);
+    dsum = (double)d2m;
+  }
+  int slot;
+  const double wsum = warp_reduce16(v, lane, slot);
+  dsum = warp_sum_d(dsum);
+  if ((lane & 1) == 0) out[slot] = wsum;
+  if (lane == 1) out[16] = dsum;
+}
+
+__device__ __forceinline__ int icp_small_converge(const IcpDev& a, const double* totals, const double morg[3], IcpSmallConv& cv, Mat4& T_inc) {
+  int stop = 0;
+  cv.n_corr = (int)totals[0];
+  if (cv.n_corr < a.min_corr) {
+    cv.state = OPE_CONV_NO_CORRESPONDENCES; cv.converged = 0; stop = 2;
+    T_inc = mat4_identity();
+  } else {
+    Mat4 T;
+    umeyama_from_moments(totals, T, morg[0], morg[1], morg[2]);
+    T_inc = T;
+    cv.final_t = mat4_mul(T, cv.final_t);
+    ++cv.iterations;
+    cv.state = OPE_CONV_NOT_CONVERGED;
+    int conv = 0;
+    if (cv.iterations >= a.max_iterations) {
+      if (!a.fail_after_max) { cv.state = OPE_CONV_ITERATIONS; conv = 1; }
+      else { conv = 0; stop = 1; }
+    } else {
+      const double cos_angle = 0.5 * (double)(T(0, 0) + T(1, 1) + T(2, 2) - 1);
+      const double translation_sqr = (double)(T(0, 3) * T(0, 3) + T(1, 3) * T(1, 3) + T(2, 3) * T(2, 3));
+      int hit = 0, hit_state = 0;
+      if (cos_angle >= a.rot_thr && translation_sqr <= a.trans_thr) { hit = 1; hit_state = OPE_CONV_TRANSFORM; }
+      else {
+        cv.cur_mse = totals[16] / (double)cv.n_corr;
+        if (fabs(cv.cur_mse - cv.prev_mse) < a.abs_mse_thr) { hit = 1; hit_state = OPE_CONV_ABS_MSE; }
+        else if (fabs(cv.cur_mse - cv.prev_mse) / cv.prev_mse < a.rel_mse_thr) { hit = 1; hit_state = OPE_CONV_REL_MSE; }
+        else cv.prev_mse = cv.cur_mse;
+      }
+      if (hit) {
+        if (cv.similar < a.max_similar) ++cv.similar;
+        else { cv.similar = 0; cv.state = hit_state; conv = 1; }
+      }
+    }
+    cv.converged = conv;
+    if (a.force_all && cv.iterations < a.max_iterations) conv = 0;
+    if (conv) stop = 1;
+  }
+  return stop;
+}
+
+__device__ __forceinline__ void icp_small_result(const IcpDev& a, const IcpSmallConv& cv) {
+  ope_reg_result r;
+  for (int i = 0; i < 16; ++i) r.T[i] = cv.final_t.m[i];
+  r.converged = cv.converged; r.state = cv.state; r.iterations = cv.iterations; r.n_correspondences = cv.n_corr;
+  r.last_mse = cv.cur_mse; r.best_error = 0.0; r.best_iteration = 0; r.reserved = 0;
+  *a.result = r;
+}
+
+template <int THREADS>
+__global__ void __launch_bounds__(THREADS, 512 / THREADS) icp_small_kernel(IcpDev a) {
+  const int tid = threadIdx.x, warp = tid >> 5, bid = blockIdx.x, nblk = gridDim.x;
+  const int s = bid * THREADS + tid;
+  const bool in_range = s < a.n_work;
+  float4 p = make_float4(0, 0, 0, 0), nv = make_float4(0, 0, 0, 0);
+  int orig = 0;
+  if (in_range) icp_small_input(a, s, p, nv, orig);
+  const IcpSmallView<THREADS> v = icp_small_prepare<THREADS>(a);
+  IcpSmallSmem<THREADS>* sm = v.sm;
+  const int k = a.k_search < a.grid.n ? a.k_search : a.grid.n;
+  const bool ok = in_range && k > 0 && finite3(p.x, p.y, p.z);
+  unsigned bar_target = 0;
+  const bool prof = a.phase_cycles != nullptr && bid == 0 && tid == 0;
+  long long t_phase[4] = {0, 0, 0, 0};
+  for (int pass = 0;; ++pass) {
+    float d2m;
+    const int match = icp_small_query<THREADS>(a, v, pass, p, nv, orig, ok, bid == 0, d2m, prof ? t_phase : nullptr, prof ? clock64() : 0);
     if (in_range) { a.corr_match[orig] = match; a.corr_d2[orig] = d2m; }
-    if (prof) { const long long t1 = clock64(); t_phase[1] += t1 - t0; t0 = t1; }
-    {
-      double v[16];
-#pragma unroll
-      for (int e = 0; e < 16; ++e) v[e] = 0.0;
-      double dsum = 0.0;
-      if (match >= 0) {
-        const float4 t = tg[match];
-#pragma unroll
-        for (int e = 0; e < 16; ++e) v[e] = moment_term(e, p, t, d2m, morg);
-        dsum = (double)d2m;
-      }
-      int slot;
-      const double wsum = warp_reduce16(v, lane, slot);
-      dsum = warp_sum_d(dsum);
-      if ((lane & 1) == 0) sm->red[warp][slot] = wsum;
-      if (lane == 1) sm->red[warp][16] = dsum;
-    }
+    long long t0 = prof ? clock64() : 0;
+    icp_small_moments(v.tg, v.morg, p, match, d2m, sm->red[warp]);
     __syncthreads();
     double* my_partials = a.partials + ((size_t)(pass & 1) * nblk + bid) * kIcpAcc;
     if (tid < kIcpAcc) {
       double sum = 0.0;
 #pragma unroll
-      for (int wv = 0; wv < kIcpWarps; ++wv) sum += sm->red[wv][tid];
+      for (int wv = 0; wv < THREADS / 32; ++wv) sum += sm->red[wv][tid];
       my_partials[tid] = sum;
     }
     if (nblk > 1) { bar_target += nblk; grid_barrier(a.barrier, bar_target); } else __syncthreads();
@@ -1115,92 +1224,117 @@
       const double* base = a.partials + (size_t)(pass & 1) * nblk * kIcpAcc;
       double sum = 0.0;
       for (int b0 = 0; b0 < nblk; b0 += 8) {
-        double v[8];
-#pragma unroll
-        for (int u = 0; u < 8; ++u) v[u] = b0 + u < nblk ? __ldcg(base + (size_t)(b0 + u) * kIcpAcc + tid) : 0.0;
-#pragma unroll
-        for (int u = 0; u < 8; ++u) sum += v[u];
+        double v8[8];
+#pragma unroll
+        for (int u = 0; u < 8; ++u) v8[u] = b0 + u < nblk ? __ldcg(base + (size_t)(b0 + u) * kIcpAcc + tid) : 0.0;
+#pragma unroll
+        for (int u = 0; u < 8; ++u) sum += v8[u];
+      }
+      sm->totals[tid] = sum;
+    }
+    __syncthreads();
+    if (prof) { const long long t1 = clock64(); t_phase[2] += t1 - t0; t0 = t1; }
+    if (tid == 0) sm->stop = icp_small_converge(a, sm->totals, v.morg, sm->conv, sm->T_inc);
+    __syncthreads();
+    const int stop = sm->stop;
+    if (stop != 2 && in_range) icp_small_xform(sm->T_inc, a.src0_nrm != nullptr, p, nv);
+    if (prof) { const long long t1 = clock64(); t_phase[3] += t1 - t0; }
+    if (stop) break;
+  }
+  if (prof) for (int i = 0; i < 4; ++i) a.phase_cycles[i] = t_phase[i];
+  if (bid == 0 && tid == 0) icp_small_result(a, sm->conv);
+}
+
+template <int THREADS>
+__global__ void __launch_bounds__(THREADS, 512 / THREADS) icp_small_batch_kernel(const IcpDev* __restrict__ descs) {
+  __shared__ IcpDev a;
+  for (int w = threadIdx.x; w < (int)(sizeof(IcpDev) / 4); w += THREADS) reinterpret_cast<int*>(&a)[w] = reinterpret_cast<const int*>(descs + blockIdx.x)[w];
+  __syncthreads();
+  const IcpSmallView<THREADS> v = icp_small_prepare<THREADS>(a);
+  IcpSmallSmem<THREADS>* sm = v.sm;
+  const unsigned full = 0xffffffffu;
+  const int tid = threadIdx.x, lane = tid & 31;
+  const int n = a.n_work, n_chunks = (n + 31) >> 5;
+  const int k = a.k_search < a.grid.n ? a.k_search : a.grid.n;
+  const bool normals = a.src0_nrm != nullptr;
+  float2* column = v.slab + tid;
+  const bool prof = a.phase_cycles != nullptr && tid == 0;
+  long long t_phase[4] = {0, 0, 0, 0};
+  for (int pass = 0;; ++pass) {
+    for (;;) {
+      int ch = 0;
+      if (lane == 0) ch = atomicAdd(&sm->next_chunk, 1);
+      ch = __shfl_sync(full, ch, 0);
+      if (ch >= n_chunks) break;
+      const long long t0 = prof ? clock64() : 0;
+      const int s = ch * 32 + lane;
+      const bool in_range = s < n;
+      float4 p = make_float4(0, 0, 0, 0), nv = make_float4(0, 0, 0, 0);
+      int orig = 0;
+      bool ok = false;
+      if (in_range) {
+        if (pass == 0) {
+          icp_small_input(a, s, p, nv, orig);
+          ok = k > 0 && finite3(p.x, p.y, p.z);
+        } else {
+          p = a.cur_pts[s]; nv = a.cur_nrm[s];
+          orig = __float_as_int(p.w);
+          ok = nv.w != 0.0f;
+          icp_small_xform(sm->T_inc, normals, p, nv);
+          if (ok) {
+            unsigned w[kSlabSlots / 2];
+#pragma unroll
+            for (int i = 0; i < kSlabSlots / 2; ++i) w[i] = 2 * i < k ? a.knn_prev[(size_t)i * n + s] : 0u;
+#pragma unroll
+            for (int i = 0; i < kSlabSlots / 2; ++i)
+#pragma unroll
+              for (int h = 0; h < 2; ++h) {
+                const unsigned idx = (w[i] >> (16 * h)) & 0xffffu;
+                if (2 * i + h < k) column[(2 * i + h) * THREADS] = make_float2(0.0f, __int_as_float(idx == 0xffffu ? -1 : (int)idx));
+              }
+          }
+        }
+        a.cur_pts[s] = p;
+        a.cur_nrm[s] = make_float4(nv.x, nv.y, nv.z, ok ? 1.0f : 0.0f);
+      }
+      float d2m;
+      const int match = icp_small_query<THREADS>(a, v, pass, p, nv, orig, ok, true, d2m, prof ? t_phase : nullptr, t0);
+      if (in_range) { a.corr_match[orig] = match; a.corr_d2[orig] = d2m; }
+      if (ok)
+        for (int i = 0; 2 * i < k; ++i) {
+          const unsigned lo = (unsigned)__float_as_int(column[2 * i * THREADS].y) & 0xffffu;
+          const unsigned hi = 2 * i + 1 < k ? (unsigned)__float_as_int(column[(2 * i + 1) * THREADS].y) & 0xffffu : 0xffffu;
+          a.knn_prev[(size_t)i * n + s] = lo | hi << 16;
+        }
+      icp_small_moments(v.tg, v.morg, p, match, d2m, a.partials + (size_t)ch * kIcpAcc);
+    }
+    long long t0 = prof ? clock64() : 0;
+    __syncthreads();
+    if (tid < kIcpAcc) {
+      double sum = 0.0;
+      for (int g = 0; g < n_chunks; g += 8) {
+        double v8[8];
+#pragma unroll
+        for (int u = 0; u < 8; ++u) v8[u] = g + u < n_chunks ? a.partials[(size_t)(g + u) * kIcpAcc + tid] : 0.0;
+        double b = 0.0;
+#pragma unroll
+        for (int u = 0; u < 8; ++u) b += v8[u];
+        sum += b;
       }
       sm->totals[tid] = sum;
     }
     __syncthreads();
     if (prof) { const long long t1 = clock64(); t_phase[2] += t1 - t0; t0 = t1; }
     if (tid == 0) {
-      int stop = 0;
-      n_corr = (int)sm->totals[0];
-      if (n_corr < a.min_corr) {
-        state = OPE_CONV_NO_CORRESPONDENCES; converged = 0; stop = 2;
-        sm->T_inc = mat4_identity();
-      } else {
-        Mat4 T;
-        umeyama_from_moments(sm->totals, T, morg[0], morg[1], morg[2]);
-        sm->T_inc = T;
-        final_t = mat4_mul(T, final_t);
-        ++iterations;
-        state = OPE_CONV_NOT_CONVERGED;
-        int conv = 0;
-        if (iterations >= a.max_iterations) {
-          if (!a.fail_after_max) { state = OPE_CONV_ITERATIONS; conv = 1; }
-          else { conv = 0; stop = 1; }
-        } else {
-          const double cos_angle = 0.5 * (double)(T(0, 0) + T(1, 1) + T(2, 2) - 1);
-          const double translation_sqr = (double)(T(0, 3) * T(0, 3) + T(1, 3) * T(1, 3) + T(2, 3) * T(2, 3));
-          int hit = 0, hit_state = 0;
-          if (cos_angle >= a.rot_thr && translation_sqr <= a.trans_thr) { hit = 1; hit_state = OPE_CONV_TRANSFORM; }
-          else {
-            cur_mse = sm->totals[16] / (double)n_corr;
-            if (fabs(cur_mse - prev_mse) < a.abs_mse_thr) { hit = 1; hit_state = OPE_CONV_ABS_MSE; }
-            else if (fabs(cur_mse - prev_mse) / prev_mse < a.rel_mse_thr) { hit = 1; hit_state = OPE_CONV_REL_MSE; }
-            else prev_mse = cur_mse;
-          }
-          if (hit) {
-            if (similar < a.max_similar) ++similar;
-            else { similar = 0; state = hit_state; conv = 1; }
-          }
-        }
-        converged = conv;
-        if (a.force_all && iterations < a.max_iterations) conv = 0;
-        if (conv) stop = 1;
-      }
-      sm->stop = stop;
+      sm->stop = icp_small_converge(a, sm->totals, v.morg, sm->conv, sm->T_inc);
+      sm->next_chunk = 0;
     }
     __syncthreads();
-    const int stop = sm->stop;
-    if (stop != 2 && in_range && finite3(p.x, p.y, p.z)) {
-      const Mat4 T = sm->T_inc;
-      float x, y, z;
-      xform_point(T, p.x, p.y, p.z, x, y, z);
-      p.x = x; p.y = y; p.z = z;
-      if (a.src0_nrm && finite3(nv.x, nv.y, nv.z)) { xform_normal(T, nv.x, nv.y, nv.z, x, y, z); nv.x = x; nv.y = y; nv.z = z; }
-    }
-    if (prof) { const long long t1 = clock64(); t_phase[3] += t1 - t0; }
-    if (stop) break;
+    if (prof) t_phase[3] += clock64() - t0;
+    if (sm->stop) break;
   }
   if (prof) for (int i = 0; i < 4; ++i) a.phase_cycles[i] = t_phase[i];
-  if (bid == 0 && tid == 0) {
-    ope_reg_result r;
-    for (int i = 0; i < 16; ++i) r.T[i] = final_t.m[i];
-    r.converged = converged; r.state = state; r.iterations = iterations; r.n_correspondences = n_corr;
-    r.last_mse = cur_mse; r.best_error = 0.0; r.best_iteration = 0; r.reserved = 0;
-    *a.result = r;
-  }
-}
-
-template <int THREADS>
-__global__ void __launch_bounds__(THREADS, 512 / THREADS) icp_small_kernel(IcpDev a) {
-  icp_small_body<THREADS>(a, (int)blockIdx.x, (int)gridDim.x);
-}
-template <int THREADS>
-__global__ void __launch_bounds__(THREADS, 512 / THREADS) icp_small_batch_kernel(const IcpDev* __restrict__ descs, const int2* __restrict__ map,
-                                                                                unsigned* ticket) {
-  __shared__ int s_ticket;
-  __shared__ IcpDev s_desc;
-  if (threadIdx.x == 0) s_ticket = (int)atomicAdd(ticket, 1u);
-  __syncthreads();
-  const int2 fb = map[s_ticket];
-  for (int w = threadIdx.x; w < (int)(sizeof(IcpDev) / 4); w += THREADS) reinterpret_cast<int*>(&s_desc)[w] = reinterpret_cast<const int*>(descs + fb.x)[w];
-  __syncthreads();
-  icp_small_body<THREADS>(s_desc, fb.y, (s_desc.n_work + THREADS - 1) / THREADS);
+  if (tid == 0) icp_small_result(a, sm->conv);
 }
 
 __global__ void __launch_bounds__(kIcpThreads, 1) correspond_once_kernel(IcpDev a) {
@@ -2427,35 +2561,46 @@
          n_tgt <= (size_t)kIcpSmemMaxTargets && n_src > 0 && n_src <= (size_t)kIcpSmallMaxBlocks * kIcpSmallThreads &&
          prm.k_search >= 1 && prm.k_search <= kSlabSlots;
 }
-template <int THREADS>
-static int icp_small_batch_launch(ope_ctx* ctx, const ope_icp_params& prm, const IcpBatchFrame* frames, int n_frames, ope_reg_result* d_results) {
+static constexpr int kIcpBatchThreads = 256;
+
+int icp_small_batch_device(ope_ctx* ctx, const ope_icp_params& prm, const IcpBatchFrame* frames, int n_frames, ope_reg_result* d_results) {
+  constexpr int THREADS = kIcpBatchThreads;
   if (n_frames <= 0) return OPE_OK;
   const bool trace = std::getenv("OPE_BATCH_TRACE") != nullptr;
   auto now = [] { return std::chrono::steady_clock::now(); };
   auto ms_since = [&](std::chrono::steady_clock::time_point t) { return std::chrono::duration<double, std::milli>(now() - t).count(); };
   const auto t_enter = now();
   std::vector<IcpDev> descs((size_t)n_frames);
-  std::vector<int2> map;
-  size_t max_nt = 0, total_src = 0, total_blocks = 0;
+  size_t max_nt = 0, total_src = 0, total_chunks = 0;
   for (int i = 0; i < n_frames; ++i) {
     if (!icp_small_batch_applicable(prm, (size_t)frames[i].n_src, (size_t)frames[i].n_tgt)) return fail(ctx, OPE_ERR_UNSUPPORTED, "alignment %d does not fit the small-cloud ICP kernel", i);
     max_nt = std::max(max_nt, (size_t)frames[i].n_tgt);
     total_src += (size_t)frames[i].n_src;
-    total_blocks += ((size_t)frames[i].n_src + THREADS - 1) / THREADS;
-  }
+    total_chunks += ((size_t)frames[i].n_src + 31) / 32;
+  }
+  for (int r = 0; r < prm.n_rejectors; ++r)
+    if (prm.rejector_kind[r] != OPE_REJ_SURFACE_NORMAL && prm.rejector_kind[r] != OPE_REJ_SELF_OCCLUDED_NORMAL)
+      return fail(ctx, OPE_ERR_UNSUPPORTED, "unknown correspondence rejector kind %d", prm.rejector_kind[r]);
   Scratch<int> match(ctx);
   Scratch<float> d2(ctx);
+  Scratch<float4> state(ctx);
+  Scratch<unsigned> seeds(ctx);
   Scratch<double> partials(ctx);
-  Scratch<unsigned> bars(ctx);
   Scratch<IcpDev> d_descs(ctx);
-  Scratch<int2> d_map(ctx);
   OPE_TRY(match.alloc(total_src)); OPE_TRY(d2.alloc(total_src));
-  OPE_TRY(partials.alloc(2 * total_blocks * kIcpAcc));
-  OPE_TRY(bars.alloc((size_t)n_frames + 1));
-  OPE_TRY(d_descs.alloc((size_t)n_frames)); OPE_TRY(d_map.alloc(total_blocks));
-  OPE_CUDA_TRY(ctx, cudaMemsetAsync(bars.p, 0, ((size_t)n_frames + 1) * sizeof(unsigned), ctx->stream));
-  size_t so = 0, bo = 0;
-  map.reserve(total_blocks);
+  OPE_TRY(state.alloc(2 * total_src));
+  const size_t words = ((size_t)prm.k_search + 1) / 2;
+  OPE_TRY(seeds.alloc(total_src * words));
+  OPE_TRY(partials.alloc(total_chunks * kIcpAcc));
+  OPE_TRY(d_descs.alloc((size_t)n_frames));
+  Scratch<long long> phases(ctx);
+  const bool profile = std::getenv("OPE_PROFILE") != nullptr;
+  const size_t n_prof = 16 + 64 * 8 + 64 + 64 * 4;
+  if (profile) {
+    OPE_TRY(phases.alloc(n_prof));
+    OPE_CUDA_TRY(ctx, cudaMemsetAsync(phases.p, 0, n_prof * sizeof(long long), ctx->stream));
+  }
+  size_t so = 0, co = 0;
   for (int i = 0; i < n_frames; ++i) {
     IcpDev& a = descs[(size_t)i];
     std::memset(&a, 0, sizeof(a));
@@ -2476,42 +2621,48 @@
     a.rel_mse_thr = prm.euclidean_fitness_epsilon; a.abs_mse_thr = prm.mse_threshold_absolute;
     a.max_similar = prm.max_iterations_similar_transforms; a.fail_after_max = prm.failure_after_max_iterations;
     a.guess = mat4_identity();
-    const int nblk = (f.n_src + THREADS - 1) / THREADS;
     a.corr_match = match.p + so; a.corr_d2 = d2.p + so;
-    a.partials = partials.p + 2 * bo * kIcpAcc;
-    a.barrier = bars.p + i;
+    a.cur_pts = state.p + so; a.cur_nrm = state.p + total_src + so;
+    a.knn_prev = seeds.p + so * words;
+    a.partials = partials.p + co * kIcpAcc;
     a.result = d_results + i;
-    for (int b = 0; b < nblk; ++b) map.push_back(make_int2(i, b));
-    so += (size_t)f.n_src; bo += (size_t)nblk;
-  }
-  for (int r = 0; r < prm.n_rejectors; ++r)
-    if (prm.rejector_kind[r] != OPE_REJ_SURFACE_NORMAL && prm.rejector_kind[r] != OPE_REJ_SELF_OCCLUDED_NORMAL)
-      return fail(ctx, OPE_ERR_UNSUPPORTED, "unknown correspondence rejector kind %d", prm.rejector_kind[r]);
+    if (profile && i == 0) a.phase_cycles = phases.p;
+    so += (size_t)f.n_src; co += ((size_t)f.n_src + 31) / 32;
+  }
   OPE_CUDA_TRY(ctx, cudaMemcpyAsync(d_descs.p, descs.data(), descs.size() * sizeof(IcpDev), cudaMemcpyHostToDevice, ctx->stream));
-  OPE_CUDA_TRY(ctx, cudaMemcpyAsync(d_map.p, map.data(), map.size() * sizeof(int2), cudaMemcpyHostToDevice, ctx->stream));
   const double t_prep = ms_since(t_enter);
   OPE_CUDA_TRY(ctx, ope::stream_sync(ctx));
   if (trace) fprintf(stderr, "[ope batch] icp launch: host preparation %.3f ms, then %.3f ms until the stream had drained\n", t_prep, ms_since(t_enter) - t_prep);
   const size_t nt8 = (max_nt + 7) & ~(size_t)7;
   const size_t smem_bytes = ((sizeof(IcpSmallSmem<THREADS>) + 15) & ~(size_t)15) + nt8 * sizeof(float4) + (nt8 / 8) * 2 * sizeof(float4) +
                             (size_t)kSlabSlots * THREADS * sizeof(float2);
-  const void* kernel = (const void*)icp_small_batch_kernel<THREADS>;
-  OPE_TRY(dyn_smem(ctx, kernel, smem_bytes));
-  int per_sm = 0;
-  OPE_CUDA_TRY(ctx, cudaOccupancyMaxActiveBlocksPerMultiprocessor(&per_sm, kernel, THREADS, smem_bytes));
-  if ((size_t)per_sm * ctx->sm_count < (size_t)kIcpSmallMaxBlocks) return fail(ctx, OPE_ERR_CUDA, "icp_small_batch_kernel: one alignment's blocks cannot be co-resident");
+  OPE_TRY(dyn_smem(ctx, (const void*)icp_small_batch_kernel<THREADS>, smem_bytes));
   cudaEventRecord(ctx->kev[0][0], ctx->stream);
-  icp_small_batch_kernel<THREADS><<<(unsigned)total_blocks, THREADS, smem_bytes, ctx->stream>>>(d_descs.p, d_map.p, bars.p + n_frames);
+  icp_small_batch_kernel<THREADS><<<(unsigned)n_frames, THREADS, smem_bytes, ctx->stream>>>(d_descs.p);
   cudaEventRecord(ctx->kev[0][1], ctx->stream);
   ctx->kev_valid[0] = true;
-  return check_launch(ctx, "icp_small_batch_kernel");
-}
-
-int icp_small_batch_device(ope_ctx* ctx, const ope_icp_params& prm, const IcpBatchFrame* frames, int n_frames, ope_reg_result* d_results) {
-  const char* e = std::getenv("OPE_ICP_BATCH_THREADS");
-  const int t = e ? std::atoi(e) : 256;
-  if (t == 128) return icp_small_batch_launch<128>(ctx, prm, frames, n_frames, d_results);
-  return icp_small_batch_launch<256>(ctx, prm, frames, n_frames, d_results);
+  OPE_TRY(check_launch(ctx, "icp_small_batch_kernel"));
+  if (profile) {
+    std::vector<long long> c(n_prof);
+    ope_reg_result r0;
+    OPE_CUDA_TRY(ctx, cudaMemcpyAsync(c.data(), phases.p, n_prof * sizeof(long long), cudaMemcpyDeviceToHost, ctx->stream));
+    OPE_CUDA_TRY(ctx, cudaMemcpyAsync(&r0, d_results, sizeof(r0), cudaMemcpyDeviceToHost, ctx->stream));
+    OPE_CUDA_TRY(ctx, ope::stream_sync(ctx));
+    const double it = std::max(r0.iterations, 1);
+    const int n0 = frames[0].n_src;
+    if (std::getenv("OPE_PROFILE_ITER")) {
+      fprintf(stderr, "[ope profile] icp_small_batch alignment 0 per iteration: mean chunk scan cycles | slowest chunk | overflow calls | threads overflowing | candidates per query\n");
+      for (int p = 0; p < std::min(r0.iterations, 64); ++p) {
+        const long long* q = c.data() + 16 + p * 8;
+        fprintf(stderr, "  it %2d: %7.0f %7lld %6lld %5lld %5.1f\n", p, (double)q[0] / (double)std::max<long long>(q[5], 1), q[1], q[2], q[3],
+                (double)q[4] / (double)std::max(n0, 1));
+      }
+    }
+    fprintf(stderr, "[ope profile] icp_small_batch_kernel alignment 0 (%d queries, %d iterations), thread 0 cycles per iteration: search %.0f | "
+            "rank+shoot+reject %.0f | moments+barrier %.0f | svd %.0f | cooperative re-searches per iteration %.1f | candidates per query %.1f\n",
+            n0, r0.iterations, c[0] / it, c[1] / it, c[2] / it, c[3] / it, c[4] / it, c[5] / it / std::max(n0, 1));
+  }
+  return OPE_OK;
 }
 
 }
```

After: 6390 (median of 6 runs). 4.1% lower.
